# fumchin/bird-sound-event-detecion

Measured on AMD Instinct MI355X. Metric: 10 s clips/sec through mel+CRNN train step, higher is better.
Workload: dtype f32; 1 GPU; waveform->STFT/mel/dB->CRNN(7 conv/BN/GLU/pool + 2xBiGRU128)->Predictor->BCE strong+weak->backward->Adam; BASELINE configs[2] (main_baseline.py train step on SYN); mode=crnn, sr=22050, frames=865, out_frames=216, batch_per_gpu=256, global_batch=256, parallelism=dp1, hip_graph=False

## Files before the change

### bird-sound-event-detecion_amd/csrc/bsed_common.h

```cpp
#pragma once
#include <hip/hip_runtime.h>
#include <stdint.h>
#include <stdio.h>
#include <algorithm>
#include "../../include/bsed.h"

#define BSED_OK 0
#define BSED_ERR_ARG (-1)
#define BSED_ERR_HIP (-2)
#define BSED_ERR_STATE (-3)

void bsed_set_error(const char* fmt, ...);
const uint64_t* bsed_seed_add_ptr();
const int* bsed_step_add_ptr();
const float* bsed_lr_ptr();

#define BSED_CHECK_ARG(cond, ...)                 \
  do {                                            \
    if (!(cond)) {                                \
      bsed_set_error(__VA_ARGS__);                \
      return BSED_ERR_ARG;                        \
    }                                             \
  } while (0)

// ... 210 lines not shown
  return kernel >= 0 && kernel < 8 ? names[kernel] : nullptr;
}
static inline int bsed_glu_plan_for(const BsedGluDesc& d, int kernel, BsedGluPlan& p) {
  const char* who = bsed_glu_name(kernel);
  BSED_CHECK_ARG(who, "bsed_glu_plan: unknown kernel %d", kernel);
  const bool tiled = kernel >= BSED_GLU_BWD_FUSED, glu3 = kernel >= BSED_GLU_FWD3;
  const bool block0 = kernel == BSED_GLU_BLOCK0_FWD || kernel == BSED_GLU_BLOCK0_BWD;
  const int C = d.C;
  BSED_CHECK_ARG(d.NB > 0 && d.H > 0 && d.W > 0, "%s: bad shape", who);
  BSED_CHECK_ARG((d.ph == 1 || d.ph == 2) && (d.pw == 1 || d.pw == 2), "%s: pooling windows must be 1 or 2", who);
  BSED_CHECK_ARG(d.act_bf16 == 0 || (d.act_bf16 == 1 && (glu3 || block0)), "%s: no bf16 activations (act_bf16 = %d)",
                 who, d.act_bf16);
  if (!tiled) BSED_CHECK_ARG(C == 16, "%s: built for 16 channels (got %d)", who, C);
  else if (kernel == BSED_GLU_BWD3) BSED_CHECK_ARG(C == 32 || C == 64, "%s: built for C in {32,64} (got %d)", who, C);
  else if (kernel == BSED_GLU_BWD3N) BSED_CHECK_ARG(C == 128, "%s: built for C = 128 (got %d)", who, C);
  else BSED_CHECK_ARG(C == 32 || C == 64 || C == 128, "%s: built for C in {32,64,128} (got %d)", who, C);
  const long positions = (long)d.NB * d.H * d.W;
  p.dw_rows = 0; p.variant = 0; p.table_bytes = 0;
  if (!tiled) {
    BSED_CHECK_ARG(d.TH == 0 && d.TW == 0, "%s: a streaming kernel without a tile: TH = TW = 0 (got %dx%d)", who, d.TH,
                   d.TW);
    BSED_CHECK_ARG(d.W % d.pw == 0 && d.H >= d.ph, "%s: bad shape (W %% pw == 0, H >= ph)", who);
    BSED_CHECK_ARG(!block0 || positions < (1L << 31), "%s: too many positions", who);
    const long rows = (long)d.NB * (d.H / d.ph);
    long items = rows, g = std::min<long>(rows, 8192);
    if (kernel == BSED_GLU_16_BWD) {
      items = (long)d.NB * d.H * ((d.W + 63) / 64);
      g = std::min<long>(2048, (long)d.NB * d.H);
    } else if (kernel == BSED_GLU_BLOCK0_FWD) {
      items = rows * ((d.W + 127) / 128);
      g = std::min<long>(items, 8192);
    } else if (kernel == BSED_GLU_BLOCK0_BWD) {
      items = rows * ((d.W + 63) / 64);
      g = std::min<long>(8192, rows);
    }
    BSED_CHECK_ARG(items < (1L << 30), "%s: too many rows", who);
    p.G = (int)g; p.max_G = (int)items;
    if (kernel == BSED_GLU_16_BWD || kernel == BSED_GLU_BLOCK0_BWD) p.dw_rows = p.G;
    if (block0) p.variant = d.ph | (positions < (1L << 28) && !(d.act_bf16 && kernel == BSED_GLU_BLOCK0_FWD) ? 16 : 0);
    return BSED_OK;
  }
  BSED_CHECK_ARG(d.TH * d.TW == 128, "%s: TH*TW must be 128 (got %dx%d)", who, d.TH, d.TW);
  const int lgTW = ilog2_exact(d.TW);
  BSED_CHECK_ARG(lgTW >= 0, "%s: TW must be a power of two", who);
  BSED_CHECK_ARG(d.W % d.TW == 0, "%s: TW must divide W", who);
  const long ntiles = (long)d.NB * ceil_div(d.H, d.TH) * (d.W / d.TW);
  BSED_CHECK_ARG(ntiles < (1L << 31), "%s: too many tiles", who);
  BSED_CHECK_ARG(!glu3 || positions * C < (1L << 32),
                 "%s: activation tensor beyond the 32-bit element offsets of this kernel", who);
  int round = 0, slabs = 0;
  if (kernel == BSED_GLU_BWD_FUSED) {
    round = C == 128 ? 256 : (C == 64 ? 512 : 768);
    slabs = C == 128 ? 1 : (C == 64 ? 2 : 4);
    p.variant = C == 128 ? 8 : 4;
  } else if (kernel == BSED_GLU_FWD3) {
    round = C == 128 ? 512 : 1536;
  } else if (kernel == BSED_GLU_BWD3) {
    round = C == 32 ? 768 : 512;
    slabs = 4;
  } else {
    round = 256;
    p.table_bytes = (size_t)2 * 4 * 8 * 2 * 64 * 16;
  }
  p.max_G = (int)(kernel == BSED_GLU_BWD3N ? (ntiles + 1) / 2 : ntiles);
  p.G = std::min(p.max_G, round);
  p.dw_rows = p.G * slabs;
  if (kernel == BSED_GLU_FWD3 || kernel == BSED_GLU_BWD3) p.variant = lgTW == 4 ? 4 : -1;
  return BSED_OK;
}

static inline int bsed_glu_args(const BsedGluDesc* desc, int kernel, unsigned reads, BsedGluPlan& plan,
                                const uint64_t*& seed_add) {
  const char* who = bsed_glu_name(kernel);
  BSED_CHECK_ARG(desc, "%s: null descriptor", who);
  const BsedGluDesc& d = *desc;
  const int rc = bsed_glu_plan_for(d, kernel, plan);
  if (rc) return rc;
  static const char* const names[] = {"x", "y", "cw", "cb", "scale", "shift", "w", "wfwd", "bias", "dpool", "pooled", "g",
                                      "dlin", "part_dw", "part_db", "part_st", "part_gx", "frag_table"};
  const void* const ptrs[] = {d.x, d.y, d.cw, d.cb, d.scale, d.shift, d.w, d.wfwd, d.bias, d.dpool, d.pooled, d.g,
                              d.dlin, d.part_dw, d.part_db, d.part_st, d.part_gx, d.frag_table};
  for (int i = 0; i < 18; ++i) {
    const bool wants = (reads >> i) & 1;
    BSED_CHECK_ARG(wants == (ptrs[i] != nullptr), wants ? "%s: null tensor %s" : "%s: does not read %s: it must be null",
                   who, names[i]);
  }
  BSED_CHECK_ARG(d.G > 0 && d.G <= plan.max_G, "%s: G must be in 1..%d (got %d)", who, plan.max_G, d.G);
  seed_add = bsed_seed_add_ptr();
  return BSED_OK;
}
enum : unsigned {
  GLU_X = 1u << 0, GLU_Y = 1u << 1, GLU_CONV = 3u << 2 , GLU_BN = 3u << 4 , GLU_W = 1u << 6,
  GLU_WFWD = 1u << 7, GLU_BIAS = 1u << 8, GLU_DPOOL = 1u << 9, GLU_POOLED = 1u << 10, GLU_G = 1u << 11,
  GLU_DLIN = 1u << 12, GLU_PART_DW = 1u << 13, GLU_PART_B = 3u << 14 , GLU_PART_GX = 1u << 16,
  GLU_FRAG = 1u << 17,
  GLU_LIN = GLU_BN | GLU_W | GLU_BIAS
};

template <class Params>
static int bsed_glu_geometry(Params& P, const BsedGluDesc* desc, int kernel, unsigned reads, BsedGluPlan& plan) {
  const int rc = bsed_glu_args(desc, kernel, reads, plan, P.seed_add);
  if (rc) return rc;
  const BsedGluDesc& d = *desc;
  P.y = d.y; P.scale = d.scale; P.shift = d.shift; P.bias = d.bias; P.dpool = d.dpool;
  P.g = d.g; P.part_dw = d.part_dw; P.part_db = d.part_db; P.part_st = d.part_st;
  P.NB = d.NB; P.H = d.H; P.W = d.W; P.TH = d.TH; P.TW = d.TW;
  P.lgTW = ilog2_exact(d.TW);
  P.tilesH = ceil_div(d.H, d.TH); P.tilesW = d.W / d.TW;
  P.ntiles = d.NB * P.tilesH * P.tilesW;
  P.ph = d.ph; P.pw = d.pw; P.Hp = d.H / d.ph; P.Wp = d.W / d.pw;
  P.drop_p = d.drop_p; P.rng_stream = d.rng_stream; P.seed = d.seed;
  return BSED_OK;
}

#if defined(__HIPCC__)
__device__ __forceinline__ uint4 philox4x32(uint64_t counter, uint32_t stream, uint64_t seed) {
  uint32_t c0 = (uint32_t)counter, c1 = (uint32_t)(counter >> 32), c2 = stream, c3 = 0x5eed5eedu;
  uint32_t k0 = (uint32_t)seed, k1 = (uint32_t)(seed >> 32);
#pragma unroll
  for (int r = 0; r < 10; ++r) {
    const uint32_t M0 = 0xD2511F53u, M1 = 0xCD9E8D57u;
    uint32_t hi0 = __umulhi(M0, c0), lo0 = M0 * c0;
    uint32_t hi1 = __umulhi(M1, c2), lo1 = M1 * c2;
    uint32_t n0 = hi1 ^ c1 ^ k0, n1 = lo1, n2 = hi0 ^ c3 ^ k1, n3 = lo0;
    c0 = n0; c1 = n1; c2 = n2; c3 = n3;
    k0 += 0x9E3779B9u; k1 += 0xBB67AE85u;
  }
  return make_uint4(c0, c1, c2, c3);
}

__device__ __forceinline__ float dropout_scale(uint64_t e, uint32_t stream, uint64_t seed, float p) {
  if (p <= 0.f) return 1.f;
  uint4 r = philox4x32(e >> 2, stream, seed);
  uint32_t w = (e & 3) == 0 ? r.x : (e & 3) == 1 ? r.y : (e & 3) == 2 ? r.z : r.w;
  float u = (float)(w >> 8) * (1.0f / 16777216.0f);
  return u >= p ? 1.0f / (1.0f - p) : 0.f;
}

__device__ __forceinline__ float sigmoidf_(float x) { return 1.0f / (1.0f + expf(-x)); }
__device__ __forceinline__ float sigmoid_fast(float x) { return __builtin_amdgcn_rcpf(1.0f + __expf(-x)); }

__device__ __forceinline__ uint32_t mix32(uint32_t x) {
  x ^= x >> 16; x *= 0x7feb352dU; x ^= x >> 15; x *= 0x846ca68bU; x ^= x >> 16;
  return x;
}
__device__ __forceinline__ uint32_t drop_key(uint32_t stream, uint64_t seed) {
  return mix32((uint32_t)seed ^ (stream * 0x9E3779B9u)) + mix32((uint32_t)(seed >> 32) ^ 0x85ebca6bu);
}
__device__ __forceinline__ uint32_t drop_threshold(float p) { return (uint32_t)(p * 16777216.0f); }
__device__ __forceinline__ float drop_mul(uint64_t e, uint32_t key, uint32_t thr, float scale) {
  const uint32_t h = mix32((uint32_t)e * 0x9E3779B1u + key + (uint32_t)(e >> 32) * 0x85ebca6bu);
  return (h >> 8) >= thr ? scale : 0.f;
}

__device__ __forceinline__ uint32_t drop_threshold16(float p) { return (uint32_t)(p * 65536.0f); }
__device__ __forceinline__ void drop_mul2(uint64_t e_even, uint32_t key, uint32_t thr16, float scale, float& m0,
                                          float& m1) {
  const uint64_t e = e_even >> 1;
  const uint32_t h = mix32((uint32_t)e * 0x9E3779B1u + key + (uint32_t)(e >> 32) * 0x85ebca6bu);
  m0 = (h & 0xFFFFu) >= thr16 ? scale : 0.f;
  m1 = (h >> 16) >= thr16 ? scale : 0.f;
}

__device__ __forceinline__ void drop_mul2_32(uint32_t e_even, uint32_t key, uint32_t thr16, float scale, float& m0,
                                             float& m1) {
  const uint32_t h = mix32((e_even >> 1) * 0x9E3779B1u + key);
  m0 = (h & 0xFFFFu) >= thr16 ? scale : 0.f;
  m1 = (h >> 16) >= thr16 ? scale : 0.f;
}

__device__ __forceinline__ float wave_sum(float v) {
#pragma unroll
  for (int o = 32; o > 0; o >>= 1) v += __shfl_xor(v, o, 64);
  return v;
}
__device__ __forceinline__ float wave_max(float v) {
#pragma unroll
  for (int o = 32; o > 0; o >>= 1) v = fmaxf(v, __shfl_xor(v, o, 64));
  return v;
}
#endif
```

### bird-sound-event-detecion_amd/csrc/capi.hip

```cpp
#include "bsed_common.h"
#include "../../include/bsed.h"
#include <stdarg.h>

static thread_local char g_err[512] = "";

void bsed_set_error(const char* fmt, ...) {
  va_list ap;
  va_start(ap, fmt);
  vsnprintf(g_err, sizeof(g_err), fmt, ap);
  va_end(ap);
}

extern "C" const char* bsed_last_error(void) { return g_err; }
extern "C" const char* bsed_build_info(void) { return "libbsed gfx950: fp32 storage/accumulation, split-fp32 (bf16x3) contractions on v_mfma_f32_32x32x16_bf16 by default, "
         "exact-fp32 v_mfma_f32_32x32x2_f32 kernels selectable (hand-written HIP)"; }
extern "C" int bsed_abi_version(void) { return 15; }

extern "C" int bsed_glu_plan(const BsedGluDesc* desc, int kernel, BsedGluPlan* out) {
  BSED_CHECK_ARG(desc && out, "bsed_glu_plan: null argument");
  return bsed_glu_plan_for(*desc, kernel, *out);
}
extern "C" int bsed_igemm_plan(const BsedIgemmDesc* desc, int kernel, BsedContractPlan* out) {
  static int (*const run[])(const BsedIgemmDesc*, void*, BsedContractPlan*) = {bsed_run_igemm, bsed_run_igemm3,
                                                                                bsed_run_igemm3s, bsed_run_igemm3n};
  BSED_CHECK_ARG(desc && out && kernel >= BSED_CONTRACT_IGEMM && kernel <= BSED_CONTRACT_IGEMM3N,
                 "bsed_igemm_plan: null argument or unknown kernel %d", kernel);
  return run[kernel](desc, nullptr, out);
}
extern "C" int bsed_wgrad_plan(const BsedWgradDesc* desc, int kernel, BsedContractPlan* out) {
  BSED_CHECK_ARG(desc && out && (kernel == BSED_CONTRACT_WGRAD || kernel == BSED_CONTRACT_WGRAD3),
                 "bsed_wgrad_plan: null argument or unknown kernel %d", kernel);
  return bsed_run_wgrad(desc, kernel == BSED_CONTRACT_WGRAD3, nullptr, out);
}

static thread_local const uint64_t* g_seed_add = nullptr;
static thread_local const int* g_step_add = nullptr;
static thread_local const float* g_lr = nullptr;
const uint64_t* bsed_seed_add_ptr() { return g_seed_add; }
const int* bsed_step_add_ptr() { return g_step_add; }
const float* bsed_lr_ptr() { return g_lr; }
extern "C" int bsed_set_step_state(const void* seed_add_dev, const void* step_add_dev, const void* lr_dev) {
  BSED_CHECK_ARG((seed_add_dev != nullptr) == (step_add_dev != nullptr) && (seed_add_dev != nullptr) == (lr_dev != nullptr),
                 "bsed_set_step_state: the three pointers are set together or cleared together");
  g_seed_add = (const uint64_t*)seed_add_dev;
  g_step_add = (const int*)step_add_dev;
  g_lr = (const float*)lr_dev;
  return BSED_OK;
}
__global__ void step_state_advance_kernel(uint64_t* seed_add, int* step_add, uint64_t seed_inc, int step_inc) {
  if (threadIdx.x == 0 && blockIdx.x == 0) { *seed_add += seed_inc; *step_add += step_inc; }
}
extern "C" int bsed_step_state_advance(void* seed_add_dev, void* step_add_dev, uint64_t seed_inc, int step_inc, void* stream) {
  BSED_CHECK_ARG(seed_add_dev && step_add_dev, "bsed_step_state_advance: null state");
  hipLaunchKernelGGL(step_state_advance_kernel, dim3(1), dim3(64), 0, (hipStream_t)stream, (uint64_t*)seed_add_dev,
                     (int*)step_add_dev, seed_inc, step_inc);
  BSED_LAUNCH_CHECK();
  return BSED_OK;
}
```

### bird-sound-event-detecion_amd/csrc/glu3.hip

```cpp
#include "bsed_common.h"
#include "../../include/bsed.h"
#include <algorithm>
#include <stdlib.h>

typedef short bf16x8 __attribute__((ext_vector_type(8)));
typedef uint32_t u32x4 __attribute__((ext_vector_type(4)));

#define G3_THREADS 256
#define G3_M 128

struct Glu3Params {
  const float* y; const float* scale; const float* shift;
  const float* w;
  const float* bias; const float* dpool;
  float* g; float* part_dw; float* part_db; float* part_st;
  float* pooled;
  int NB, H, W, TH, TW, lgTW, tilesH, tilesW, ntiles;
  int ph, pw, Hp, Wp;
  float drop_p; uint32_t rng_stream; uint64_t seed;
  const uint64_t* seed_add;
};

__device__ __forceinline__ void wave_lds_fence() { asm volatile("s_waitcnt lgkmcnt(0)" ::: "memory"); }
template <int NT>
__device__ __forceinline__ void acc_handoff_fence(f32x16 (&acc)[NT]) {
  if constexpr (NT == 1) asm volatile("s_waitcnt lgkmcnt(0)\n\ts_nop 7" : "+v"(acc[0]) :: "memory");
  else if constexpr (NT == 2) asm volatile("s_waitcnt lgkmcnt(0)\n\ts_nop 7" : "+v"(acc[0]), "+v"(acc[1]) :: "memory");
  else asm volatile("s_waitcnt lgkmcnt(0)\n\ts_nop 7" : "+v"(acc[0]), "+v"(acc[1]), "+v"(acc[2]), "+v"(acc[3]) :: "memory");
}
template <int ABF>
__device__ __forceinline__ f32x16 mfma_sp(const bf16x8& a_hi, const bf16x8& a_lo, const bf16x8& b_hi, const bf16x8& b_lo,
                                          f32x16 acc) {
  if (!ABF) {
    acc = __builtin_amdgcn_mfma_f32_32x32x16_bf16(a_lo, b_hi, acc, 0, 0, 0);
    acc = __builtin_amdgcn_mfma_f32_32x32x16_bf16(a_hi, b_lo, acc, 0, 0, 0);
  }
  return __builtin_amdgcn_mfma_f32_32x32x16_bf16(a_hi, b_hi, acc, 0, 0, 0);
}
__device__ __forceinline__ int crow3g(int r, int lh) { return (r & 3) + 8 * (r >> 2) + 4 * lh; }
__device__ __forceinline__ uint32_t rne_bits(float x) {
  const uint32_t u = __float_as_uint(x);
  return u + 0x7FFFu + ((u >> 16) & 1u);
}
__device__ __forceinline__ void split_pack2(float a, float b, uint32_t& hi, uint32_t& lo) { bsed_split2(a, b, hi, lo); }
__device__ __forceinline__ void split_pack8(const float* v, bf16x8& hi, bf16x8& lo) {
  u32x4 h, l;
#pragma unroll
  for (int i = 0; i < 4; ++i) {
    uint32_t hh, ll;
    split_pack2(v[2 * i], v[2 * i + 1], hh, ll);
    h[i] = hh; l[i] = ll;
  }
  hi = __builtin_bit_cast(bf16x8, h);
  lo = __builtin_bit_cast(bf16x8, l);
}

template <int C>
__device__ __forceinline__ void build_weight_frags(const float* __restrict__ w, bf16x8* WF, bf16x8* WB, int tid) {
  constexpr int NT = C / 32, KS = C / 16;
  for (int f = tid; f < NT * KS * 64; f += G3_THREADS) {
    const int lane = f & 63, li = lane & 31, lh = lane >> 5;
    const int ks = (f >> 6) % KS, j = (f >> 6) / KS;
    float v[8];
    bf16x8 hi, lo;
#pragma unroll
    for (int q = 0; q < 8; ++q) v[q] = w[(size_t)(32 * j + li) * C + 16 * ks + 8 * lh + q];
    split_pack8(v, hi, lo);
    WF[((j * KS + ks) * 2 + 0) * 64 + lane] = hi;
    WF[((j * KS + ks) * 2 + 1) * 64 + lane] = lo;
    if (WB) {
#pragma unroll
      for (int q = 0; q < 8; ++q) v[q] = w[(size_t)(16 * ks + 8 * lh + q) * C + 32 * j + li];
      split_pack8(v, hi, lo);
      WB[((j * KS + ks) * 2 + 0) * 64 + lane] = hi;
      WB[((j * KS + ks) * 2 + 1) * 64 + lane] = lo;
    }
  }
}

template <int C, int ABF>
__device__ __forceinline__ float a_frags_issue(const Glu3Params& P, int lgTW, int nb, int th0, int tw0, int wave, int li, int lh,
                                               float (&raw)[C / 16][8]) {
  constexpr int KS = C / 16;
  const int mA = wave * 32 + li;
  const int gh = th0 + (mA >> lgTW), gw = tw0 + (mA & ((1 << lgTW) - 1));
  const bool ok = gh < P.H;
  const size_t rp = (((size_t)nb * P.H + (ok ? gh : 0)) * P.W + gw) * C + 8 * lh;
#pragma unroll
  for (int ks = 0; ks < KS; ++ks) act_ld8<ABF>(P.y, rp + 16 * ks, raw[ks]);
  return ok ? 1.0f : 0.0f;
}
template <int C>
__device__ __forceinline__ void a_frags_finish(const float (&raw)[C / 16][8], float okf, const float* s_sc, const float* s_sh,
                                               int lh, bf16x8* a_hi, bf16x8* a_lo) {
  constexpr int KS = C / 16;
#pragma unroll
  for (int ks = 0; ks < KS; ++ks) {
    const float4 s0 = *reinterpret_cast<const float4*>(s_sc + 16 * ks + 8 * lh);
    const float4 s1 = *reinterpret_cast<const float4*>(s_sc + 16 * ks + 8 * lh + 4);
    const float4 h0 = *reinterpret_cast<const float4*>(s_sh + 16 * ks + 8 * lh);
    const float4 h1 = *reinterpret_cast<const float4*>(s_sh + 16 * ks + 8 * lh + 4);
    float v[8];
    v[0] = fmaf(raw[ks][0], s0.x, h0.x) * okf; v[1] = fmaf(raw[ks][1], s0.y, h0.y) * okf;
    v[2] = fmaf(raw[ks][2], s0.z, h0.z) * okf; v[3] = fmaf(raw[ks][3], s0.w, h0.w) * okf;
    v[4] = fmaf(raw[ks][4], s1.x, h1.x) * okf; v[5] = fmaf(raw[ks][5], s1.y, h1.y) * okf;
    v[6] = fmaf(raw[ks][6], s1.z, h1.z) * okf; v[7] = fmaf(raw[ks][7], s1.w, h1.w) * okf;
    split_pack8(v, a_hi[ks], a_lo[ks]);
  }
}
template <int C, int ABF>
__device__ __forceinline__ void load_a_frags(const Glu3Params& P, int lgTW, const float* s_sc, const float* s_sh, int nb,
                                             int th0, int tw0, int wave, int li, int lh, bf16x8* a_hi, bf16x8* a_lo) {
  float raw[C / 16][8];
  const float okf = a_frags_issue<C, ABF>(P, lgTW, nb, th0, tw0, wave, li, lh, raw);
  a_frags_finish<C>(raw, okf, s_sc, s_sh, lh, a_hi, a_lo);
}

__device__ float g3_sink[G3_M];

__device__ __forceinline__ float drop_mul32(uint32_t e, uint32_t key, uint32_t thr, float scale) {
  const uint32_t h = mix32(e * 0x9E3779B1u + key);
  return (h >> 8) >= thr ? scale : 0.f;
}

#define G3_B32_WPE 3
template <int C, int LGTW, int ABF>
__global__ __launch_bounds__(G3_THREADS, C == 32 ? G3_B32_WPE : 2) void glu_bwd3_kernel(const Glu3Params P) {
  constexpr int NT = C / 32, KS = C / 16;
  const int lgTW = LGTW >= 0 ? LGTW : P.lgTW;
  const int TWc = 1 << lgTW, THc = G3_M >> lgTW;
  constexpr int DP = 2 * C + 8;
  extern __shared__ __align__(16) unsigned char smem_raw[];
  bf16x8* WF = reinterpret_cast<bf16x8*>(smem_raw);
  bf16x8* WB = WF + NT * KS * 2 * 64;
  float* s_sc = reinterpret_cast<float*>(WB + NT * KS * 2 * 64);
  float* s_sh = s_sc + C;
  unsigned short* Dall = reinterpret_cast<unsigned short*>(s_sh + C);
  const int tid = threadIdx.x, wave = __builtin_amdgcn_readfirstlane(tid >> 6), lane = tid & 63, li = lane & 31, lh = lane >> 5;
  unsigned short* D = Dall + wave * 32 * DP;

  build_weight_frags<C>(P.w, WF, WB, tid);
  for (int i = tid; i < C; i += G3_THREADS) { s_sc[i] = P.scale[i]; s_sh[i] = P.shift[i]; }
  __syncthreads();

  const int sph = P.ph >> 1, spw = P.pw >> 1;
  const float inv_pool = 1.0f / (float)(P.ph * P.pw);
  const uint32_t dkey = drop_key(P.rng_stream, P.seed + (P.seed_add ? *P.seed_add : 0)), dthr = drop_threshold(P.drop_p);
  const float dscale = P.drop_p > 0.f ? 1.0f / (1.0f - P.drop_p) : 1.0f;

  float bias[NT], csc[NT], csh[NT], sdb[NT], sgs[NT], sgy[NT];
  f32x16 acc3[NT][NT];
#pragma unroll
  for (int j = 0; j < NT; ++j) {
    bias[j] = P.bias[32 * j + li];
    csc[j] = s_sc[32 * j + li]; csh[j] = s_sh[32 * j + li];
    sdb[j] = 0.f; sgs[j] = 0.f; sgy[j] = 0.f;
#pragma unroll
    for (int jc = 0; jc < NT; ++jc)
#pragma unroll
      for (int r = 0; r < 16; ++r) acc3[j][jc][r] = 0.f;
  }

  constexpr bool PREF = C == 32 && LGTW >= 0;
  constexpr bool KEEPY = C == 32 && LGTW >= 0;
  constexpr bool G2 = C == 32 && LGTW >= 0;
  float nraw[KS][8];
  float nokf = 0.f;
  auto tile_origin = [&](int t, int& nb_, int& th0_, int& tw0_) {
    const int tw_i = t % P.tilesW; t /= P.tilesW;
    const int th_i = t % P.tilesH;
    nb_ = t / P.tilesH; th0_ = th_i * THc; tw0_ = tw_i * TWc;
  };
  if (PREF && (int)blockIdx.x < P.ntiles) {
    int nb_, th0_, tw0_;
    tile_origin(blockIdx.x, nb_, th0_, tw0_);
    nokf = a_frags_issue<C, ABF>(P, lgTW, nb_, th0_, tw0_, wave, li, lh, nraw);
  }
  for (int tile0 = blockIdx.x; tile0 < P.ntiles; tile0 += gridDim.x) {
    int nb, th0, tw0;
    tile_origin(tile0, nb, th0, tw0);
    int lhv = 4 * lh;
    if (LGTW < 0) asm volatile("" : "+v"(lhv));

    f32x16 acc[NT];
    {
      bf16x8 a_hi[KS], a_lo[KS];
      if (PREF) a_frags_finish<C>(nraw, nokf, s_sc, s_sh, lh, a_hi, a_lo);
      else load_a_frags<C, ABF>(P, lgTW, s_sc, s_sh, nb, th0, tw0, wave, li, lh, a_hi, a_lo);
#pragma unroll
      for (int j = 0; j < NT; ++j)
#pragma unroll
        for (int r = 0; r < 16; ++r) acc[j][r] = 0.f;
#pragma unroll
      for (int ks = 0; ks < KS; ++ks)
#pragma unroll
        for (int j = 0; j < NT; ++j) {
          const bf16x8 b_hi = WF[((j * KS + ks) * 2 + 0) * 64 + lane];
          const bf16x8 b_lo = WF[((j * KS + ks) * 2 + 1) * 64 + lane];
          acc[j] = mfma_sp<ABF>(a_hi[ks], a_lo[ks], b_hi, b_lo, acc[j]);
        }
    }
    if (PREF) {
      const int nt = tile0 + (int)gridDim.x < P.ntiles ? tile0 + (int)gridDim.x : tile0;
      int nb_, th0_, tw0_;
      tile_origin(nt, nb_, th0_, tw0_);
      nokf = a_frags_issue<C, ABF>(P, lgTW, nb_, th0_, tw0_, wave, li, lh, nraw);
    }

    bf16x8 da_hi[NT][2], da_lo[NT][2], xb_hi[NT][2], xb_lo[NT][2];
    uint32_t ykeep[KEEPY ? 16 : 1][NT];
#pragma unroll
    for (int f = 0; f < 2; ++f) {
      float dl8[NT][8], xn8[NT][8];
      uint32_t dvr[2][4][NT], yvr[2][4][NT];
      float mk[2][4];
      uint32_t posv[2][4];
      auto issue = [&](int h) {
        const int rg = 2 * f + h;
#pragma unroll
        for (int rr = 0; rr < 4; ++rr) {
          const int mm = wave * 32 + 8 * rg + lhv + rr;
          const int gh = th0 + (mm >> lgTW), gw = tw0 + (mm & (TWc - 1));
          const int gph = gh >> sph, gpw = gw >> spw;
          mk[h][rr] = (gh < P.H && gph < P.Hp && gpw < P.Wp) ? inv_pool : 0.f;
          posv[h][rr] = ((uint32_t)(nb * P.H + min(gh, P.H - 1)) * (uint32_t)P.W + gw) * C + li;
          const uint32_t dpo = ((uint32_t)(nb * P.Hp + min(gph, P.Hp - 1)) * (uint32_t)P.Wp + min(gpw, P.Wp - 1)) * C + li;
#pragma unroll
          for (int j = 0; j < NT; ++j) {
            dvr[h][rr][j] = act_ld_raw<ABF>(P.dpool, dpo + 32 * j);
            yvr[h][rr][j] = act_ld_raw<ABF>(P.y, posv[h][rr] + 32 * j);
          }
        }
      };
      if (G2) { issue(0); issue(1); __builtin_amdgcn_sched_barrier(0); }
#pragma unroll
      for (int h = 0; h < 2; ++h) {
        const int rg = 2 * f + h;
        if (!G2) { issue(h); __builtin_amdgcn_sched_barrier(0); }
#pragma unroll
        for (int rr = 0; rr < 4; ++rr) {
          const int r = 4 * rg + rr;
          const int row = 8 * rg + lhv + rr;
#pragma unroll
          for (int j = 0; j < NT; ++j) {
            const int n = 32 * j + li;
            if (KEEPY) ykeep[r][j] = yvr[h][rr][j];
            const float xn = fmaf(act_cvt<ABF>(yvr[h][rr][j]), csc[j], csh[j]);
            const float sg = sigmoid_fast(xn);
            const float lin = acc[j][r] + bias[j];
            const float dres = act_cvt<ABF>(dvr[h][rr][j]) * mk[h][rr] * drop_mul32(posv[h][rr] + 32 * j, dkey, dthr, dscale);
            const float dl = dres * sg;
            const float tt = dres * lin * sg * (1.0f - sg);
            sdb[j] += dl;
            dl8[j][4 * h + rr] = dl;
            xn8[j][4 * h + rr] = xn;
            acc[j][r] = tt;
            const uint32_t hb = rne_bits(dl) & 0xFFFF0000u;
            D[row * DP + n] = (unsigned short)(hb >> 16);
            D[row * DP + C + n] = (unsigned short)(rne_bits(dl - __uint_as_float(hb)) >> 16);
          }
        }
      }
#pragma unroll
      for (int j = 0; j < NT; ++j) {
        split_pack8(dl8[j], da_hi[j][f], da_lo[j][f]);
        split_pack8(xn8[j], xb_hi[j][f], xb_lo[j][f]);
      }
    }
    acc_handoff_fence<NT>(acc);

#pragma unroll
    for (int ks = 0; ks < KS; ++ks) {
      const bf16x8 d_hi = *reinterpret_cast<const bf16x8*>(D + li * DP + 16 * ks + 8 * lh);
      const bf16x8 d_lo = *reinterpret_cast<const bf16x8*>(D + li * DP + C + 16 * ks + 8 * lh);
#pragma unroll
      for (int j = 0; j < NT; ++j) {
        const bf16x8 b_hi = WB[((j * KS + ks) * 2 + 0) * 64 + lane];
        const bf16x8 b_lo = WB[((j * KS + ks) * 2 + 1) * 64 + lane];
        acc[j] = mfma_sp<ABF>(d_hi, d_lo, b_hi, b_lo, acc[j]);
      }
    }
    wave_lds_fence();

#pragma unroll
    for (int jc = 0; jc < NT; ++jc)
#pragma unroll
      for (int jn = 0; jn < NT; ++jn)
#pragma unroll
        for (int f = 0; f < 2; ++f) {
          acc3[jn][jc] = mfma_sp<ABF>(da_hi[jn][f], da_lo[jn][f], xb_hi[jc][f], xb_lo[jc][f], acc3[jn][jc]);
        }

#pragma unroll
    for (int rg = 0; rg < 4; ++rg) {
      uint32_t yvr[4][NT];
      float okf[4];
      uint32_t posv[4];
      float* gdst[4];
      uint32_t gidx[4];
#pragma unroll
      for (int rr = 0; rr < 4; ++rr) {
        const int mm = wave * 32 + 8 * rg + lhv + rr;
        const int gh = th0 + (mm >> lgTW), gw = tw0 + (mm & (TWc - 1));
        okf[rr] = gh < P.H ? 1.0f : 0.0f;
        posv[rr] = ((uint32_t)(nb * P.H + min(gh, P.H - 1)) * (uint32_t)P.W + gw) * C + li;
        gdst[rr] = gh < P.H ? P.g : g3_sink;
        gidx[rr] = gh < P.H ? posv[rr] : (uint32_t)li;
#pragma unroll
        for (int j = 0; j < NT; ++j) yvr[rr][j] = KEEPY ? ykeep[4 * rg + rr][j] : act_ld_raw<ABF>(P.y, posv[rr] + 32 * j);
      }
      if (!KEEPY) __builtin_amdgcn_sched_barrier(0);
#pragma unroll
      for (int rr = 0; rr < 4; ++rr) {
#pragma unroll
        for (int j = 0; j < NT; ++j) {
          const float gv = acc[j][4 * rg + rr] * okf[rr];
          act_st<ABF>(gdst[rr], gidx[rr] + 32 * j, gv);
          sgs[j] += gv;
          sgy[j] = fmaf(gv, act_cvt<ABF>(yvr[rr][j]), sgy[j]);
        }
      }
    }
  }

#pragma unroll
  for (int jn = 0; jn < NT; ++jn)
#pragma unroll
    for (int jc = 0; jc < NT; ++jc)
#pragma unroll
      for (int r = 0; r < 16; ++r) {
        const int n = 32 * jn + crow3g(r, lh);
        P.part_dw[(((size_t)blockIdx.x * 4 + wave) * C + n) * C + 32 * jc + li] = acc3[jn][jc][r];
      }
  __syncthreads();
  float* red = reinterpret_cast<float*>(Dall);
#pragma unroll
  for (int j = 0; j < NT; ++j) {
    const float a = sdb[j] + __shfl_xor(sdb[j], 32, 64);
    const float b = sgs[j] + __shfl_xor(sgs[j], 32, 64);
    const float c = sgy[j] + __shfl_xor(sgy[j], 32, 64);
    if (lh == 0) {
      red[(wave * 3 + 0) * C + 32 * j + li] = a;
      red[(wave * 3 + 1) * C + 32 * j + li] = b;
      red[(wave * 3 + 2) * C + 32 * j + li] = c;
    }
  }
  __syncthreads();
  for (int e = tid; e < 3 * C; e += G3_THREADS) {
    const int which = e / C, n = e % C;
    const float s = red[(0 * 3 + which) * C + n] + red[(1 * 3 + which) * C + n] + red[(2 * 3 + which) * C + n] +
                    red[(3 * 3 + which) * C + n];
    if (which == 0) {
      P.part_db[((size_t)blockIdx.x * 2 + 0) * C + n] = s;
      P.part_db[((size_t)blockIdx.x * 2 + 1) * C + n] = 0.f;
    } else {
      P.part_st[((size_t)blockIdx.x * 2 + (which - 1)) * C + n] = s;
    }
  }
}

__global__ void glu3_pack_frags_kernel(const float* __restrict__ w, bf16x8* __restrict__ table) {
  constexpr int C = 128, NT = 4, KS = 8;
  const int f = blockIdx.x * blockDim.x + threadIdx.x;
  if (f >= NT * KS * 64) return;
  const int lane = f & 63, li = lane & 31, lh = lane >> 5;
  const int ks = (f >> 6) % KS, j = (f >> 6) / KS;
  bf16x8* WF = table;
  bf16x8* WB = table + NT * KS * 2 * 64;
  float v[8];
  bf16x8 hi, lo;
#pragma unroll
  for (int q = 0; q < 8; ++q) v[q] = w[(size_t)(32 * j + li) * C + 16 * ks + 8 * lh + q];
  split_pack8(v, hi, lo);
  WF[((j * KS + ks) * 2 + 0) * 64 + lane] = hi;
  WF[((j * KS + ks) * 2 + 1) * 64 + lane] = lo;
#pragma unroll
  for (int q = 0; q < 8; ++q) v[q] = w[(size_t)(16 * ks + 8 * lh + q) * C + 32 * j + li];
  split_pack8(v, hi, lo);
  WB[((j * KS + ks) * 2 + 0) * 64 + lane] = hi;
  WB[((j * KS + ks) * 2 + 1) * 64 + lane] = lo;
}

#define G3N_THREADS 512
template <int ABF>
__global__ __launch_bounds__(G3N_THREADS) void glu_bwd3n_kernel(const Glu3Params P, const bf16x8* __restrict__ table,
                                                                float* __restrict__ dlin) {
  constexpr int C = 128, NT = 4, KS = 8;
#ifdef G3N_LGTW
  constexpr int g3n_lgTW = G3N_LGTW, g3n_TW = 1 << G3N_LGTW;
#else
  const int g3n_lgTW = P.lgTW, g3n_TW = P.TW;
#endif
  constexpr int DQ = 2 * 16 + 8;
  extern __shared__ __align__(16) unsigned char smem_raw[];
  bf16x8* WF = reinterpret_cast<bf16x8*>(smem_raw);
  bf16x8* WB = WF + NT * KS * 2 * 64;
  float* s_sc = reinterpret_cast<float*>(WB + NT * KS * 2 * 64);
  float* s_sh = s_sc + C;
  unsigned short* Dall = reinterpret_cast<unsigned short*>(s_sh + C);
  const int tid = threadIdx.x, wave8 = __builtin_amdgcn_readfirstlane(tid >> 6), lane = tid & 63, li = lane & 31, lh = lane >> 5;
  const int wave = wave8 & 3, half = wave8 >> 2;
  unsigned short* D = Dall + wave8 * 32 * DQ;

  for (int i = tid; i < 2 * NT * KS * 2 * 64; i += G3N_THREADS) WF[i] = table[i];
  for (int i = tid; i < C; i += G3N_THREADS) { s_sc[i] = P.scale[i]; s_sh[i] = P.shift[i]; }
  __syncthreads();

  const int sph = P.ph >> 1, spw = P.pw >> 1;
  const float inv_pool = 1.0f / (float)(P.ph * P.pw);
  const uint32_t dkey = drop_key(P.rng_stream, P.seed + (P.seed_add ? *P.seed_add : 0)), dthr = drop_threshold(P.drop_p);
  const float dscale = P.drop_p > 0.f ? 1.0f / (1.0f - P.drop_p) : 1.0f;

  float bias[NT], csc[NT], csh[NT], sdb[NT], sgs[NT], sgy[NT];
#pragma unroll
  for (int j = 0; j < NT; ++j) {
    bias[j] = P.bias[32 * j + li];
    csc[j] = s_sc[32 * j + li]; csh[j] = s_sh[32 * j + li];
    sdb[j] = 0.f; sgs[j] = 0.f; sgy[j] = 0.f;
  }

  for (int tile0 = 2 * blockIdx.x + half; tile0 < P.ntiles; tile0 += 2 * gridDim.x) {
    int tile = tile0;
    const int tw_i = tile % P.tilesW; tile /= P.tilesW;
    const int th_i = tile % P.tilesH;
    const int nb = tile / P.tilesH;
    const int th0 = th_i * P.TH, tw0 = tw_i * P.TW;
    int lhv = 4 * lh;
    asm volatile("" : "+v"(lhv));

    f32x16 acc[NT];
    {
      bf16x8 a_hi[KS], a_lo[KS];
      load_a_frags<C, ABF>(P, g3n_lgTW, s_sc, s_sh, nb, th0, tw0, wave, li, lh, a_hi, a_lo);
#pragma unroll
      for (int j = 0; j < NT; ++j)
#pragma unroll
        for (int r = 0; r < 16; ++r) acc[j][r] = 0.f;
#pragma unroll
      for (int ks = 0; ks < KS; ++ks)
#pragma unroll
        for (int j = 0; j < NT; ++j) {
          const bf16x8 b_hi = WF[((j * KS + ks) * 2 + 0) * 64 + lane];
          const bf16x8 b_lo = WF[((j * KS + ks) * 2 + 1) * 64 + lane];
          acc[j] = mfma_sp<ABF>(a_hi[ks], a_lo[ks], b_hi, b_lo, acc[j]);
        }
    }

    uint32_t dph[NT][8], dpl[NT][8];
#pragma unroll
    for (int rg = 0; rg < 4; ++rg) {
      uint32_t dvr[4][NT], yvr[4][NT];
      float mk[4];
      uint32_t posv[4];
      float* dlrow[4];
      uint32_t dlidx[4];
#pragma unroll
      for (int rr = 0; rr < 4; ++rr) {
        const int mm = wave * 32 + 8 * rg + lhv + rr;
        const int gh = th0 + (mm >> g3n_lgTW), gw = tw0 + (mm & (g3n_TW - 1));
        const int gph = gh >> sph, gpw = gw >> spw;
        mk[rr] = (gh < P.H && gph < P.Hp && gpw < P.Wp) ? inv_pool : 0.f;
        posv[rr] = ((uint32_t)(nb * P.H + min(gh, P.H - 1)) * (uint32_t)P.W + gw) * C + li;
        dlrow[rr] = gh < P.H ? dlin : g3_sink;
        dlidx[rr] = gh < P.H ? posv[rr] : (uint32_t)li;
        const uint32_t dpo = ((uint32_t)(nb * P.Hp + min(gph, P.Hp - 1)) * (uint32_t)P.Wp + min(gpw, P.Wp - 1)) * C + li;
#pragma unroll
        for (int j = 0; j < NT; ++j) {
          dvr[rr][j] = act_ld_raw<ABF>(P.dpool, dpo + 32 * j);
          yvr[rr][j] = act_ld_raw<ABF>(P.y, posv[rr] + 32 * j);
        }
      }
      __builtin_amdgcn_sched_barrier(0);
#pragma unroll
      for (int rp = 0; rp < 2; ++rp)
#pragma unroll
        for (int j = 0; j < NT; ++j) {
          float dl2[2];
#pragma unroll
          for (int e = 0; e < 2; ++e) {
            const int rr = 2 * rp + e, r = 4 * rg + rr;
            const float xn = fmaf(act_cvt<ABF>(yvr[rr][j]), csc[j], csh[j]);
            const float sg = sigmoid_fast(xn);
            const float lin = acc[j][r] + bias[j];
            const float dres = act_cvt<ABF>(dvr[rr][j]) * mk[rr] * drop_mul32(posv[rr] + 32 * j, dkey, dthr, dscale);
            const float dl = dres * sg;
            acc[j][r] = dres * lin * sg * (1.0f - sg);
            sdb[j] += dl;
            act_st<ABF>(dlrow[rr], dlidx[rr] + 32 * j, dl);
            dl2[e] = dl;
          }
          split_pack2(dl2[0], dl2[1], dph[j][2 * rg + rp], dpl[j][2 * rg + rp]);
        }
    }

    acc_handoff_fence<NT>(acc);
#pragma unroll
    for (int q = 0; q < 8; ++q) {
      if ((li >> 4) == (q & 1)) {
#pragma unroll
        for (int i = 0; i < 8; ++i) {
          const int r = 2 * i;
          const int row = 8 * (r >> 2) + lhv + (r & 3);
          D[row * DQ + (li & 15)] = (unsigned short)(dph[q >> 1][i] & 0xFFFFu);
          D[(row + 1) * DQ + (li & 15)] = (unsigned short)(dph[q >> 1][i] >> 16);
          D[row * DQ + 16 + (li & 15)] = (unsigned short)(dpl[q >> 1][i] & 0xFFFFu);
          D[(row + 1) * DQ + 16 + (li & 15)] = (unsigned short)(dpl[q >> 1][i] >> 16);
        }
      }
      wave_lds_fence();
      const bf16x8 d_hi = *reinterpret_cast<const bf16x8*>(D + li * DQ + 8 * lh);
      const bf16x8 d_lo = *reinterpret_cast<const bf16x8*>(D + li * DQ + 16 + 8 * lh);
#pragma unroll
      for (int j = 0; j < NT; ++j) {
        const bf16x8 b_hi = WB[((j * KS + q) * 2 + 0) * 64 + lane];
        const bf16x8 b_lo = WB[((j * KS + q) * 2 + 1) * 64 + lane];
        acc[j] = mfma_sp<ABF>(d_hi, d_lo, b_hi, b_lo, acc[j]);
      }
      wave_lds_fence();
    }

#pragma unroll
    for (int rg = 0; rg < 4; ++rg) {
      uint32_t yvr[4][NT];
      float okf[4];
      uint32_t posv[4];
      float* gdst[4];
      uint32_t gidx[4];
#pragma unroll
      for (int rr = 0; rr < 4; ++rr) {
        const int mm = wave * 32 + 8 * rg + lhv + rr;
        const int gh = th0 + (mm >> g3n_lgTW), gw = tw0 + (mm & (g3n_TW - 1));
        okf[rr] = gh < P.H ? 1.0f : 0.0f;
        posv[rr] = ((uint32_t)(nb * P.H + min(gh, P.H - 1)) * (uint32_t)P.W + gw) * C + li;
        gdst[rr] = gh < P.H ? P.g : g3_sink;
        gidx[rr] = gh < P.H ? posv[rr] : (uint32_t)li;
#pragma unroll
        for (int j = 0; j < NT; ++j) yvr[rr][j] = act_ld_raw<ABF>(P.y, posv[rr] + 32 * j);
      }
      __builtin_amdgcn_sched_barrier(0);
#pragma unroll
      for (int rr = 0; rr < 4; ++rr)
#pragma unroll
        for (int j = 0; j < NT; ++j) {
          const float gv = acc[j][4 * rg + rr] * okf[rr];
          act_st<ABF>(gdst[rr], gidx[rr] + 32 * j, gv);
          sgs[j] += gv;
          sgy[j] = fmaf(gv, act_cvt<ABF>(yvr[rr][j]), sgy[j]);
        }
    }
  }

  __syncthreads();
  float* red = reinterpret_cast<float*>(Dall);
#pragma unroll
  for (int j = 0; j < NT; ++j) {
    const float a = sdb[j] + __shfl_xor(sdb[j], 32, 64);
    const float b = sgs[j] + __shfl_xor(sgs[j], 32, 64);
    const float c = sgy[j] + __shfl_xor(sgy[j], 32, 64);
    if (lh == 0) {
      red[(wave8 * 3 + 0) * C + 32 * j + li] = a;
      red[(wave8 * 3 + 1) * C + 32 * j + li] = b;
      red[(wave8 * 3 + 2) * C + 32 * j + li] = c;
    }
  }
  __syncthreads();
  for (int e = tid; e < 3 * C; e += G3N_THREADS) {
    const int which = e / C, n = e % C;
    float s = 0.f;
#pragma unroll
    for (int wv = 0; wv < 8; ++wv) s += red[(wv * 3 + which) * C + n];
    if (which == 0) {
      P.part_db[((size_t)blockIdx.x * 2 + 0) * C + n] = s;
      P.part_db[((size_t)blockIdx.x * 2 + 1) * C + n] = 0.f;
    } else {
      P.part_st[((size_t)blockIdx.x * 2 + (which - 1)) * C + n] = s;
    }
  }
}

template <int C, int LGTW, int ABF>
__global__ __launch_bounds__(G3_THREADS, 2) void glu_fwd3_kernel(const Glu3Params P) {
  constexpr int NT = C / 32, KS = C / 16;
  const int lgTW = LGTW >= 0 ? LGTW : P.lgTW;
  const int TWc = 1 << lgTW, THc = G3_M >> lgTW;
  extern __shared__ __align__(16) unsigned char smem_raw[];
  bf16x8* WF = reinterpret_cast<bf16x8*>(smem_raw);
  float* s_sc = reinterpret_cast<float*>(WF + NT * KS * 2 * 64);
  float* s_sh = s_sc + C;
  const int tid = threadIdx.x, wave = __builtin_amdgcn_readfirstlane(tid >> 6), lane = tid & 63, li = lane & 31, lh = lane >> 5;
  constexpr bool STAGE = C <= 64;
  constexpr int YROW = C + 4;
  float* Ys = s_sh + C + wave * 32 * YROW;

  build_weight_frags<C>(P.w, WF, nullptr, tid);
  for (int i = tid; i < C; i += G3_THREADS) { s_sc[i] = P.scale[i]; s_sh[i] = P.shift[i]; }
  __syncthreads();

  const int sph = P.ph >> 1, spw = P.pw >> 1;
  const float inv_pool = 1.0f / (float)(P.ph * P.pw);
  const uint32_t dkey = drop_key(P.rng_stream, P.seed + (P.seed_add ? *P.seed_add : 0)), dthr = drop_threshold(P.drop_p);
  const float dscale = P.drop_p > 0.f ? 1.0f / (1.0f - P.drop_p) : 1.0f;
  const int TW = TWc;
  float bias[NT], csc[NT], csh[NT];
#pragma unroll
  for (int j = 0; j < NT; ++j) {
    bias[j] = P.bias[32 * j + li];
    csc[j] = s_sc[32 * j + li]; csh[j] = s_sh[32 * j + li];
  }

  for (int tile0 = blockIdx.x; tile0 < P.ntiles; tile0 += gridDim.x) {
    int tile = tile0;
    const int tw_i = tile % P.tilesW; tile /= P.tilesW;
    const int th_i = tile % P.tilesH;
    const int nb = tile / P.tilesH;
    const int th0 = th_i * THc, tw0 = tw_i * TWc;
    int lhv = 4 * lh;
    if (C > 64) asm volatile("" : "+v"(lhv));

    f32x16 acc[NT];
    {
      bf16x8 a_hi[KS], a_lo[KS];
      if constexpr (STAGE) {
        constexpr int EP = ABF ? 8 : 4, Q = C / EP, NL = 32 * Q / 64;
        f32x4 raw[NL][ABF ? 2 : 1];
#pragma unroll
        for (int k = 0; k < NL; ++k) {
          const int e = lane + 64 * k, pr = e / Q, q = e % Q;
          const int mm = wave * 32 + pr;
          const int gh = th0 + (mm >> lgTW), gw = tw0 + (mm & (TW - 1));
          const size_t o = (((size_t)nb * P.H + min(gh, P.H - 1)) * P.W + gw) * C + EP * q;
          const float okr = gh < P.H ? 1.0f : 0.0f;
          if (ABF) {
            float v8[8];
            act_ld8<ABF>(P.y, o, v8);
            raw[k][0] = f32x4{v8[0], v8[1], v8[2], v8[3]} * okr;
            raw[k][ABF ? 1 : 0] = f32x4{v8[4], v8[5], v8[6], v8[7]} * okr;
          } else {
            raw[k][0] = *reinterpret_cast<const f32x4*>(P.y + o) * okr;
          }
        }
        asm volatile("s_waitcnt lgkmcnt(0)" ::: "memory");
#pragma unroll
        for (int k = 0; k < NL; ++k) {
          const int e = lane + 64 * k;
          *reinterpret_cast<f32x4*>(Ys + (e / Q) * YROW + EP * (e % Q)) = raw[k][0];
          if (ABF) *reinterpret_cast<f32x4*>(Ys + (e / Q) * YROW + EP * (e % Q) + 4) = raw[k][ABF ? 1 : 0];
        }
        asm volatile("s_waitcnt lgkmcnt(0)" ::: "memory");
        const int mA = wave * 32 + li;
        const float okf = th0 + (mA >> lgTW) < P.H ? 1.0f : 0.0f;
#pragma unroll
        for (int ks = 0; ks < KS; ++ks) {
          const f32x4 r0 = *reinterpret_cast<const f32x4*>(Ys + li * YROW + 16 * ks + 8 * lh);
          const f32x4 r1 = *reinterpret_cast<const f32x4*>(Ys + li * YROW + 16 * ks + 8 * lh + 4);
          const float4 s0 = *reinterpret_cast<const float4*>(s_sc + 16 * ks + 8 * lh);
          const float4 s1 = *reinterpret_cast<const float4*>(s_sc + 16 * ks + 8 * lh + 4);
          const float4 h0 = *reinterpret_cast<const float4*>(s_sh + 16 * ks + 8 * lh);
          const float4 h1 = *reinterpret_cast<const float4*>(s_sh + 16 * ks + 8 * lh + 4);
          float v[8];
          v[0] = fmaf(r0[0], s0.x, h0.x) * okf; v[1] = fmaf(r0[1], s0.y, h0.y) * okf;
          v[2] = fmaf(r0[2], s0.z, h0.z) * okf; v[3] = fmaf(r0[3], s0.w, h0.w) * okf;
          v[4] = fmaf(r1[0], s1.x, h1.x) * okf; v[5] = fmaf(r1[1], s1.y, h1.y) * okf;
          v[6] = fmaf(r1[2], s1.z, h1.z) * okf; v[7] = fmaf(r1[3], s1.w, h1.w) * okf;
          split_pack8(v, a_hi[ks], a_lo[ks]);
        }
      } else {
        load_a_frags<C, ABF>(P, lgTW, s_sc, s_sh, nb, th0, tw0, wave, li, lh, a_hi, a_lo);
      }
#pragma unroll
      for (int j = 0; j < NT; ++j)
#pragma unroll
        for (int r = 0; r < 16; ++r) acc[j][r] = 0.f;
#pragma unroll
      for (int ks = 0; ks < KS; ++ks)
#pragma unroll
        for (int j = 0; j < NT; ++j) {
          const bf16x8 b_hi = WF[((j * KS + ks) * 2 + 0) * 64 + lane];
          const bf16x8 b_lo = WF[((j * KS + ks) * 2 + 1) * 64 + lane];
          acc[j] = mfma_sp<ABF>(a_hi[ks], a_lo[ks], b_hi, b_lo, acc[j]);
        }
    }

#pragma unroll
    for (int rg = 0; rg < 4; ++rg) {
      uint32_t yvr[4][NT];
      float mk[4];
      uint32_t posv[4];
#pragma unroll
      for (int rr = 0; rr < 4; ++rr) {
        const int mm = wave * 32 + 8 * rg + lhv + rr;
        const int gh = th0 + (mm >> lgTW), gw = tw0 + (mm & (TW - 1));
        mk[rr] = gh < P.H ? 1.0f : 0.0f;
        posv[rr] = ((uint32_t)(nb * P.H + min(gh, P.H - 1)) * (uint32_t)P.W + gw) * C + li;
#pragma unroll
        for (int j = 0; j < NT; ++j)
          yvr[rr][j] = STAGE ? __float_as_uint(Ys[(8 * rg + lhv + rr) * YROW + 32 * j + li]) : act_ld_raw<ABF>(P.y, posv[rr] + 32 * j);
      }
      if (!STAGE) __builtin_amdgcn_sched_barrier(0);
#pragma unroll
      for (int rr = 0; rr < 4; ++rr)
#pragma unroll
        for (int j = 0; j < NT; ++j) {
          const float xn = fmaf((STAGE ? __uint_as_float(yvr[rr][j]) : act_cvt<ABF>(yvr[rr][j])), csc[j], csh[j]);
          const float keep = mk[rr] * drop_mul32(posv[rr] + 32 * j, dkey, dthr, dscale);
          acc[j][4 * rg + rr] = (acc[j][4 * rg + rr] + bias[j]) * sigmoid_fast(xn) * keep;
        }
    }

    if (P.ph == 1) {
#pragma unroll
      for (int r = 0; r < 16; ++r) {
        if (P.pw == 2 && (r & 1)) continue;
        const int mm = wave * 32 + crow3g(r, 0) + lhv;
        const int gh = th0 + (mm >> lgTW), gw = tw0 + (mm & (TW - 1));
        const int gpw = gw >> spw;
        if (gh < P.H && gpw < P.Wp) {
          const size_t dst = (((size_t)nb * P.Hp + gh) * P.Wp + gpw) * C + li;
#pragma unroll
          for (int j = 0; j < NT; ++j) {
            const float v = P.pw == 2 ? acc[j][r] + acc[j][r | 1] : acc[j][r];
            act_st<ABF>(P.pooled, dst + 32 * j, v * inv_pool);
          }
        }
      }
    } else {
      const int dr = TW == 16 ? 8 : (TW == 8 ? 4 : (TW == 2 ? 2 : 1));
#pragma unroll
      for (int r = 0; r < 16; ++r) {
        const int mm = wave * 32 + crow3g(r, 0) + lhv;
        const int lr = mm >> lgTW;
        const int gh = th0 + lr, gw = tw0 + (mm & (TW - 1));
        const int gph = gh >> 1, gpw = gw >> spw;
        const bool top = (lr & 1) == 0 && (P.pw == 1 || (gw & 1) == 0);
        if (top && gph < P.Hp && gpw < P.Wp) {
          const size_t dst = (((size_t)nb * P.Hp + gph) * P.Wp + gpw) * C + li;
#pragma unroll
          for (int j = 0; j < NT; ++j) {
            float v;
            if (dr == 8) v = acc[j][r] + acc[j][(r + 8) & 15] + (P.pw == 2 ? acc[j][r | 1] + acc[j][((r + 8) & 15) | 1] : 0.f);
            else if (dr == 4) v = acc[j][r] + acc[j][(r + 4) & 15] + (P.pw == 2 ? acc[j][r | 1] + acc[j][((r + 4) & 15) | 1] : 0.f);
            else if (dr == 2) v = acc[j][r] + acc[j][(r + 2) & 15] + (P.pw == 2 ? acc[j][r | 1] + acc[j][((r + 2) & 15) | 1] : 0.f);
            else v = acc[j][r] + acc[j][(r + 1) & 15];
            act_st<ABF>(P.pooled, dst + 32 * j, v * inv_pool);
          }
        }
      }
    }
  }
}

template <int C, int ABF>
static int launch_glu_fwd3(const Glu3Params& P, int G, bool const_tw, hipStream_t s) {
  constexpr int NT = C / 32, KS = C / 16;
  const size_t smem = (size_t)NT * KS * 2 * 64 * 16 + 2 * C * sizeof(float) +
                      (C <= 64 ? (size_t)4 * 32 * (C + 4) * sizeof(float) : 0);
  static BsedLdsOnce once, once4;
  if (const_tw) {
    BSED_HIP(bsed_max_lds(once4, (const void*)glu_fwd3_kernel<C, 4, ABF>));
    hipLaunchKernelGGL((glu_fwd3_kernel<C, 4, ABF>), dim3(G), dim3(G3_THREADS), smem, s, P);
  } else {
    BSED_HIP(bsed_max_lds(once, (const void*)glu_fwd3_kernel<C, -1, ABF>));
    hipLaunchKernelGGL((glu_fwd3_kernel<C, -1, ABF>), dim3(G), dim3(G3_THREADS), smem, s, P);
  }
  BSED_LAUNCH_CHECK();
  return BSED_OK;
}

template <int C>
static size_t glu_bwd3_smem() {
  constexpr int NT = C / 32, KS = C / 16;
  return (size_t)2 * NT * KS * 2 * 64 * 16 + 2 * C * sizeof(float) + (size_t)4 * 32 * (2 * C + 8) * 2;
}

template <int C, int ABF>
static int launch_glu_bwd3(const Glu3Params& P, int G, bool const_tw, hipStream_t s) {
  const size_t smem = glu_bwd3_smem<C>();
  static BsedLdsOnce once, once4;
  if (const_tw) {
    BSED_HIP(bsed_max_lds(once4, (const void*)glu_bwd3_kernel<C, 4, ABF>));
    hipLaunchKernelGGL((glu_bwd3_kernel<C, 4, ABF>), dim3(G), dim3(G3_THREADS), smem, s, P);
  } else {
    BSED_HIP(bsed_max_lds(once, (const void*)glu_bwd3_kernel<C, -1, ABF>));
    hipLaunchKernelGGL((glu_bwd3_kernel<C, -1, ABF>), dim3(G), dim3(G3_THREADS), smem, s, P);
  }
  BSED_LAUNCH_CHECK();
  return BSED_OK;
}

extern "C" int bsed_glu_bwd3(const BsedGluDesc* desc, void* stream) {
  Glu3Params P;
  BsedGluPlan plan;
  const int rc = bsed_glu_geometry(P, desc, BSED_GLU_BWD3, GLU_Y | GLU_LIN | GLU_DPOOL | GLU_G | GLU_PART_DW | GLU_PART_B,
                                   plan);
  if (rc) return rc;
  P.w = desc->w; P.pooled = nullptr;
  const int C = desc->C, G = desc->G;
  const bool ctw = plan.variant == 4;
  hipStream_t s = (hipStream_t)stream;
  if (desc->act_bf16) return C == 64 ? launch_glu_bwd3<64, 1>(P, G, ctw, s) : launch_glu_bwd3<32, 1>(P, G, ctw, s);
  if (C == 64) return launch_glu_bwd3<64, 0>(P, G, ctw, s);
  return launch_glu_bwd3<32, 0>(P, G, ctw, s);
}

extern "C" int bsed_glu_fwd3(const BsedGluDesc* desc, void* stream) {
  Glu3Params P;
  BsedGluPlan plan;
  const int rc = bsed_glu_geometry(P, desc, BSED_GLU_FWD3, GLU_Y | GLU_LIN | GLU_POOLED, plan);
  if (rc) return rc;
  const int C = desc->C, G = desc->G, TH = P.TH, TW = P.TW, ph = P.ph, pw = P.pw;
  BSED_CHECK_ARG(pw == 1 || TW >= 2, "bsed_glu_fwd3: horizontal pooling needs TW >= 2");
  BSED_CHECK_ARG(ph == 1 || ((TW == 16 || TW == 8 || TW == 2 || (TW == 1 && pw == 1)) && TH % 2 == 0),
                 "bsed_glu_fwd3: vertical pooling is lane-local only for TW in {1,2,8,16} (got %d)", TW);
  P.w = desc->w; P.pooled = desc->pooled;
  const bool ctw = plan.variant == 4;
  hipStream_t s = (hipStream_t)stream;
  if (desc->act_bf16) return C == 128 ? launch_glu_fwd3<128, 1>(P, G, ctw, s) : (C == 64 ? launch_glu_fwd3<64, 1>(P, G, ctw, s) : launch_glu_fwd3<32, 1>(P, G, ctw, s));
  if (C == 128) return launch_glu_fwd3<128, 0>(P, G, ctw, s);
  if (C == 64) return launch_glu_fwd3<64, 0>(P, G, ctw, s);
  return launch_glu_fwd3<32, 0>(P, G, ctw, s);
}

extern "C" int bsed_glu_bwd3n(const BsedGluDesc* desc, void* stream) {
  Glu3Params P;
  BsedGluPlan plan;
  const int rc = bsed_glu_geometry(P, desc, BSED_GLU_BWD3N,
                                   GLU_Y | GLU_LIN | GLU_DPOOL | GLU_G | GLU_DLIN | GLU_PART_B | GLU_FRAG, plan);
  if (rc) return rc;
  P.w = desc->w; P.pooled = nullptr;
  void* frag_table = desc->frag_table;
  float* dlin = desc->dlin;
  const int G = desc->G;
  hipStream_t s = (hipStream_t)stream;
  hipLaunchKernelGGL(glu3_pack_frags_kernel, dim3(4 * 8 * 64 / 256), dim3(256), 0, s, P.w, (bf16x8*)frag_table);
  const size_t smem = plan.table_bytes + 2 * 128 * sizeof(float) + (size_t)8 * 32 * (2 * 16 + 8) * 2;
  static BsedLdsOnce once, onceb;
  if (desc->act_bf16) {
    BSED_HIP(bsed_max_lds(onceb, (const void*)glu_bwd3n_kernel<1>));
    hipLaunchKernelGGL(glu_bwd3n_kernel<1>, dim3(G), dim3(G3N_THREADS), smem, s, P, (const bf16x8*)frag_table, dlin);
  } else {
    BSED_HIP(bsed_max_lds(once, (const void*)glu_bwd3n_kernel<0>));
    hipLaunchKernelGGL(glu_bwd3n_kernel<0>, dim3(G), dim3(G3N_THREADS), smem, s, P, (const bf16x8*)frag_table, dlin);
  }
  BSED_LAUNCH_CHECK();
  return BSED_OK;
}
```

### bird-sound-event-detecion_amd/csrc/wgrad.hip

```cpp
#include "wgrad_tiles.h"
#include <algorithm>
#include <type_traits>

#define W3_DY_BYTES (2 * IG_TILE_M * 32 * 2)

struct WgradParams {
  BsedWgradDesc d;
  int PW, PH, PP, lgTW, dy_off, ntiles, nct, ntw;
  int CC, lgc4, pw_magic;
  int pack2;
};

template <int MAXS, int NW>
__global__ __launch_bounds__(NW * 64) void wgrad_kernel(const WgradParams P) {
  constexpr int NTHR = NW * 64;
  const BsedWgradDesc& p = P.d;
  extern __shared__ __align__(16) float smem[];
  const int XP = P.CC + 1;
  const int cz0 = blockIdx.z * P.CC;
  float* Xs = smem;
  float* DYs = smem + P.dy_off;
  const int tid = threadIdx.x, wave = tid >> 6, lane = tid & 63, li = lane & 31, lh = lane >> 5;
  const int DYW = 32 * P.ntw;
  const int n0 = blockIdx.y * DYW;
  const int PW = P.PW;
  const int ntap_items = P.pack2 ? (p.ntaps + 1) / 2 : p.ntaps;
  const int nitems = ntap_items * P.nct * P.ntw;

  int xoff[MAXS], boff[MAXS];
  bool valid[MAXS];
  f32x16 acc[MAXS];
#pragma unroll
  for (int s = 0; s < MAXS; ++s) {
    const int it = wave + NW * s;
    valid[s] = it < nitems;
    const int cit = valid[s] ? it % P.nct : 0, rr = valid[s] ? it / P.nct : 0;
    const int nt = rr % P.ntw, tap = rr / P.ntw;
    if (P.pack2) {
      const int ta = 2 * tap, tb = 2 * tap + 1;
      if (li < 16 || tb >= p.ntaps) xoff[s] = (p.dh[ta] * PW + p.dw[ta]) * XP + li;
      else xoff[s] = (p.dh[tb] * PW + p.dw[tb]) * XP + (li - 16);
    } else {
      xoff[s] = (p.dh[tap] * PW + p.dw[tap]) * XP + cit * 32 + li;
    }
    boff[s] = nt * 32 + li;
#pragma unroll
    for (int r = 0; r < 16; ++r) acc[s][r] = 0.f;
  }

  for (int tile0 = blockIdx.x; tile0 < P.ntiles; tile0 += gridDim.x) {
    int tile = tile0;
    const int tw_i = tile % p.tilesW; tile /= p.tilesW;
    const int th_i = tile % p.tilesH;
    const int nb = tile / p.tilesH;
    const int th0 = th_i * p.TH, tw0 = tw_i * p.TW;
    const float* inb = p.in + (size_t)nb * p.H * p.W * p.in_pitch;
    const float* dyb = p.dy + (size_t)nb * p.H * p.W * p.dy_pitch;
    __syncthreads();
    const int c4n = 1 << P.lgc4;
    const int x_total = P.PP * c4n;
    for (int e0 = tid; e0 < x_total; e0 += 4 * NTHR) {
      float4 v[4];
      bool okv[4];
#pragma unroll
      for (int u = 0; u < 4; ++u) {
        const int e = e0 + u * NTHR;
        const int c4 = e & (c4n - 1), pos = e >> P.lgc4;
        const int pr = (pos * P.pw_magic) >> 20, pc = pos - pr * PW;
        const int gh = th0 - p.hh + pr, gw = tw0 - p.hw + pc;
        const int cg = cz0 + 4 * c4;
        v[u] = make_float4(0.f, 0.f, 0.f, 0.f);
        okv[u] = e < x_total && gh >= 0 && gh < p.H && gw >= 0 && gw < p.W && cg < p.CIN;
        if (okv[u]) v[u] = *reinterpret_cast<const float4*>(inb + ((size_t)gh * p.W + gw) * p.in_pitch + cg);
      }
#pragma unroll
      for (int u = 0; u < 4; ++u) {
        const int e = e0 + u * NTHR;
        if (e < x_total) {
          const int c4 = e & (c4n - 1), pos = e >> P.lgc4;
          if (p.a_scale && okv[u]) {
            const int cg = cz0 + 4 * c4;
            const float4 sc = *reinterpret_cast<const float4*>(p.a_scale + cg);
            const float4 sh = *reinterpret_cast<const float4*>(p.a_shift + cg);
            v[u].x = fmaf(v[u].x, sc.x, sh.x); v[u].y = fmaf(v[u].y, sc.y, sh.y);
            v[u].z = fmaf(v[u].z, sc.z, sh.z); v[u].w = fmaf(v[u].w, sc.w, sh.w);
          }
          float* dst = Xs + pos * XP + 4 * c4;
          dst[0] = v[u].x; dst[1] = v[u].y; dst[2] = v[u].z; dst[3] = v[u].w;
        }
      }
    }
    const int n4n = 8 * P.ntw;
    const int lgn4 = P.ntw == 4 ? 5 : (P.ntw == 2 ? 4 : 3);
    for (int e0 = tid; e0 < IG_TILE_M * n4n; e0 += 4 * NTHR) {
      float4 v[4];
#pragma unroll
      for (int u = 0; u < 4; ++u) {
        const int e = e0 + u * NTHR;
        const int n4 = e & (n4n - 1), mm = e >> lgn4;
        const int gh = th0 + (mm >> P.lgTW), gw = tw0 + (mm & (p.TW - 1));
        v[u] = make_float4(0.f, 0.f, 0.f, 0.f);
        if (e < IG_TILE_M * n4n && gh < p.H && gw < p.W && n0 + 4 * n4 < p.N)
          v[u] = *reinterpret_cast<const float4*>(dyb + ((size_t)gh * p.W + gw) * p.dy_pitch + n0 + 4 * n4);
      }
#pragma unroll
      for (int u = 0; u < 4; ++u) {
        const int e = e0 + u * NTHR;
        const int n4 = e & (n4n - 1), mm = e >> lgn4;
        if (e < IG_TILE_M * n4n) *reinterpret_cast<float4*>(DYs + mm * DYW + 4 * n4) = v[u];
      }
    }
    __syncthreads();
#pragma unroll 2
    for (int kp = 0; kp < IG_TILE_M; kp += 2) {
      const int mk = kp + lh;
      const float* dyrow = DYs + mk * DYW;
      const float* xrow = Xs + (((mk >> P.lgTW) + p.hh) * PW + (mk & (p.TW - 1)) + p.hw) * XP;
      float av[MAXS], bv[MAXS];
#pragma unroll
      for (int s = 0; s < MAXS; ++s) {
        av[s] = xrow[xoff[s]];
        bv[s] = dyrow[boff[s]];
      }
#pragma unroll
      for (int s = 0; s < MAXS; ++s) acc[s] = __builtin_amdgcn_mfma_f32_32x32x2f32(av[s], bv[s], acc[s], 0, 0, 0);
    }
  }
  const int NPo = gridDim.y * DYW;
#pragma unroll
  for (int s = 0; s < MAXS; ++s) {
    if (valid[s]) {
      const int it = wave + NW * s;
      const int cit = it % P.nct, rr = it / P.nct;
      const int nt = rr % P.ntw, tap = rr / P.ntw;
#pragma unroll
      for (int r = 0; r < 16; ++r) {
        int ci = cz0 + cit * 32 + crow(r, lh), tp = tap;
        if (P.pack2) {
          const int row = crow(r, lh);
          tp = 2 * tap + (row >> 4);
          ci = row & 15;
          if (tp >= p.ntaps) continue;
        }
        p.part[(((size_t)blockIdx.x * p.ntaps + tp) * p.CINP + ci) * NPo + n0 + nt * 32 + li] = acc[s][r];
      }
    }
  }
}


#define W3_WPE(MAXS, NW) ((MAXS) <= 2 && (NW) == 4 ? 4 : 2)
template <int MAXS, int NW, bool BS, int ABF>
__global__ __launch_bounds__(NW * 64) __attribute__((amdgpu_waves_per_eu(W3_WPE(MAXS, NW)))) void wgrad3_kernel(const WgradParams P) {
  constexpr int NTHR = NW * 64;
  const BsedWgradDesc& p = P.d;
  extern __shared__ __align__(16) uint32_t smw[];
  const int CC = P.CC;
  const int cz0 = blockIdx.z * CC;
  const int DYW = 32 * P.ntw;
  w3_lds_u16* Xh = (w3_lds_u16*)smw;
  w3_lds_u16* Xl = Xh + P.PP * CC;
  w3_lds_u16* DYh = Xh + 2 * P.dy_off;
  w3_lds_u16* DYl = DYh + IG_TILE_M * DYW;
  const int tid = threadIdx.x, wave = tid >> 6, lane = tid & 63, li = lane & 31, lh = lane >> 5;
// ... 26 lines not shown
      const int mk = 8 * lh + 4 * rd + gq;
      const int pr = (mk >> P.lgTW) + p.hh + p.dh[tp], pc = (mk & (p.TW - 1)) + p.hw + p.dw[tp];
      xa[s][rd] = xh0 + 2 * ((pr * PW + pc) * CC + (w3_chunk(cit, pc, P.nct) << 5) + col);
      if (!BS || s == 0) xb[BS ? 0 : s][rd] = dh0 + 2 * (mk * DYW + (w3_chunk(nt, mk, P.ntw) << 5) + 16 * gh + gc);
    }
#pragma unroll
    for (int r = 0; r < 16; ++r) acc[s][r] = 0.f;
  }
  const uint32_t kstep = 2 * (16 >> P.lgTW) * PW * CC;
  const uint32_t bstep = 2 * 16 * DYW;
  float4 sc = make_float4(1.f, 1.f, 1.f, 1.f), sh = make_float4(0.f, 0.f, 0.f, 0.f);
  if (p.a_scale && cz0 + 4 * (tid & ((1 << P.lgc4) - 1)) < p.CIN) {
    sc = *reinterpret_cast<const float4*>(p.a_scale + cz0 + 4 * (tid & ((1 << P.lgc4) - 1)));
    sh = *reinterpret_cast<const float4*>(p.a_shift + cz0 + 4 * (tid & ((1 << P.lgc4) - 1)));
  }
  float4 cA = make_float4(1.f, 1.f, 1.f, 1.f), cB = make_float4(0.f, 0.f, 0.f, 0.f), cC = cB;
  if (p.bn_y && n0 + 4 * (tid & (8 * P.ntw - 1)) < p.N) {
    const int cn = n0 + 4 * (tid & (8 * P.ntw - 1));
    cA = *reinterpret_cast<const float4*>(p.bn_coef + cn);
    cB = *reinterpret_cast<const float4*>(p.bn_coef + p.N + cn);
    const float4 c2 = *reinterpret_cast<const float4*>(p.bn_coef + 2 * p.N + cn);
    const float4 mu = *reinterpret_cast<const float4*>(p.bn_mean + cn);
    cC = make_float4(fmaf(-cB.x, mu.x, c2.x), fmaf(-cB.y, mu.y, c2.y), fmaf(-cB.z, mu.z, c2.z), fmaf(-cB.w, mu.w, c2.w));
  }

  for (int tile0 = blockIdx.x; tile0 < P.ntiles; tile0 += gridDim.x) {
    int tile = tile0;
    const int tw_i = tile % p.tilesW; tile /= p.tilesW;
    const int th_i = tile % p.tilesH;
    const int nb = tile / p.tilesH;
    const int th0 = th_i * p.TH, tw0 = tw_i * p.TW;
    const float* inb = p.in + (size_t)nb * p.H * p.W * p.in_pitch;
    const float* dyb = p.dy + (size_t)nb * p.H * p.W * p.dy_pitch;
    __syncthreads();
    constexpr int UX = 6, UD = 8;
    const int c4n = 1 << P.lgc4;
    const int x_total = P.PP * c4n;
    for (int e0 = tid; e0 < x_total; e0 += UX * NTHR) {
      float4 v[UX];
      bool okv[UX];
      int ov[UX];
#pragma unroll
      for (int u = 0; u < UX; ++u) {
        const int e = e0 + u * NTHR;
        const int c4 = e & (c4n - 1), pos = e >> P.lgc4;
        const int pr = (pos * P.pw_magic) >> 20, pc = pos - pr * PW;
        const int gh_ = th0 - p.hh + pr, gw = tw0 - p.hw + pc;
        const int cg = cz0 + 4 * c4;
        ov[u] = pos * CC + (w3_chunk(c4 >> 3, pc, P.nct) << 5) + 4 * (c4 & 7);
        v[u] = make_float4(0.f, 0.f, 0.f, 0.f);
        okv[u] = e < x_total && gh_ >= 0 && gh_ < p.H && gw >= 0 && gw < p.W && cg < p.CIN;
        if (okv[u]) v[u] = w3_ld4<ABF>(p.in, inb + ((size_t)gh_ * p.W + gw) * p.in_pitch + cg);
      }
#pragma unroll
      for (int u = 0; u < UX; ++u) {
        const int e = e0 + u * NTHR;
        if (e < x_total) {
          if (p.a_scale && okv[u]) {
            v[u].x = fmaf(v[u].x, sc.x, sh.x); v[u].y = fmaf(v[u].y, sc.y, sh.y);
            v[u].z = fmaf(v[u].z, sc.z, sh.z); v[u].w = fmaf(v[u].w, sc.w, sh.w);
          }
          w3_store4<ABF>(Xh, Xl, ov[u], v[u]);
        }
      }
    }
    const int n4n = 8 * P.ntw, lgn4 = P.ntw == 4 ? 5 : (P.ntw == 2 ? 4 : 3);
    const int d_total = IG_TILE_M * n4n;
    for (int e0 = tid; e0 < d_total; e0 += UD * NTHR) {
      float4 v[UD];
#pragma unroll
      for (int u = 0; u < UD; ++u) {
        const int e = e0 + u * NTHR;
        const int n4 = e & (n4n - 1), mm = e >> lgn4;
        const int gh_ = th0 + (mm >> P.lgTW), gw = tw0 + (mm & (p.TW - 1));
        v[u] = make_float4(0.f, 0.f, 0.f, 0.f);
        if (e < d_total && gh_ < p.H && gw < p.W && n0 + 4 * n4 < p.N) {
          const size_t o = ((size_t)nb * p.H * p.W + (size_t)gh_ * p.W + gw) * p.dy_pitch + n0 + 4 * n4;
          v[u] = w3_ld4<ABF>(p.dy, p.dy + o);
          if (p.bn_y) {
            const float4 yv = w3_ld4<ABF>(p.bn_y, p.bn_y + o);
            v[u].x = fmaf(cA.x, v[u].x, fmaf(cB.x, yv.x, cC.x)); v[u].y = fmaf(cA.y, v[u].y, fmaf(cB.y, yv.y, cC.y));
            v[u].z = fmaf(cA.z, v[u].z, fmaf(cB.z, yv.z, cC.z)); v[u].w = fmaf(cA.w, v[u].w, fmaf(cB.w, yv.w, cC.w));
            if (p.dy_out && blockIdx.z == 0) w3_st4<ABF>(p.dy_out, p.dy_out + o, v[u]);
          }
        }
      }
#pragma unroll
      for (int u = 0; u < UD; ++u) {
        const int e = e0 + u * NTHR;
        const int n4 = e & (n4n - 1), mm = e >> lgn4;
        if (e < d_total) w3_store4<ABF>(DYh, DYl, mm * DYW + (w3_chunk(n4 >> 3, mm, P.ntw) << 5) + 4 * (n4 & 7), v[u]);
      }
    }
    __syncthreads();
    constexpr int SG = MAXS > 5 ? 2 : 3, NG = (MAXS + SG - 1) / SG;
    constexpr int SB = BS ? 1 : SG;
    uint32_t ko = 0, kb = 0;
#pragma unroll 1
    for (int kp = 0; kp < IG_TILE_M; kp += 16, ko += kstep, kb += bstep) {
      w3_bf16x8 ah[2][SG], al[2][SG], bh[2][SB], bl[2][SB];
#pragma unroll
      for (int g = 0; g <= NG; ++g) {
        if (g < NG) {
#pragma unroll
          for (int j = 0; j < SG; ++j) {
            const int sl = g * SG + j;
            if (sl < MAXS) {
              ah[g & 1][j] = w3_frag(xa[sl][0] + ko, xa[sl][1] + ko);
              al[g & 1][j] = w3_frag(xa[sl][0] + ko + xlo, xa[sl][1] + ko + xlo);
              if (!BS || sl == 0) {
                bh[g & 1][BS ? 0 : j] = w3_frag(xb[BS ? 0 : sl][0] + kb, xb[BS ? 0 : sl][1] + kb);
                bl[g & 1][BS ? 0 : j] = w3_frag(xb[BS ? 0 : sl][0] + kb + dlo, xb[BS ? 0 : sl][1] + kb + dlo);
              }
            }
          }
        }
        __builtin_amdgcn_sched_barrier(0);
        if (g > 0) {
#pragma unroll
          for (int j = 0; j < SG; ++j) {
            const int sl = (g - 1) * SG + j;
            if (sl < MAXS) {
              const w3_bf16x8 b_hi = BS ? bh[0][0] : bh[(g - 1) & 1][BS ? 0 : j];
              const w3_bf16x8 b_lo = BS ? bl[0][0] : bl[(g - 1) & 1][BS ? 0 : j];
              acc[sl] = w3_mfma<ABF>(ah[(g - 1) & 1][j], al[(g - 1) & 1][j], b_hi, b_lo, acc[sl]);
            }
          }
          __builtin_amdgcn_sched_barrier(0);
        }
      }
    }
  }
  const int NPo = gridDim.y * DYW;
#pragma unroll
  for (int s = 0; s < MAXS; ++s) {
    if (valid[s]) {
      const int it = wave + NW * s;
      const int cit = it % P.nct, rr = it / P.nct;
      const int nt = rr % P.ntw, tap = rr / P.ntw;
#pragma unroll
      for (int r = 0; r < 16; ++r) {
        int ci = cz0 + cit * 32 + crow(r, lh), tp = tap;
        if (P.pack2) {
          const int row = crow(r, lh);
          tp = 2 * tap + (row >> 4);
          ci = row & 15;
          if (tp >= p.ntaps) continue;
        }
        p.part[(((size_t)blockIdx.x * p.ntaps + tp) * p.CINP + ci) * NPo + n0 + nt * 32 + li] = acc[s][r];
      }
    }
  }
}

#define W1_TP 64
#define W1_THREADS 512
#define W1_PLANE (W1_TP * 128 * 2)
#define W1_STAGE (4 * W1_PLANE)

struct W1Set { float4 x[4], d[4]; };

template <bool SHIFT, int ABF>
__global__ __launch_bounds__(W1_THREADS) __attribute__((amdgpu_waves_per_eu(2, 2))) void wgrad1_kernel(const WgradParams P) {
  const BsedWgradDesc& p = P.d;
  extern __shared__ __align__(16) uint32_t smw[];
  const int tid = threadIdx.x, wave = tid >> 6, lane = tid & 63, li = lane & 31, lh = lane >> 5;
  const int cz0 = blockIdx.z * 128, n0 = blockIdx.y * 128;
  const long M = (long)p.NB * p.H * p.W;
  const int ntile = (int)((M + W1_TP - 1) / W1_TP);
  const int cit = wave & 3, nt0 = wave >> 2;
  const int gq = (lane >> 2) & 3, gc = 4 * (lane & 3), gh = (lane >> 4) & 1;
  const uint32_t base = (uint32_t)(uintptr_t)smw;
  uint32_t xa[2], xb[2][2];
#pragma unroll
  for (int rd = 0; rd < 2; ++rd) {
    const int mk = 8 * lh + 4 * rd + gq;
    xa[rd] = base + 2 * (mk * 128 + (w3_chunk(cit, mk, 4) << 5) + 16 * gh + gc);
#pragma unroll
    for (int s = 0; s < 2; ++s)
      xb[s][rd] = base + 2 * W1_PLANE + 2 * (mk * 128 + (w3_chunk(nt0 + 2 * s, mk, 4) << 5) + 16 * gh + gc);
  }
  f32x16 acc[2];
#pragma unroll
  for (int s = 0; s < 2; ++s)
#pragma unroll
    for (int r = 0; r < 16; ++r) acc[s][r] = 0.f;

  const int c4 = tid & 31, p0 = tid >> 5;
  const bool xok = cz0 + 4 * c4 < p.CIN, dok = n0 + 4 * c4 < p.N;
  const float* xsrc = p.in + cz0 + 4 * (xok ? c4 : 0);
  const float* dsrc = p.dy + n0 + 4 * (dok ? c4 : 0);
  float4 sc = make_float4(1.f, 1.f, 1.f, 1.f), sh = make_float4(0.f, 0.f, 0.f, 0.f);
  if (p.a_scale && xok) {
    sc = *reinterpret_cast<const float4*>(p.a_scale + cz0 + 4 * c4);
    sh = *reinterpret_cast<const float4*>(p.a_shift + cz0 + 4 * c4);
  }
  const int shift = SHIFT ? p.dh[0] * p.W + p.dw[0] : 0;
  const int so = p0 * 128 + (w3_chunk(c4 >> 3, p0, 4) << 5) + 4 * (c4 & 7);
  w3_lds_u16* lds = (w3_lds_u16*)smw;

  uint32_t xmask = 0, dmask = 0;
  auto issue = [&](int tile, W1Set& S) {
#pragma unroll
    for (int u = 0; u < 4; ++u) {
      const long m = (long)tile * W1_TP + p0 + 16 * u;
      const long mc = m < M ? m : M - 1;
      long ms = mc;
      if (SHIFT) {
        ms = mc + shift;
        ms = ms < 0 ? 0 : (ms >= M ? M - 1 : ms);
      }
      S.x[u] = w3_ld4<ABF>(p.in, xsrc + (size_t)ms * p.in_pitch);
      S.d[u] = w3_ld4<ABF>(p.dy, dsrc + (size_t)mc * p.dy_pitch);
    }
  };
  auto convert = [&](int tile, const W1Set& S, int stage) {
    w3_lds_u16* xh = lds + stage * (W1_STAGE / 2);
    w3_lds_u16* xl = xh + W1_PLANE / 2;
    w3_lds_u16* dh_ = xh + W1_PLANE;
    w3_lds_u16* dl = dh_ + W1_PLANE / 2;
#pragma unroll
    for (int u = 0; u < 4; ++u) {
      const long m = (long)tile * W1_TP + p0 + 16 * u;
      bool okx = m < M && xok;
      if (SHIFT) {
        const int rem = (int)(m % ((long)p.H * p.W));
        const int h = rem / p.W + p.dh[0], w = rem % p.W + p.dw[0];
        okx = okx && h >= 0 && h < p.H && w >= 0 && w < p.W;
      }
      const bool okd = m < M && dok;
      float4 v = S.x[u];
      v.x = okx ? fmaf(v.x, sc.x, sh.x) : 0.f; v.y = okx ? fmaf(v.y, sc.y, sh.y) : 0.f;
      v.z = okx ? fmaf(v.z, sc.z, sh.z) : 0.f; v.w = okx ? fmaf(v.w, sc.w, sh.w) : 0.f;
      w3_store4<ABF>(xh, xl, so + 16 * u * 128, v);
      float4 g = S.d[u];
      g.x = okd ? g.x : 0.f; g.y = okd ? g.y : 0.f; g.z = okd ? g.z : 0.f; g.w = okd ? g.w : 0.f;
      w3_store4<ABF>(dh_, dl, so + 16 * u * 128, g);
    }
  };
  auto mma = [&](int stage) {
    const uint32_t so_ = stage * W1_STAGE;
#pragma unroll
    for (int k = 0; k < W1_TP / 16; ++k) {
      const uint32_t ko = so_ + k * 16 * 128 * 2;
      const w3_bf16x8 ah = w3_frag(xa[0] + ko, xa[1] + ko);
      const w3_bf16x8 al = w3_frag(xa[0] + ko + W1_PLANE, xa[1] + ko + W1_PLANE);
      w3_bf16x8 bh[2], bl[2];
#pragma unroll
      for (int s = 0; s < 2; ++s) {
        bh[s] = w3_frag(xb[s][0] + ko, xb[s][1] + ko);
        bl[s] = w3_frag(xb[s][0] + ko + W1_PLANE, xb[s][1] + ko + W1_PLANE);
      }
#pragma unroll
      for (int s = 0; s < 2; ++s) {
        acc[s] = w3_mfma<ABF>(ah, al, bh[s], bl[s], acc[s]);
      }
    }
  };
  (void)xmask; (void)dmask;

  const int t0 = blockIdx.x, G = gridDim.x;
  const int n = t0 < ntile ? (ntile - t0 + G - 1) / G : 0;
  W1Set A, B;
  if (n > 0) {
    issue(t0, A);
    issue(t0 + G, B);
    convert(t0, A, 0);
    __syncthreads();
    for (int i = 0; i < n; i += 2) {
      issue(t0 + (i + 2) * G, A);
      mma(0);
      convert(t0 + (i + 1) * G, B, 1);
      __syncthreads();
      if (i + 1 >= n) break;
      issue(t0 + (i + 3) * G, B);
      mma(1);
      convert(t0 + (i + 2) * G, A, 0);
      __syncthreads();
    }
  }
  const int NPo = gridDim.y * 128;
#pragma unroll
  for (int s = 0; s < 2; ++s)
#pragma unroll
    for (int r = 0; r < 16; ++r) {
      const int ci = cz0 + cit * 32 + crow(r, lh);
      p.part[((size_t)blockIdx.x * p.CINP + ci) * NPo + n0 + (nt0 + 2 * s) * 32 + li] = acc[s][r];
    }
}

#define W3P_UX 13
#define W3P_UD 8

struct W3Geo { int CC, lgTW, PW, PP, ntw; };
__host__ __device__ constexpr W3Geo w3_geo(int g) {
  return g == 1 ? W3Geo{64, 4, 18, 180, 2}
       : g == 2 ? W3Geo{64, 3, 10, 180, 2}
       : g == 3 ? W3Geo{32, 4, 18, 180, 2}
       : g == 4 ? W3Geo{64, 2, 6, 204, 1}
       : g == 5 ? W3Geo{32, 1, 4, 264, 2}
       : g == 6 ? W3Geo{32, 4, 18, 180, 1}
                : W3Geo{0, 0, 0, 0, 0};
}
#define W3_NGEO 6

template <int MAXS, int GEO, int ABF>
__global__ __launch_bounds__(512) __attribute__((amdgpu_waves_per_eu(2, 2))) void wgrad3p_kernel(const WgradParams P) {
  constexpr int NTHR = 256, NW = 4, UX = W3P_UX, UD = W3P_UD;
  const BsedWgradDesc& p = P.d;
  extern __shared__ __align__(16) uint32_t smw[];
  const int CC = P.CC;
  const int cz0 = blockIdx.z * CC;
  const int DYW = 32 * P.ntw;
// ... 213 lines not shown
      for (int u = 0; u < UD; ++u) {
        if (GEO && u * NTHR >= d_tot) continue;
        bool ok;
        const uint32_t o = d_at(u, gc, ok);
        vd[u] = ld16(p.dy, gc.dy_img, o);
        if (BNB) vy[u] = ld16(p.bn_y, gc.dy_img, o);
      }
#pragma unroll
      for (int u = 0; u < UX; ++u) {
        if (GEO && u * NTHR >= x_tot) continue;
        bool ok;
        vx[u] = ld16(p.in, gc.in_img, x_at(u, gc, ok));
      }
      for (; tile < P.ntiles; buf ^= 1) {
        const int nxt = tile + gridDim.x;
        const W3Tile gn = w3_tile(p, nxt < P.ntiles ? nxt : tile);
        const int bo = buf * buf_u16;
#pragma unroll
        for (int u = 0; u < UD; ++u) {
          if (GEO && u * NTHR >= d_tot) continue;
          bool ok, okn;
          const uint32_t o = d_at(u, gc, ok);
          w3_f32x4 v = vd[u];
          if (BNB) {
            v[0] = fmaf(cA.x, v[0], fmaf(cB.x, vy[u][0], cC.x));
            v[1] = fmaf(cA.y, v[1], fmaf(cB.y, vy[u][1], cC.y));
            v[2] = fmaf(cA.z, v[2], fmaf(cB.z, vy[u][2], cC.z));
            v[3] = fmaf(cA.w, v[3], fmaf(cB.w, vy[u][3], cC.w));
            if (STORE) *reinterpret_cast<w3_f32x4*>(reinterpret_cast<char*>(p.dy_out + gc.dy_img) + o) = v;
          }
          const float4 w = make_float4(ok ? v[0] : 0.f, ok ? v[1] : 0.f, ok ? v[2] : 0.f, ok ? v[3] : 0.f);
          if (tid + u * NTHR < d_tot) w3_store4<ABF>(DYh, DYl, bo + dyo[u], w);
          const uint32_t on = d_at(u, gn, okn);
          vd[u] = ld16(p.dy, gn.dy_img, on);
          if (BNB) vy[u] = ld16(p.bn_y, gn.dy_img, on);
        }
#pragma unroll
        for (int u = 0; u < UX; ++u) {
          if (GEO && u * NTHR >= x_tot) continue;
          bool ok, okn;
          (void)x_at(u, gc, ok);
          const w3_f32x4 v = vx[u];
          const float4 w = make_float4(ok ? fmaf(v[0], sc.x, sh.x) : 0.f, ok ? fmaf(v[1], sc.y, sh.y) : 0.f,
                                       ok ? fmaf(v[2], sc.z, sh.z) : 0.f, ok ? fmaf(v[3], sc.w, sh.w) : 0.f);
          if (tid + u * NTHR < x_tot) w3_store4<ABF>(Xh, Xl, bo + xo[u], w);
          vx[u] = ld16(p.in, gn.in_img, x_at(u, gn, okn));
        }
        gc = gn; tile = nxt;
        __syncthreads();
      }
    };
    if (!bnb) produce(std::false_type{}, std::false_type{});
    else if (!dy_store) produce(std::true_type{}, std::false_type{});
    else produce(std::true_type{}, std::true_type{});
    __syncthreads();
    return;
  }

  const int tid = threadIdx.x, wave = tid >> 6, lane = tid & 63, li = lane & 31, lh = lane >> 5;
  const int ntap_items = P.pack2 ? (p.ntaps + 1) / 2 : p.ntaps;
  const int nitems = ntap_items * P.nct * P.ntw;
  const int gq = (lane >> 2) & 3, gc = 4 * (lane & 3), gh = (lane >> 4) & 1;
  const uint32_t xh0 = (uint32_t)(uintptr_t)Xh, dh0 = (uint32_t)(uintptr_t)DYh;
  const uint32_t xlo = 2 * P.PP * CC, dlo = 2 * IG_TILE_M * DYW;
  uint32_t xa[MAXS][2], xb[1][2];
  bool valid[MAXS];
  f32x16 acc[MAXS];
#pragma unroll
  for (int s = 0; s < MAXS; ++s) {
    const int it = wave + NW * s;
    valid[s] = it < nitems;
    const int cit = valid[s] ? it % P.nct : 0, rr = valid[s] ? it / P.nct : 0;
    const int nt = rr % P.ntw, tap = rr / P.ntw;
    int tp = tap, col = 16 * gh + gc;
    if (P.pack2) {
      const int tb = 2 * tap + 1;
      tp = 2 * tap;
      if (gh && tb < p.ntaps) { tp = tb; col = gc; }
    }
#pragma unroll
    for (int rd = 0; rd < 2; ++rd) {
      const int mk = 8 * lh + 4 * rd + gq;
      const int pr = (mk >> P.lgTW) + p.hh + p.dh[tp], pc = (mk & (p.TW - 1)) + p.hw + p.dw[tp];
      xa[s][rd] = xh0 + 2 * ((pr * PW + pc) * CC + (w3_chunk(cit, pc, P.nct) << 5) + col);
      if (s == 0) xb[0][rd] = dh0 + 2 * (mk * DYW + (w3_chunk(nt, mk, P.ntw) << 5) + 16 * gh + gc);
    }
#pragma unroll
    for (int r = 0; r < 16; ++r) acc[s][r] = 0.f;
  }
  __syncthreads();
  int buf = 0;
  constexpr int SG = 2;
  for (int tile = blockIdx.x; tile < P.ntiles; tile += gridDim.x, buf ^= 1) {
    if constexpr (GEO > 0) {
      constexpr W3Geo Gm = w3_geo(GEO);
      constexpr uint32_t kstep = 2 * (16 >> Gm.lgTW) * Gm.PW * Gm.CC, bstep = 2 * 16 * 32 * Gm.ntw;
      constexpr uint32_t xloc = 2 * Gm.PP * Gm.CC, dloc = 2 * IG_TILE_M * 32 * Gm.ntw;
      const uint32_t bo = 2 * buf * buf_u16;
      uint32_t xab[MAXS][2], xbb[1][2];
#pragma unroll
      for (int s = 0; s < MAXS; ++s) { xab[s][0] = xa[s][0] + bo; xab[s][1] = xa[s][1] + bo; }
      xbb[0][0] = xb[0][0] + bo; xbb[0][1] = xb[0][1] + bo;
#pragma unroll
      for (int kpi = 0; kpi < IG_TILE_M / 16; ++kpi) w3_kstep<MAXS, SG, true, ABF>(xab, xbb, kpi * kstep, kpi * bstep, xloc, dloc, acc);
    } else {
      const uint32_t kstep = 2 * (16 >> P.lgTW) * PW * CC;
      const uint32_t bstep = 2 * 16 * DYW;
      uint32_t ko = 2 * buf * buf_u16, kb = ko;
#pragma unroll 1
      for (int kp = 0; kp < IG_TILE_M; kp += 16, ko += kstep, kb += bstep) w3_kstep<MAXS, SG, true, ABF>(xa, xb, ko, kb, xlo, dlo, acc);
    }
    __syncthreads();
  }
  const int NPo = gridDim.y * DYW;
#pragma unroll
  for (int s = 0; s < MAXS; ++s) {
    if (valid[s]) {
      const int it = wave + NW * s;
      const int cit = it % P.nct, rr = it / P.nct;
      const int nt = rr % P.ntw, tap = rr / P.ntw;
#pragma unroll
      for (int r = 0; r < 16; ++r) {
        int ci = cz0 + cit * 32 + crow(r, lh), tp = tap;
        if (P.pack2) {
          const int row = crow(r, lh);
          tp = 2 * tap + (row >> 4);
          ci = row & 15;
          if (tp >= p.ntaps) continue;
        }
        p.part[(((size_t)blockIdx.x * p.ntaps + tp) * p.CINP + ci) * NPo + n0 + nt * 32 + li] = acc[s][r];
      }
    }
  }
}

template <int MAXS, int NW>
static int launch_wgrad(const WgradParams& P, const BsedLaunch& L) {
  BSED_LABEL_ONLY(L, "wgrad_kernel<%d, %d>", MAXS, NW);
  static BsedLdsOnce once;
  BSED_HIP(bsed_max_lds(once, (const void*)wgrad_kernel<MAXS, NW>));
  hipLaunchKernelGGL((wgrad_kernel<MAXS, NW>), L.grid, dim3(NW * 64), L.smem, L.s, P);
  BSED_LAUNCH_CHECK();
  return BSED_OK;
}

static int wgrad_prepare(const BsedWgradDesc* desc, WgradParams& P, size_t& smem, dim3& grid_yz, int mode3 = 0) {
  BSED_CHECK_ARG(desc, "bsed_wgrad: null descriptor");
  P.d = *desc;
  BsedWgradDesc& d = P.d;
  P.ntiles = bsed_tile_geometry(P, "bsed_wgrad", 4, 4);
  if (P.ntiles < 0) return P.ntiles;
  BSED_CHECK_ARG(d.N % 4 == 0, "bsed_wgrad: N must be a multiple of 4");
  BSED_CHECK_ARG(d.CINP % 32 == 0 && d.CINP >= d.CIN, "bsed_wgrad: bad padding");
  BSED_CHECK_ARG(d.dy_pitch >= d.N && d.dy_pitch % 4 == 0, "bsed_wgrad: bad pitch");
  BSED_CHECK_ARG((d.bn_y == nullptr) == (d.bn_coef == nullptr) && (d.bn_y == nullptr) == (d.bn_mean == nullptr),
                 "bsed_wgrad: bn_y, bn_coef and bn_mean come together (BatchNorm backward applied on load) or not at all");
  BSED_CHECK_ARG(d.bn_y || !d.dy_out, "bsed_wgrad: dy_out only goes with bn_y");
  BSED_CHECK_ARG(!d.bn_y || mode3, "bsed_wgrad: BatchNorm backward on load is built into the split-fp32 kernels (bsed_wgrad3) only");
  BSED_CHECK_ARG(!d.dy_out || (d.dy_out != d.dy && d.dy_out != d.bn_y), "bsed_wgrad: dy_out must not alias dy or bn_y "
                 "(other workgroups still read them)");
  const bool wide1 = d.ntaps == 1;
  P.CC = 32;
  for (int cand = (wide1 ? 128 : 64); cand >= 32; cand >>= 1)
    if (d.CINP % cand == 0) { P.CC = cand; break; }
  if (mode3 && d.ntaps > 1 && P.CC > 32 && (size_t)P.PP * P.CC * 4 + (size_t)W3_DY_BYTES > 80 * 1024) P.CC = 32;
  BSED_CHECK_ARG(d.CINP % P.CC == 0 && d.CINP / P.CC <= 65535, "bsed_wgrad: CINP must be a multiple of 32");
  P.lgc4 = ilog2_exact(P.CC / 4);
  P.nct = P.CC / 32;
  P.pack2 = (d.CIN <= 16 && d.CINP == 32 && d.ntaps > 1) ? 1 : 0;
  P.dy_off = mode3 ? P.PP * P.CC : ((P.PP * (P.CC + 1) + 3) & ~3);
  P.ntw = 1;
  const int tap_items = P.pack2 ? (d.ntaps + 1) / 2 : d.ntaps;
  for (int cand = 4; cand >= 2; cand >>= 1) {
    const size_t need = mode3 ? (size_t)P.dy_off * 4 + (size_t)W3_DY_BYTES * cand
                              : ((size_t)P.dy_off + IG_TILE_M * 32 * cand) * sizeof(float);
    const size_t budget = wide1 ? 160 * 1024 : 80 * 1024;
    if (d.NP % (32 * cand) == 0 && tap_items * P.nct * cand <= 36 && need <= budget) { P.ntw = cand; break; }
  }
  smem = mode3 ? (size_t)P.dy_off * 4 + (size_t)W3_DY_BYTES * P.ntw
               : ((size_t)P.dy_off + IG_TILE_M * 32 * P.ntw) * sizeof(float);
  BSED_CHECK_ARG(tap_items * P.nct * P.ntw <= 36, "bsed_wgrad: %d work items per workgroup exceed the 36 supported",
                 tap_items * P.nct * P.ntw);
  BSED_CHECK_ARG(smem <= 160 * 1024, "bsed_wgrad: tile needs %zu B of LDS", smem);
  grid_yz = dim3(1, d.NP / (32 * P.ntw), d.CINP / P.CC);
  return BSED_OK;
}

static int wgrad_auto_g(const WgradParams& P, size_t smem, dim3 gyz) {
  const long slots = smem <= 80 * 1024 ? 512 : 256;
  const long want = std::max<long>(1, slots / ((long)gyz.y * gyz.z));
  return (int)std::max<long>(1, std::min<long>(want, P.ntiles));
}

static int wgrad_variant(const WgradParams& P) {
  const BsedWgradDesc& d = P.d;
  const int nitems = (P.pack2 ? (d.ntaps + 1) / 2 : d.ntaps) * P.nct * P.ntw;
  if (nitems >= 16 && d.ntaps == 1) {
    const int slots8 = ceil_div(nitems, 8);
    if (slots8 <= 2) return 2 * 16 + 8;
    if (slots8 <= 3) return 3 * 16 + 8;
    if (slots8 <= 5) return 5 * 16 + 8;
  }
  const int slots = ceil_div(nitems, 4);
  const int m = slots <= 1 ? 1 : slots <= 2 ? 2 : slots <= 3 ? 3 : slots <= 5 ? 5 : 9;
  return m * 16 + 4;
}

static int wgrad_dispatch(const WgradParams& P, const BsedLaunch& L) {
  switch (wgrad_variant(P)) {
#define CASE(MAXS, NW) \
  case MAXS * 16 + NW: return launch_wgrad<MAXS, NW>(P, L);
    CASE(2, 8) CASE(3, 8) CASE(5, 8)
    CASE(1, 4) CASE(2, 4) CASE(3, 4) CASE(5, 4) CASE(9, 4)
#undef CASE
  }
  bsed_set_error("bsed_wgrad: no kernel instance for variant %d", wgrad_variant(P));
  return BSED_ERR_ARG;
}

template <int MAXS, int NW, bool BS>
static int launch_wgrad3(const WgradParams& P, const BsedLaunch& L) {
  BSED_LABEL_ONLY(L, "wgrad3_kernel<%d, %d, %s, %d>", MAXS, NW, BS ? "true" : "false", P.d.act_bf16 ? 1 : 0);
  static BsedLdsOnce once, onceb;
  if (P.d.act_bf16) {
    BSED_HIP(bsed_max_lds(onceb, (const void*)wgrad3_kernel<MAXS, NW, BS, 1>));
    hipLaunchKernelGGL((wgrad3_kernel<MAXS, NW, BS, 1>), L.grid, dim3(NW * 64), L.smem, L.s, P);
  } else {
    BSED_HIP(bsed_max_lds(once, (const void*)wgrad3_kernel<MAXS, NW, BS, 0>));
    hipLaunchKernelGGL((wgrad3_kernel<MAXS, NW, BS, 0>), L.grid, dim3(NW * 64), L.smem, L.s, P);
  }
  BSED_LAUNCH_CHECK();
  return BSED_OK;
}

template <int MAXS, int GEO>
static int launch_wgrad3p_geo(const WgradParams& P, const BsedLaunch& L) {
  BSED_LABEL_ONLY(L, "wgrad3p_kernel<%d, %d, %d>", MAXS, GEO, P.d.act_bf16 ? 1 : 0);
  static BsedLdsOnce once, onceb;
  if (P.d.act_bf16) {
    BSED_HIP(bsed_max_lds(onceb, (const void*)wgrad3p_kernel<MAXS, GEO, 1>));
    hipLaunchKernelGGL((wgrad3p_kernel<MAXS, GEO, 1>), L.grid, dim3(512), 2 * L.smem, L.s, P);
  } else {
    BSED_HIP(bsed_max_lds(once, (const void*)wgrad3p_kernel<MAXS, GEO, 0>));
    hipLaunchKernelGGL((wgrad3p_kernel<MAXS, GEO, 0>), L.grid, dim3(512), 2 * L.smem, L.s, P);
  }
  BSED_LAUNCH_CHECK();
  return BSED_OK;
}

static int wgrad3p_geo(const WgradParams& P) {
  for (int g = 1; g <= W3_NGEO; ++g) {
    const W3Geo G = w3_geo(g);
    if (P.CC == G.CC && P.lgTW == G.lgTW && P.PW == G.PW && P.PP == G.PP && P.ntw == G.ntw) return g;
  }
  return 0;
}

static constexpr int w3p_geo_maxs(int g) { return g <= 2 ? 9 : (g <= 5 ? 5 : 3); }

static bool wgrad3_pipelined(const WgradParams& P, size_t smem) {
  const int nitems = (P.pack2 ? (P.d.ntaps + 1) / 2 : P.d.ntaps) * P.nct * P.ntw;
  return P.d.ntaps > 1 && nitems > 4 &&
         P.d.H < 16384 && P.d.W < 16384 && 2 * smem <= 160 * 1024 && 4 % (P.nct * P.ntw) == 0 && nitems <= 36 &&
         P.PP * (P.CC / 4) <= W3P_UX * 256 && IG_TILE_M * 8 * P.ntw <= W3P_UD * 256 && !getenv("BSED_WGRAD3_NOPIPE");
}

static bool wgrad1_streaming(const WgradParams& P) {
  const BsedWgradDesc& d = P.d;
  return d.ntaps == 1 && P.CC == 128 && P.ntw == 4 && d.CINP % 128 == 0 && d.NP % 128 == 0 && !d.bn_y &&
         (long)d.NB * d.H * d.W < (1L << 31) - 4 * 65536;
}

enum W3Kind { W3_TILE, W3_PIPE, W3_STREAM1 };
struct W3Plan {
  W3Kind kind;
  int maxs, nw, geo;
  bool bs, shifted;
};
static W3Plan wgrad3_plan(const WgradParams& P, size_t smem) {
  if (wgrad1_streaming(P)) return {W3_STREAM1, 0, 0, 0, false, P.d.dh[0] != 0 || P.d.dw[0] != 0};
  const int v = wgrad_variant(P), maxs = v / 16, nw = v % 16;
  if (wgrad3_pipelined(P, smem)) {
    const int m = maxs <= 3 ? 3 : (maxs <= 5 ? 5 : 9), g = wgrad3p_geo(P);
    return {W3_PIPE, m, 1, g && w3p_geo_maxs(g) == m ? g : 0, false, false};
  }
  return {W3_TILE, maxs, nw, 0, nw % (P.nct * P.ntw) == 0, false};
}

template <int GEO = W3_NGEO>
static int launch_wgrad3p(const W3Plan& pl, const WgradParams& P, const BsedLaunch& L) {
  if constexpr (GEO > 0) {
    if (pl.geo == GEO) return launch_wgrad3p_geo<w3p_geo_maxs(GEO), GEO>(P, L);
    return launch_wgrad3p<GEO - 1>(pl, P, L);
  } else {
    if (pl.maxs == 3) return launch_wgrad3p_geo<3, 0>(P, L);
    if (pl.maxs == 5) return launch_wgrad3p_geo<5, 0>(P, L);
    return launch_wgrad3p_geo<9, 0>(P, L);
  }
}

template <bool SHIFT>
static int launch_wgrad1(const WgradParams& P, const BsedLaunch& L) {
  BSED_LABEL_ONLY(L, "wgrad1_kernel<%s, %d>", SHIFT ? "true" : "false", P.d.act_bf16 ? 1 : 0);
  static BsedLdsOnce once, onceb;
  if (P.d.act_bf16) {
    BSED_HIP(bsed_max_lds(onceb, (const void*)wgrad1_kernel<SHIFT, 1>));
    hipLaunchKernelGGL((wgrad1_kernel<SHIFT, 1>), L.grid, dim3(W1_THREADS), 2 * W1_STAGE, L.s, P);
  } else {
    BSED_HIP(bsed_max_lds(once, (const void*)wgrad1_kernel<SHIFT, 0>));
    hipLaunchKernelGGL((wgrad1_kernel<SHIFT, 0>), L.grid, dim3(W1_THREADS), 2 * W1_STAGE, L.s, P);
  }
  BSED_LAUNCH_CHECK();
  return BSED_OK;
}

template <int MAXS, int NW>
static int launch_wgrad3_tile(const W3Plan& pl, const WgradParams& P, const BsedLaunch& L) {
  return pl.bs ? launch_wgrad3<MAXS, NW, true>(P, L) : launch_wgrad3<MAXS, NW, false>(P, L);
}

static int wgrad3_auto_g(const WgradParams& P, const W3Plan& pl, size_t smem, dim3 gyz) {
  long slots = pl.kind == W3_PIPE ? 256 : smem <= 80 * 1024 ? 512 : 256;
  if (pl.kind != W3_PIPE && smem <= 52 * 1024 && wgrad_variant(P) / 16 <= 2) slots = 1024;
  long want = std::max<long>(1, slots / ((long)gyz.y * gyz.z));
  if (gyz.y * gyz.z > 1 && (want % 8) * 16 <= want) want -= want % 8;
  return (int)std::max<long>(1, std::min<long>(want, P.ntiles));
}

static int wgrad3_dispatch(const WgradParams& P, const W3Plan& pl, const BsedLaunch& L) {
  if (pl.kind == W3_STREAM1) return pl.shifted ? launch_wgrad1<true>(P, L) : launch_wgrad1<false>(P, L);
  if (pl.kind == W3_PIPE) return launch_wgrad3p(pl, P, L);
  if (pl.nw == 8) {
    if (pl.maxs == 2) return launch_wgrad3_tile<2, 8>(pl, P, L);
    if (pl.maxs == 3) return launch_wgrad3_tile<3, 8>(pl, P, L);
    return launch_wgrad3_tile<5, 8>(pl, P, L);
  }
  if (pl.maxs == 1) return launch_wgrad3_tile<1, 4>(pl, P, L);
  if (pl.maxs == 2) return launch_wgrad3_tile<2, 4>(pl, P, L);
  if (pl.maxs == 3) return launch_wgrad3_tile<3, 4>(pl, P, L);
  if (pl.maxs == 5) return launch_wgrad3_tile<5, 4>(pl, P, L);
  return launch_wgrad3_tile<9, 4>(pl, P, L);
}

int bsed_run_wgrad(const BsedWgradDesc* desc, int mode3, void* stream, BsedContractPlan* plan) {
  WgradParams P;
  size_t smem;
  dim3 gyz;
  const int rc = wgrad_prepare(desc, P, smem, gyz, mode3);
  if (rc != BSED_OK) return rc;
  const BsedWgradDesc& d = P.d;
  const W3Plan pl = mode3 ? wgrad3_plan(P, smem) : W3Plan{};
  BsedLaunch L;
  if (plan) L = bsed_plan_begin(plan, mode3 ? wgrad3_auto_g(P, pl, smem, gyz) : wgrad_auto_g(P, smem, gyz), P.ntiles, 0);
  else {
    const char* who = mode3 ? "bsed_wgrad3" : "bsed_wgrad";
    BSED_CHECK_ARG(d.in && d.dy && d.part, "%s: null tensor", who);
    BSED_CHECK_ARG(d.G > 0 && d.G <= P.ntiles, "%s: G (%d) must be in 1..%d tiles", who, d.G, P.ntiles);
    L = BsedLaunch{dim3((unsigned)d.G, gyz.y, gyz.z), smem, (hipStream_t)stream, nullptr};
  }
  return mode3 ? wgrad3_dispatch(P, pl, L) : wgrad_dispatch(P, L);
}
extern "C" int bsed_wgrad(const BsedWgradDesc* desc, void* stream) { return bsed_run_wgrad(desc, 0, stream, nullptr); }
extern "C" int bsed_wgrad3(const BsedWgradDesc* desc, void* stream) { return bsed_run_wgrad(desc, 1, stream, nullptr); }
```

### bird-sound-event-detecion_amd/csrc/wgrad_tiles.h

```cpp
#pragma once
#include "bsed_common.h"
#include "../../include/bsed.h"

struct W3Tile { int nb, th0, tw0; size_t in_img, dy_img; };
__device__ __forceinline__ W3Tile w3_tile(const BsedWgradDesc& p, int tile) {
  int t = tile;
  const int tw_i = t % p.tilesW; t /= p.tilesW;
  const int th_i = t % p.tilesH;
  W3Tile g;
  g.nb = t / p.tilesH;
  g.th0 = th_i * p.TH; g.tw0 = tw_i * p.TW;
  g.in_img = (size_t)g.nb * p.H * p.W * p.in_pitch;
  g.dy_img = (size_t)g.nb * p.H * p.W * p.dy_pitch;
  return g;
}

struct W3Bn { float4 A, B, C; };
__device__ __forceinline__ W3Bn w3_bn_identity() {
  const float4 z = make_float4(0.f, 0.f, 0.f, 0.f);
  return W3Bn{make_float4(1.f, 1.f, 1.f, 1.f), z, z};
}
__device__ __forceinline__ W3Bn w3_bn_coef(const BsedWgradDesc& p, int cn) {
  W3Bn c;
  c.A = *reinterpret_cast<const float4*>(p.bn_coef + cn);
  c.B = *reinterpret_cast<const float4*>(p.bn_coef + p.N + cn);
  const float4 c2 = *reinterpret_cast<const float4*>(p.bn_coef + 2 * p.N + cn);
  const float4 mu = *reinterpret_cast<const float4*>(p.bn_mean + cn);
  c.C = make_float4(fmaf(-c.B.x, mu.x, c2.x), fmaf(-c.B.y, mu.y, c2.y), fmaf(-c.B.z, mu.z, c2.z), fmaf(-c.B.w, mu.w, c2.w));
  return c;
}

template <int MAXS, int SG, bool BS, int ABF>
__device__ __forceinline__ void w3_kstep(const uint32_t (&xa)[MAXS][2], const uint32_t (&xb)[BS ? 1 : MAXS][2], uint32_t ko, uint32_t kb,
                                         uint32_t xlo, uint32_t dlo, f32x16 (&acc)[MAXS]) {
  constexpr int NG = (MAXS + SG - 1) / SG, SB = BS ? 1 : SG;
  w3_bf16x8 ah[2][SG], al[2][SG], bh[2][SB], bl[2][SB];
#pragma unroll
  for (int g = 0; g <= NG; ++g) {
    if (g < NG) {
#pragma unroll
      for (int j = 0; j < SG; ++j) {
        const int sl = g * SG + j;
        if (sl < MAXS) {
          ah[g & 1][j] = w3_frag(xa[sl][0] + ko, xa[sl][1] + ko);
          al[g & 1][j] = w3_frag(xa[sl][0] + ko + xlo, xa[sl][1] + ko + xlo);
          if (!BS || sl == 0) {
            bh[g & 1][BS ? 0 : j] = w3_frag(xb[BS ? 0 : sl][0] + kb, xb[BS ? 0 : sl][1] + kb);
            bl[g & 1][BS ? 0 : j] = w3_frag(xb[BS ? 0 : sl][0] + kb + dlo, xb[BS ? 0 : sl][1] + kb + dlo);
          }
        }
      }
    }
    __builtin_amdgcn_sched_barrier(0);
    if (g > 0) {
#pragma unroll
      for (int j = 0; j < SG; ++j) {
        const int sl = (g - 1) * SG + j;
        if (sl < MAXS) {
          const w3_bf16x8 b_hi = BS ? bh[0][0] : bh[(g - 1) & 1][BS ? 0 : j];
          const w3_bf16x8 b_lo = BS ? bl[0][0] : bl[(g - 1) & 1][BS ? 0 : j];
          acc[sl] = w3_mfma<ABF>(ah[(g - 1) & 1][j], al[(g - 1) & 1][j], b_hi, b_lo, acc[sl]);
        }
      }
      __builtin_amdgcn_sched_barrier(0);
    }
  }
}
```

### bird-sound-event-detecion_amd/ops.py

```python
import ctypes
import functools
import os
from typing import NamedTuple

import torch

from . import _lib as L

EPI_PLAIN, EPI_STATS, EPI_GLU_POOL, EPI_GLU_BWD, EPI_ADD_STATS2 = (
    L.CONSTANTS["BSED_EPI_" + n] for n in ("PLAIN", "STATS", "GLU_POOL", "GLU_BWD", "ADD_STATS2"))
PACK_MAX_JOBS = L.CONSTANTS["BSED_PACK_MAX_JOBS"]
REDUCE_MAX_JOBS = L.CONSTANTS["BSED_REDUCE_MAX_JOBS"]
BN_EVAL_MAX_JOBS = L.CONSTANTS["BSED_BN_EVAL_MAX_JOBS"]
IgemmDesc, WgradDesc, HeadBwdDesc, PackJob, ReduceJob, BnEvalJob, GluDesc, GluPlan, ContractPlan = (
    L.STRUCTS["Bsed" + n] for n in ("IgemmDesc", "WgradDesc", "HeadBwdDesc", "PackJob", "ReduceJob", "BnEvalJob", "GluDesc",
                                    "GluPlan", "ContractPlan"))

TAPS3x3 = [(kh - 1, kw - 1) for kh in range(3) for kw in range(3)]
TAP1 = ((0, 0),)


class WeightView(NamedTuple):
    tensor: torch.Tensor
    offset: int
# ... 574 lines not shown

_GLU_KERNELS = {
    "bsed_glu16_fwd": (L.CONSTANTS["BSED_GLU_16_FWD"], False, "glu16_fwd_kernel"),
    "bsed_glu16_bwd": (L.CONSTANTS["BSED_GLU_16_BWD"], False, "glu16_bwd_kernel"),
    "bsed_block0_fwd": (L.CONSTANTS["BSED_GLU_BLOCK0_FWD"], False, "b0_fwd_kernel<{ph}, {small}, {ab}>"),
    "bsed_block0_bwd": (L.CONSTANTS["BSED_GLU_BLOCK0_BWD"], False, "b0_bwd_kernel<{ph}, {small}, {ab}>"),
    "bsed_glu_bwd_fused": (L.CONSTANTS["BSED_GLU_BWD_FUSED"], True, "glu_bwd_fused_kernel<{C}, {v}>"),
    "bsed_glu_fwd3": (L.CONSTANTS["BSED_GLU_FWD3"], True, "glu_fwd3_kernel<{C}, {v}, {ab}>"),
    "bsed_glu_bwd3": (L.CONSTANTS["BSED_GLU_BWD3"], True, "glu_bwd3_kernel<{C}, {v}, {ab}>"),
    "bsed_glu_bwd3n": (L.CONSTANTS["BSED_GLU_BWD3N"], True, "glu_bwd3n_kernel<{ab}>"),
}
_GLU_ACTIVATIONS = ("y", "dpool", "pooled", "g", "dlin")
_GLU_PARAMETERS = ("cw", "cb", "w", "bias")


def _glu_plan(entry, d):
    plan = GluPlan()
    L.check(L.lib().bsed_glu_plan(ctypes.byref(d), _GLU_KERNELS[entry][0], ctypes.byref(plan)), entry)
    d.G = plan.G
    return plan


def _glu_label(entry, d, plan):
    v = plan.variant
    return _GLU_KERNELS[entry][2].format(C=d.C, v=v, ph=v & 15, small="true" if v >> 4 else "false", ab=d.act_bf16)


def _glu_desc(entry, NB, H, W, C, pool, drop_p, rng_stream, seed, **tensors):
    d = GluDesc(NB=NB, H=H, W=W, C=C, ph=pool[0], pw=pool[1], drop_p=drop_p, rng_stream=rng_stream, seed=seed,
                act_bf16=_abf(*(tensors.get(n) for n in _GLU_ACTIVATIONS)))
    if _GLU_KERNELS[entry][1]:
        d.TH, d.TW = tile_for(W)
    for name, t in tensors.items():
        setattr(d, name, _pa(t) if name in _GLU_ACTIVATIONS else _dp(t) if name in _GLU_PARAMETERS else L.ptr(t))
    return d, _glu_plan(entry, d)


def _glu_launch(entry, d, plan, flops, nbytes):
    if L.timer is not None:
        label = _glu_label(entry, d, plan)
        if _GLU_KERNELS[entry][1]:
            return _launch((label, 1, d.C, d.C, d.H, d.W), flops, lambda: L.call(entry, ctypes.byref(d), L.stream()), nbytes)
        _note(label, f"{d.H}x{d.W}", flops, nbytes)
    L.call(entry, ctypes.byref(d), L.stream())


def _glu_partials(plan, C, dev):
    return (torch.empty((plan.dw_rows, C, C), device=dev, dtype=torch.float32),
            torch.empty((plan.G, 2, C), device=dev, dtype=torch.float32),
            torch.empty((plan.G, 2, C), device=dev, dtype=torch.float32))


def glu16_fwd(y, scale, shift, wg, bg, B, H, W, pool, drop_p, rng_stream, seed):
    ph, pw = pool
    out = torch.empty((B, H // ph, W // pw, 16), device=y.device, dtype=torch.float32)
    d, plan = _glu_desc("bsed_glu16_fwd", B, H, W, 16, pool, drop_p, rng_stream, seed, y=y, scale=scale,
                        shift=shift, w=wg, bias=bg, pooled=out)
    _glu_launch("bsed_glu16_fwd", d, plan, 2.0 * B * H * W * 256, 4.0 * B * H * W * 16 * (1.0 + 1.0 / (ph * pw)))
    return out


def glu16_bwd(y, scale, shift, wg, bg, dpool, B, H, W, pool, drop_p, rng_stream, seed):
    ph, pw = pool
    g = torch.empty_like(y)
    d, plan = _glu_desc("bsed_glu16_bwd", B, H, W, 16, pool, drop_p, rng_stream, seed, y=y, scale=scale,
                        shift=shift, w=wg, bias=bg, dpool=dpool, g=g)
    part_dw, part_db, part_st = _glu_partials(plan, 16, y.device)
    d.part_dw, d.part_db, d.part_st = L.ptr(part_dw), L.ptr(part_db), L.ptr(part_st)
    _glu_launch("bsed_glu16_bwd", d, plan, 3 * 2.0 * B * H * W * 256,
                4.0 * B * H * W * 16 * (2.0 + 1.0 / (ph * pw)))
    return g, part_dw, part_db, part_st, plan.G


def block0_stats(x, cw, cb, NB, H, W):
    G = int(min(2048, max(1, (NB * H * W) // 256)))
    dev = x.device
    stats = torch.empty((G, 2, 16), device=dev, dtype=torch.float32)
    xr_part = torch.empty((G, 54), device=dev, dtype=torch.float32)
    xr64 = torch.empty(54, device=dev, dtype=torch.float64)
    _note("b0_stats_kernel", f"{H}x{W}", 2.0 * NB * H * W * (9 * 16 + 16 + 54), 4.0 * NB * H * W)
    cwt = cw.detach().reshape(16, 9).t().contiguous()
    L.call("bsed_block0_stats", L.ptr(x), L.ptr(cwt), _dp(cb), L.ptr(stats), L.ptr(xr_part),
           L.ptr(xr64, torch.float64), G, NB, H, W, 16, L.stream())
    return stats, xr64


def block0_fwd(x, cw, cb, scale, shift, wg, bg, B, H, W, pool, drop_p, rng_stream, seed, out_dtype=torch.float32):
    ph, pw = pool
    out = torch.empty((B, H // ph, W // pw, 16), device=x.device, dtype=out_dtype)
    d, plan = _glu_desc("bsed_block0_fwd", B, H, W, 16, pool, drop_p, rng_stream, seed, x=x, cw=cw, cb=cb,
                        scale=scale, shift=shift, w=wg, bias=bg, pooled=out)
    _glu_launch("bsed_block0_fwd", d, plan, 2.0 * B * H * W * (9 * 16 + 256),
                B * H * W * (4.0 + _esz(out) * 16.0 / (ph * pw)))
    return out


def block0_bwd(x, cw, cb, scale, shift, wg, bg, dpool, B, H, W, pool, drop_p, rng_stream, seed):
    ph, pw = pool
    d, plan = _glu_desc("bsed_block0_bwd", B, H, W, 16, pool, drop_p, rng_stream, seed, x=x, cw=cw, cb=cb,
                        scale=scale, shift=shift, w=wg, bias=bg, dpool=dpool)
    part_dw, part_db, part_st = _glu_partials(plan, 16, x.device)
    part_gx = torch.empty((plan.G, 9, 16), device=x.device, dtype=torch.float32)
    d.part_dw, d.part_db, d.part_st, d.part_gx = L.ptr(part_dw), L.ptr(part_db), L.ptr(part_st), L.ptr(part_gx)
    _glu_launch("bsed_block0_bwd", d, plan, 2.0 * B * H * W * (2 * 9 * 16 + 3 * 256),
                B * H * W * (4.0 + _esz(dpool) * 16.0 / (ph * pw)))
    return part_dw, part_db, part_st, part_gx, plan.G


def block0_wgrad_finish(part_gx, G, xr64, coef, mean, cw, cb, dst, accumulate=True):
    _note("b0_wgrad_finish_kernel", f"G{G}", float(part_gx.numel()), 4.0 * part_gx.numel())
    L.call("bsed_block0_wgrad_finish", L.ptr(part_gx), G, L.ptr(xr64, torch.float64), L.ptr(coef), L.ptr(mean),
           _dp(cw), _dp(cb), _dp(dst), 1 if accumulate else 0, 16, L.stream())


def _glu_bwd_tiled(entry, esz, y, dpool, B, H, W, C, pool, drop_p, rng_stream, seed, **weights):
    g = torch.empty_like(y)
    d, plan = _glu_desc(entry, B, H, W, C, pool, drop_p, rng_stream, seed, y=y, dpool=dpool, g=g, **weights)
    part_dw, part_db, part_st = _glu_partials(plan, C, y.device)
    d.part_dw, d.part_db, d.part_st = L.ptr(part_dw), L.ptr(part_db), L.ptr(part_st)
    _glu_launch(entry, d, plan, 3 * 2.0 * B * H * W * C * C,
                esz * B * H * W * C * (2.0 + 1.0 / (pool[0] * pool[1])))
    return g, part_dw, part_db, part_st, plan.G, plan.dw_rows // plan.G


def glu_bwd_fused(y, scale, shift, wfwd, w, bias, dpool, B, H, W, C, pool, drop_p, rng_stream, seed):
    return _glu_bwd_tiled("bsed_glu_bwd_fused", 4.0, y, dpool, B, H, W, C, pool, drop_p, rng_stream, seed,
                          scale=scale, shift=shift, wfwd=wfwd, w=w, bias=bias)


def glu_fwd3_supported(W, C, pool):
    TH, TW = tile_for(W)
    return (C in (32, 64, 128) and (pool[1] == 1 or TW >= 2) and
            (pool[0] == 1 or ((TW in (2, 8, 16) or (TW == 1 and pool[1] == 1)) and TH % 2 == 0)))


def glu_fwd3(y, scale, shift, w, bias, B, H, W, C, pool, drop_p, rng_stream, seed):
    ph, pw = pool
    out = torch.empty((B, H // ph, W // pw, C), device=y.device, dtype=y.dtype)
    d, plan = _glu_desc("bsed_glu_fwd3", B, H, W, C, pool, drop_p, rng_stream, seed, y=y, scale=scale, shift=shift,
                        w=w, bias=bias, pooled=out)
    _glu_launch("bsed_glu_fwd3", d, plan, 2.0 * B * H * W * C * C,
                _esz(y) * B * H * W * C * (1.0 + 1.0 / (ph * pw)))
    return out


def glu_bwd3(y, scale, shift, w, bias, dpool, B, H, W, C, pool, drop_p, rng_stream, seed):
    return _glu_bwd_tiled("bsed_glu_bwd3", _esz(y), y, dpool, B, H, W, C, pool, drop_p, rng_stream, seed,
                          scale=scale, shift=shift, w=w, bias=bias)


_frag_tables = {}


def glu_bwd3n(y, scale, shift, w, bias, dpool, B, H, W, C, pool, drop_p, rng_stream, seed):
    dev = y.device
    g = torch.empty_like(y)
    dlin = torch.empty_like(y)
    d, plan = _glu_desc("bsed_glu_bwd3n", B, H, W, C, pool, drop_p, rng_stream, seed, y=y, scale=scale,
                        shift=shift, w=w, bias=bias, dpool=dpool, g=g, dlin=dlin)
    tb = _frag_tables.get(str(dev))
    if tb is None:
        tb = _frag_tables[str(dev)] = torch.empty(plan.table_bytes, device=dev, dtype=torch.uint8)
    part_db = torch.empty((plan.G, 2, C), device=dev, dtype=torch.float32)
    part_st = torch.empty((plan.G, 2, C), device=dev, dtype=torch.float32)
    d.part_db, d.part_st, d.frag_table = L.ptr(part_db), L.ptr(part_st), tb.data_ptr()
    _glu_launch("bsed_glu_bwd3n", d, plan, 2 * 2.0 * B * H * W * C * C,
                _esz(y) * B * H * W * C * (3.0 + 1.0 / (pool[0] * pool[1])))
    return g, dlin, part_db, part_st, plan.G


def glu_route(direction, C, W, pool, mode, fused=True):
    if mode not in ("fp32", "bf16x3", "bf16"):
        raise L.BsedError(f"glu_route: unknown mode {mode!r}")
    if direction not in ("forward", "backward"):
        raise L.BsedError(f"glu_route: unknown direction {direction!r}")
    if C == 16:
        return "glu16"
    if direction == "forward":
        if mode != "fp32" and glu_fwd3_supported(W, C, pool):
            return "glu3"
        return "igemm"
    if C in (32, 64) and fused and mode != "fp32":
        return "glu3"
    if C == 128 and fused and mode != "fp32":
        return "glu3n"
    if C in (32, 64, 128) and fused:
        return "fused_fp32"
    return "unfused"


def glu_forward(y, scale, shift, w, bias, B, H, W, C, pool, drop_p, rng_stream, seed, *, mode):
    route = glu_route("forward", C, W, pool, mode)
    if route == "glu16":
        return glu16_fwd(y, scale, shift, w, bias, B, H, W, pool, drop_p, rng_stream, seed)
    if route == "glu3":
        return glu_fwd3(y, scale, shift, w, bias, B, H, W, C, pool, drop_p, rng_stream, seed)
    wg = pack_weight(w, 1, C, C, 0, 1, C)
    return igemm(y, wg, C, B, H, W, C, bias=bias, epilogue=EPI_GLU_POOL, a_scale=scale, a_shift=shift, e_src=y,
                 e_scale=scale, e_shift=shift, pool=pool, drop_p=drop_p, rng_stream=rng_stream, seed=seed)[0]


def glu_backward(y, scale, shift, w, bias, dpool, B, H, W, C, pool, drop_p, rng_stream, seed, *, mode, fused, dw, db):
    route = glu_route("backward", C, W, pool, mode, fused)
    dpool = dpool.contiguous()
    tail = (pool, drop_p, rng_stream, seed)
    if route in ("glu3n", "unfused"):
        if route == "glu3n":
            g, dlin, pdb, st2, _ = glu_bwd3n(y, scale, shift, w, bias, dpool, B, H, W, C, *tail)
        else:
            tt = torch.empty_like(y)
            dlin, pdb = igemm(y, pack_weight(w, 1, C, C, 0, 1, C), C, B, H, W, C, bias=bias, epilogue=EPI_GLU_BWD,
                              a_scale=scale, a_shift=shift, e_src=y, e_scale=scale, e_shift=shift, e_dpool=dpool,
                              out2=tt, pool=pool, drop_p=drop_p, rng_stream=rng_stream, seed=seed)
        stats_to_grad(pdb, C, 0, db)
        weight_grad(y, dlin, linear_weight(dw), B, H, W, a_scale=scale, a_shift=shift, mode=mode)
        if route == "unfused":
            g, st2 = igemm(dlin, pack_weight(w, 1, C, C, 0, C, 1), C, B, H, W, C, epilogue=EPI_ADD_STATS2, out=tt,
                           out2=tt, e_src=y)
        return g, st2
    if route == "glu16":
        g, pdw, pdb, st2, G = glu16_bwd(y, scale, shift, w, bias, dpool, B, H, W, *tail)
        slabs = 1
    elif route == "glu3":
        g, pdw, pdb, st2, G, slabs = glu_bwd3(y, scale, shift, w, bias, dpool, B, H, W, C, *tail)
    else:
        wfwd = pack_weight(w, 1, C, C, 0, 1, C)
        g, pdw, pdb, st2, G, slabs = glu_bwd_fused(y, scale, shift, wfwd, w, bias, dpool, B, H, W, C, *tail)
    reduce_partials(pdw, G * slabs, 1, C, C, C, C, dw, 0, C, 1)
    stats_to_grad(pdb, C, 0, db)
    return g, st2


def bn_finalize(stats, C, count, eps, momentum, gamma, beta, rmean, rvar, nbt):
    dev = stats.device
    mean, invstd, scale, shift = (torch.empty(C, device=dev, dtype=torch.float32) for _ in range(4))
    _note("stats_chunk_kernel+stats_finish_kernel", f"C{C}", 0.0, 4.0 * stats.numel())
    L.call("bsed_bn_finalize", L.ptr(stats), stats.shape[0], C, count, eps, momentum, _dp(gamma), _dp(beta), _dp(rmean),
           _dp(rvar), _dp(nbt), L.ptr(mean), L.ptr(invstd), L.ptr(scale),
           L.ptr(shift), L.ptr(stats_scratch(C, dev), torch.float64), L.stream())
    return mean, invstd, scale, shift


def bn_eval(C, eps, gamma, beta, rmean, rvar):
    dev = gamma.device
    scale, shift = (torch.empty(C, device=dev, dtype=torch.float32) for _ in range(2))
    L.call("bsed_bn_eval", C, eps, _dp(gamma), _dp(beta), _dp(rmean), _dp(rvar), L.ptr(scale), L.ptr(shift),
           L.stream())
    return scale, shift


def bn_eval_batch(layers, eps):
    dev = layers[0][1].device
    out = torch.empty(2 * sum(l[0] for l in layers), device=dev, dtype=torch.float32)
    arr = (BnEvalJob * len(layers))()
    res, off = [], 0
    for a, (C, gamma, beta, rmean, rvar) in zip(arr, layers):
        scale, shift = out[off:off + C], out[off + C:off + 2 * C]
        off += 2 * C
        a.gamma, a.beta, a.running_mean, a.running_var = _dp(gamma), _dp(beta), _dp(rmean), _dp(rvar)
        a.scale, a.shift, a.C = scale.data_ptr(), shift.data_ptr(), C
        res.append((scale, shift))
    _note("bn_eval_batch_kernel", "", 0.0, 4.0 * 3 * out.numel())
    L.call("bsed_bn_eval_batch", arr, len(layers), eps, L.stream())
    return res


def bn_bwd(stats, C, count, gamma, mean, invstd, dgamma, dbeta, g_inout, y, apply=True):
    dev = stats.device
    coef = torch.empty((3, C), device=dev, dtype=torch.float32)
    _note("bn_bwd_apply_kernel" if apply else "stats_chunk_kernel+stats_finish_kernel", f"C{C}", 3.0 * y.numel() if apply else 0.0,
          12.0 * y.numel() if apply else 4.0 * stats.numel())
    L.call("bsed_bn_bwd", L.ptr(stats), stats.shape[0], C, count, _dp(gamma), L.ptr(mean), L.ptr(invstd), _dp(dgamma),
           _dp(dbeta), 1,
           L.ptr(g_inout) if apply else None, L.ptr(y) if apply else None,
           y.numel() if apply else C, L.ptr(coef), L.ptr(stats_scratch(C, dev), torch.float64),
           L.stream())
    return coef


def stats_to_grad(stats, C, which, dst):
    if _rq is not None and _rq["stream"] == L.stream().value and which == 0 and stats.dim() == 3 and stats.shape[1] == 2:
        _rq["jobs"].append((stats, _dp(dst), stats.shape[0], 1, 2, C, 1, C, 0, 0, 1, 1))
        return
    _note("stats_chunk_kernel+stats_finish_kernel", f"C{C}", 0.0, 4.0 * stats.numel())
    L.call("bsed_stats_to_grad", L.ptr(stats), stats.shape[0], C, which, _dp(dst), 1,
           L.ptr(stats_scratch(C, stats.device), torch.float64), L.stream())


def colsum(inp, M, C, pitch, dst, accumulate=True, in_offset=0):
    G = int(min(512, M))
    part = torch.empty((G, 2, C), device=inp.device, dtype=torch.float32)
    _note("colsum_kernel", f"C{C}", float(M) * C, 4.0 * M * C)
    if _rq is not None and _rq["stream"] == L.stream().value:
        L.call("bsed_colsum_part", _dp(inp, in_offset), M, C, pitch, L.ptr(part), G,
               L.stream())
        _rq["jobs"].append((part, _dp(dst), G, 1, 2, C, 1, C, 0, 0, 1, 1 if accumulate else 0))
        return
    L.call("bsed_colsum", _dp(inp, in_offset), M, C, pitch, L.ptr(part), G,
           _dp(dst), 1 if accumulate else 0, L.ptr(stats_scratch(C, inp.device), torch.float64), L.stream())


def dropout(x, p, rng_stream, seed):
    out = torch.empty_like(x)
    _note("dropout_kernel", "", float(x.numel()), 8.0 * x.numel())
    L.call("bsed_dropout", L.ptr(x), L.ptr(out), x.numel(), p, rng_stream, seed, L.stream())
    return out


def gru_rows(B):
    return 1 if B * 2 <= 256 else 2


def gru_fwd(xp, w_hh, b_hh, B, T, save_gates, mode="fp32"):
    out = torch.empty((B, T, 256), device=xp.device, dtype=torch.float32)
    gates = torch.empty((B, T, 2, 4, 128), device=xp.device, dtype=torch.float32) if save_gates else None
    _note("gru_fwd_mfma_kernel<true>" if mode == "bf16x3" else "gru_fwd_kernel", f"T{T}", 2.0 * B * T * 2 * 128 * 384,
          4.0 * B * T * (768 + 256 + (1024 if save_gates else 0)))
    if mode == "bf16x3":
        L.call("bsed_gru_fwd3", L.ptr(xp), _dp(w_hh), _dp(b_hh), L.ptr(out), _p(gates), B, T,
               L.stream())
    else:
        L.call("bsed_gru_fwd", L.ptr(xp), _dp(w_hh), _dp(b_hh), L.ptr(out), _p(gates), B, T, gru_rows(B),
               L.stream())
    return out, gates


def gru_bwd(dout, out, gates, w_hh, B, T, mode="fp32"):
    dxp = torch.empty((B, T, 768), device=dout.device, dtype=torch.float32)
    dgh = torch.empty((B, T, 768), device=dout.device, dtype=torch.float32)
    _note("gru_bwd_mfma_kernel" if mode == "bf16x3" else "gru_bwd_kernel", f"T{T}", 2.0 * B * T * 2 * 128 * 384,
          4.0 * B * T * (256 + 256 + 1024 + 768 + 768))
    if mode == "bf16x3":
        rows = L.lib().bsed_gru_bwd3_rows(B)
        pih = torch.empty((rows, 768), device=dout.device, dtype=torch.float32)
        phh = torch.empty((rows, 768), device=dout.device, dtype=torch.float32)
        L.call("bsed_gru_bwd3", L.ptr(dout), L.ptr(out), L.ptr(gates), _dp(w_hh), L.ptr(dxp), L.ptr(dgh),
               L.ptr(pih), L.ptr(phh), B, T, L.stream())
        return dxp, dgh, pih, phh
    else:
        L.call("bsed_gru_bwd", L.ptr(dout), L.ptr(out), L.ptr(gates), _dp(w_hh), L.ptr(dxp), L.ptr(dgh), B, T,
               gru_rows(B), L.stream())
    return dxp, dgh, None, None


def max_over_time(y):
    y = y.contiguous().float()
    B, T, C = y.shape
    out = torch.empty((B, C), device=y.device, dtype=torch.float32)
    _note("max_over_time_kernel", f"T{T}", 0.0, 4.0 * (y.numel() + out.numel()))
    L.call("bsed_max_over_time", L.ptr(y), L.ptr(out), B, T, C, L.stream())
    return out


def _head_kernel(direction, C):
    if C == 20:
        return f"head_{direction}_kernel<20>"
    return f"head_{direction}_n_kernel<{(2 * C + 31) // 32},{'lds' if C <= 32 else 'l2'}>"


def head_fwd(x, w, b, B, T, K, C, attention):
    dev = x.device
    strong = torch.empty((B, T, C), device=dev, dtype=torch.float32)
    sof = torch.empty((B, T, C), device=dev, dtype=torch.float32)
    weak = torch.empty((B, C), device=dev, dtype=torch.float32)
    den = torch.empty((B, C), device=dev, dtype=torch.float32)
    S = L.lib().bsed_head_splits(B, T)
    part = torch.empty((B, S, 2, C), device=dev, dtype=torch.float32) if S > 1 else None
# ... 130 lines not shown
```

### include/bsed.h

```cpp
#ifndef BSED_H
#define BSED_H
#include <stddef.h>
#include <stdint.h>

#ifdef __cplusplus
extern "C" {
#endif

const char* bsed_last_error(void);
const char* bsed_build_info(void);
int bsed_abi_version(void);

typedef struct BsedMelCfg {
  int sr;
  int n_fft;
  int hop;
  int n_mels;
  float fmin;
  float fmax;
} BsedMelCfg;

int bsed_mel_plan_create(const BsedMelCfg* cfg , void** plan );
int bsed_mel_plan_destroy(void* plan);
int bsed_mel_plan_nnz(const void* plan);
int bsed_mel_plan_frames_per_wave(const void* plan);
int bsed_mel_num_frames(const void* plan, int n_samples);
long bsed_mel_scratch_floats(const void* plan, int B, int n_samples);
int bsed_mel_linear(const void* plan, const float* wav, int B, int n_samples, float* mel_lin,
                    float* clip_max, float* bin_sumsq, float* scratch, void* stream);
int bsed_mel_stats(const float* mel_lin, int B, int T, int n_mels, float* clip_max, float* bin_sumsq, void* stream);
int bsed_mel_noise(const float* mel_lin, const float* bin_sumsq, const float* unit_noise, int B, int T,
                   int n_mels, float snr_db, uint64_t seed, float* noisy, float* clip_max_noisy,
                   void* stream);
int bsed_mel_db(const float* mel_lin, const float* clip_max, int B, int T, int T_out, int n_mels,
                float top_db, float* out_db, void* stream);
int bsed_mel_db_views(const float* mel_lin, const float* clip_max, int B, int T, int T_out, int n_mels,
                      float top_db, const int* shift_frames, const int* shift_bins, float* out_db,
                      float* out_db_tshift, float* out_db_fshift, void* stream);

long bsed_scaler_scratch_doubles(int B, int T, int T_out, int n_mels);
int bsed_scaler_accum(const float* mel_lin, const float* clip_max, int B, int T, int T_out, int n_mels,
                      float top_db, double* acc, double* scratch, void* stream);
int bsed_scaler_accum_db(const float* x_db, int B, int T_out, int n_mels, double* acc, double* scratch,
                         void* stream);
int bsed_scaler_normalize(const float* x_db, long long n_rows, int n_mels, const double* mean, const double* stdev,
                          float* out, void* stream);
int bsed_mel_db_norm(const float* mel_lin, const float* clip_max, int B, int T, int T_out, int n_mels,
                     float top_db, const double* mean, const double* stdev, float* out_db, void* stream);
int bsed_mel_db_views_norm(const float* mel_lin, const float* clip_max, int B, int T, int T_out, int n_mels,
                           float top_db, const int* shift_frames, const int* shift_bins, const double* mean,
                           const double* stdev, float* out_db, float* out_db_tshift, float* out_db_fshift,
                           void* stream);

enum {
  BSED_EPI_PLAIN = 0,
  BSED_EPI_STATS = 1,
  BSED_EPI_GLU_POOL = 2,
  BSED_EPI_GLU_BWD = 3,
  BSED_EPI_ADD_STATS2 = 4
};

typedef struct BsedIgemmDesc {
  const float* in;
  const float* w;
  const float* bias;
  float* out;
  float* out2;
  float* stats;
  const float* a_scale;
  const float* a_shift;
  const float* e_src;
  const float* e_scale;
  const float* e_shift;
  const float* e_dpool;
  int in_pitch, out_pitch, e_pitch;
  int NB, H, W, CIN, N, NP;
  int TH, TW;
  int tilesH, tilesW;
  int hh, hw;
  int ntaps, dh[9], dw[9];
  int ph, pw, Hp, Wp;
  int epilogue;
  float drop_p;
  uint32_t rng_stream;
  uint64_t seed;
  int valid_h, valid_w;
  int act_bf16;
  int G;
} BsedIgemmDesc;

enum { BSED_CONTRACT_IGEMM = 0, BSED_CONTRACT_IGEMM3 = 1, BSED_CONTRACT_IGEMM3S = 2, BSED_CONTRACT_IGEMM3N = 3,
       BSED_CONTRACT_WGRAD = 4, BSED_CONTRACT_WGRAD3 = 5 };
typedef struct BsedContractPlan {
  int G;
  int max_G;
  int stats_rows;
  char label[96];
} BsedContractPlan;
int bsed_igemm_plan(const BsedIgemmDesc* desc , int kernel , BsedContractPlan* out );

int bsed_igemm(const BsedIgemmDesc* desc , void* stream);

int bsed_igemm3(const BsedIgemmDesc* desc , void* stream);
int bsed_pack_weight3(const float* src, void* dst, int ntaps, int K, int N, int NP, long s_tap, long s_k, long s_n,
                      void* stream);
int bsed_pack_weight3s(const float* src, void* dst, int ntaps, int K, int N, int NP, long s_tap, long s_k, long s_n,
                       void* stream);
#define BSED_PACK_MAX_JOBS 32
typedef struct BsedPackJob {
  const float* src; void* dst;
  int kind, ntaps, K, N, NP;
  long s_tap, s_k, s_n;
} BsedPackJob;
int bsed_pack_weights_batch(const BsedPackJob* jobs , int njobs, void* stream);
int bsed_igemm3s(const BsedIgemmDesc* desc , void* stream);
int bsed_igemm3n(const BsedIgemmDesc* desc , void* stream);
void bsed_igemm3n_set_wpe(int knob);
void bsed_igemm3n_set_shape(int shape);

typedef struct BsedWgradDesc {
  const float* in;
  const float* dy;
  float* part;
  const float* a_scale;
  const float* a_shift;
  int in_pitch, dy_pitch;
  int NB, H, W, CIN, CINP, N, NP, G;
  int TH, TW, tilesH, tilesW, hh, hw;
  int ntaps, dh[9], dw[9];
  const float* bn_y;
  const float* bn_coef;
  const float* bn_mean;
  float* dy_out;
  int act_bf16;
  const void* w3s;
  float* d_in;
  int din_pitch;
} BsedWgradDesc;

int bsed_wgrad_plan(const BsedWgradDesc* desc , int kernel , BsedContractPlan* out );
int bsed_wgrad(const BsedWgradDesc* desc , void* stream);
int bsed_wgrad3(const BsedWgradDesc* desc , void* stream);
int bsed_conv_bwd_plan(const BsedWgradDesc* desc , BsedContractPlan* out );
int bsed_conv_bwd3(const BsedWgradDesc* desc , void* stream);
int bsed_reduce_partials(const float* part, int G, int ntaps, int KP, int NP, int K, int N, float* dst,
                         long s_tap, long s_k, long s_n, int accumulate, void* stream);
#define BSED_REDUCE_MAX_JOBS 40
typedef struct BsedReduceJob {
  const float* part; float* dst;
  int G, ntaps, KP, NP, K, N, accumulate;
  long s_tap, s_k, s_n;
} BsedReduceJob;
int bsed_reduce_partials_batch(const BsedReduceJob* jobs , int njobs, void* stream);
int bsed_pack_weight(const float* src, float* dst, int ntaps, int K, int N, int NP, long s_tap, long s_k,
                     long s_n, void* stream);

int bsed_conv0_fwd(const float* x, const float* w, const float* bias, float* y, float* stats, int NB, int H,
                   int W, int CO, void* stream);
int bsed_conv0_num_tiles(int NB, int H, int W);
int bsed_conv0_wgrad(const float* x, const float* dy, const float* y, const float* coef, const float* mean,
                     float* part, int G, int NB, int H, int W, int CO, void* stream);
size_t bsed_stats_scratch_bytes(int C);
int bsed_bn_finalize(const float* partial, long ntiles, int C, double count, float eps, float momentum,
                     const float* gamma, const float* beta, float* running_mean, float* running_var,
                     long long* num_batches_tracked, float* mean, float* invstd, float* scale, float* shift,
                     void* scratch, void* stream);
int bsed_bn_eval(int C, float eps, const float* gamma, const float* beta, const float* running_mean,
                 const float* running_var, float* scale, float* shift, void* stream);
#define BSED_BN_EVAL_MAX_JOBS 16
typedef struct BsedBnEvalJob {
  const float *gamma, *beta, *running_mean, *running_var;
  float *scale, *shift;
  int C;
} BsedBnEvalJob;
int bsed_bn_eval_batch(const BsedBnEvalJob* jobs , int njobs, float eps, void* stream);
int bsed_bn_bwd(const float* partial, long ntiles, int C, double count, const float* gamma, const float* mean,
                const float* invstd, float* dgamma, float* dbeta, int accumulate, float* g_inout, const float* y,
                long n_elems, float* coef, void* scratch, void* stream);
int bsed_stats_to_grad(const float* partial, long ntiles, int C, int which, float* dst, int accumulate,
                       void* scratch, void* stream);
int bsed_colsum(const float* in, long M, int C, int pitch, float* part, int G, float* dst, int accumulate,
                void* scratch, void* stream);
int bsed_colsum_part(const float* in, long M, int C, int pitch, float* part, int G, void* stream);
int bsed_dropout(const float* in, float* out, long n, float p, uint32_t rng_stream, uint64_t seed, void* stream);

typedef struct BsedGluDesc {
  const float* x;
  const float* y;
  const float *cw, *cb;
  const float *scale, *shift;
  const float* w;
  const float* wfwd;
  const float* bias;
  const float* dpool;
  float* pooled;
  float* g;
  float* dlin;
  float* part_dw;
  float *part_db, *part_st;
  float* part_gx;
  void* frag_table;
  int NB, H, W, C;
  int TH, TW;
  int ph, pw;
  float drop_p;
  uint32_t rng_stream;
  uint64_t seed;
  int act_bf16;
  int G;
} BsedGluDesc;

enum {
  BSED_GLU_16_FWD = 0, BSED_GLU_16_BWD = 1, BSED_GLU_BLOCK0_FWD = 2, BSED_GLU_BLOCK0_BWD = 3,
  BSED_GLU_BWD_FUSED = 4, BSED_GLU_FWD3 = 5, BSED_GLU_BWD3 = 6, BSED_GLU_BWD3N = 7
};
typedef struct BsedGluPlan {
  int G;
  int max_G;
  int dw_rows;
  int variant;
  size_t table_bytes;
} BsedGluPlan;
int bsed_glu_plan(const BsedGluDesc* desc , int kernel, BsedGluPlan* out);

int bsed_glu16_fwd(const BsedGluDesc* desc , void* stream);
int bsed_glu16_bwd(const BsedGluDesc* desc , void* stream);

int bsed_block0_stats(const float* x, const float* cw_t ,
                      const float* cb, float* stats, float* xr_part, double* xr64,
                      int G, int NB, int H, int W, int CO, void* stream);
int bsed_block0_fwd(const BsedGluDesc* desc , void* stream);
int bsed_block0_bwd(const BsedGluDesc* desc , void* stream);
int bsed_block0_wgrad_finish(const float* part_gx, int G, const double* xr64, const float* coef, const float* mean,
                             const float* cw, const float* cb, float* dst, int accumulate, int CO, void* stream);

int bsed_glu_bwd_fused(const BsedGluDesc* desc , void* stream);
int bsed_glu_bwd3(const BsedGluDesc* desc , void* stream);
int bsed_glu_bwd3n(const BsedGluDesc* desc , void* stream);
int bsed_glu_fwd3(const BsedGluDesc* desc , void* stream);

int bsed_leaky_dropout_fwd(const float* a, float* out, long n, float slope, float drop_p, uint32_t rng_stream,
                           uint64_t seed, void* stream);
int bsed_leaky_dropout_bwd(const float* d_out, const float* a, float* d_a, long n, float slope, float drop_p,
                           uint32_t rng_stream, uint64_t seed, void* stream);
int bsed_frame_head_fwd(const float* x, const float* w, const float* b, float* d, long M, int K, void* stream);
int bsed_frame_head_bwd(const float* x, const float* w, const float* d, const float* d_out, float* dx, float* part, int G,
                        long M, int K, void* stream);

int bsed_s2d_fwd(const float* y, const float* scale, const float* shift, float* xp, int N, int Ha, int Wa, int Hi, int Wi,
                 int C, void* stream);
int bsed_s2d_num_blocks(int N, int Ha, int Wa, int C);
int bsed_s2d_bwd(const float* dxp, const float* y, const float* scale, const float* shift, float* g, float* stats, int N,
                 int Ha, int Wa, int Hi, int Wi, int C, void* stream);

int bsed_im2col_s2(const float* act, const float* scale, const float* shift, float* col, int N, int Hi, int Wi,
                   int C, int CP, void* stream);
int bsed_col2im_s2(const float* dcol, const float* y, const float* scale, const float* shift, float* out,
                   float* stats, int N, int Hi, int Wi, int C, int CP, float out_scale, void* stream);
int bsed_col2im_s2_num_blocks(int N, int Hi, int Wi, int C);
int bsed_disc_head(const float* y5, const float* scale, const float* shift, const float* wl, const float* bl, int N,
                   int Ns, int H5, int W5, int C5, int train, float* d_out, float* g5, float* stats, float* dwl_part,
                   float* dbl_part, float* loss_part, void* stream);

int bsed_upsample_time_fwd(const float* in, float* out, int B, int T_in, int T_out, int C, int in_pitch, int out_pitch,
                           void* stream);
int bsed_upsample_time_bwd(const float* dout, float* din, int B, int T_in, int T_out, int C, int dout_pitch,
                           int din_pitch, void* stream);

int bsed_gru_fwd(const float* xp, const float* w_hh, const float* b_hh, float* out, float* gates, int B, int T,
                 int rows_per_wg, void* stream);
int bsed_gru_bwd(const float* dout, const float* out, const float* gates, const float* w_hh, float* dxp,
                 float* dgh, int B, int T, int rows_per_wg, void* stream);
int bsed_gru_fwd3(const float* xp, const float* w_hh, const float* b_hh, float* out, float* gates, int B, int T,
                  void* stream);
int bsed_gru_bwd3(const float* dout, const float* out, const float* gates, const float* w_hh, float* dxp,
                  float* dgh, float* part_bih, float* part_bhh, int B, int T, void* stream);
int bsed_gru_bwd3_rows(int B);

int bsed_max_over_time(const float* y, float* out, int B, int T, int C, void* stream);
int bsed_head_splits(int B, int T);
#define BSED_HEAD_MAX_CLASSES 64
int bsed_head_lds_bytes(int C, int backward);
int bsed_head_fwd(const float* x, const float* w, const float* b, float* strong, float* sof_raw, float* weak,
                  float* den, float* part, int B, int T, int K, int C, int attention, void* stream);

int bsed_tag_splits(int B, int T);
int bsed_tag_head_fwd(const float* x, const float* logits, float* strong, float* weak, float* part, int B, int T, int C,
// ... 103 lines not shown
```

Baseline: 21820 clips/s.

## Recompute GLU d_lin inside the 1x1 weight-gradient kernel instead of storing it

Adds a GLU-aware wgrad path (wgrad1g) that forms d_lin on load from y, dpool, BN scale/shift and the dropout hash, so the GLU backward kernel can skip writing the d_lin tensor. It also adds a glu_bwd3k variant compiled without the d_lin store. The aim is to remove one full activation-sized write plus the matching read of d_lin. In exchange the wgrad kernel redoes the sigmoid and dropout arithmetic and gains new constraints (C=128, 1x1 tap only).

```diff
diff --git a/bird-sound-event-detecion_amd/csrc/bsed_common.h b/bird-sound-event-detecion_amd/csrc/bsed_common.h
--- a/bird-sound-event-detecion_amd/csrc/bsed_common.h
+++ b/bird-sound-event-detecion_amd/csrc/bsed_common.h
@@ -386,6 +386,10 @@
   const uint32_t h = mix32((uint32_t)e * 0x9E3779B1u + key + (uint32_t)(e >> 32) * 0x85ebca6bu);
   return (h >> 8) >= thr ? scale : 0.f;
 }
+__device__ __forceinline__ float drop_mul32(uint32_t e, uint32_t key, uint32_t thr, float scale) {
+  const uint32_t h = mix32(e * 0x9E3779B1u + key);
+  return (h >> 8) >= thr ? scale : 0.f;
+}
 
 __device__ __forceinline__ uint32_t drop_threshold16(float p) { return (uint32_t)(p * 65536.0f); }
 __device__ __forceinline__ void drop_mul2(uint64_t e_even, uint32_t key, uint32_t thr16, float scale, float& m0,
diff --git a/bird-sound-event-detecion_amd/csrc/capi.hip b/bird-sound-event-detecion_amd/csrc/capi.hip
--- a/bird-sound-event-detecion_amd/csrc/capi.hip
+++ b/bird-sound-event-detecion_amd/csrc/capi.hip
@@ -14,7 +14,7 @@
 extern "C" const char* bsed_last_error(void) { return g_err; }
 extern "C" const char* bsed_build_info(void) { return "libbsed gfx950: fp32 storage/accumulation, split-fp32 (bf16x3) contractions on v_mfma_f32_32x32x16_bf16 by default, "
          "exact-fp32 v_mfma_f32_32x32x2_f32 kernels selectable (hand-written HIP)"; }
-extern "C" int bsed_abi_version(void) { return 15; }
+extern "C" int bsed_abi_version(void) { return 16; }
 
 extern "C" int bsed_glu_plan(const BsedGluDesc* desc, int kernel, BsedGluPlan* out) {
   BSED_CHECK_ARG(desc && out, "bsed_glu_plan: null argument");
diff --git a/bird-sound-event-detecion_amd/csrc/glu3.hip b/bird-sound-event-detecion_amd/csrc/glu3.hip
--- a/bird-sound-event-detecion_amd/csrc/glu3.hip
+++ b/bird-sound-event-detecion_amd/csrc/glu3.hip
@@ -117,11 +117,6 @@
 }
 
 __device__ float g3_sink[G3_M];
-
-__device__ __forceinline__ float drop_mul32(uint32_t e, uint32_t key, uint32_t thr, float scale) {
-  const uint32_t h = mix32(e * 0x9E3779B1u + key);
-  return (h >> 8) >= thr ? scale : 0.f;
-}
 
 #define G3_B32_WPE 3
 template <int C, int LGTW, int ABF>
@@ -382,201 +377,16 @@
 }
 
 #define G3N_THREADS 512
-template <int ABF>
-__global__ __launch_bounds__(G3N_THREADS) void glu_bwd3n_kernel(const Glu3Params P, const bf16x8* __restrict__ table,
-                                                                float* __restrict__ dlin) {
-  constexpr int C = 128, NT = 4, KS = 8;
-#ifdef G3N_LGTW
-  constexpr int g3n_lgTW = G3N_LGTW, g3n_TW = 1 << G3N_LGTW;
-#else
-  const int g3n_lgTW = P.lgTW, g3n_TW = P.TW;
-#endif
-  constexpr int DQ = 2 * 16 + 8;
-  extern __shared__ __align__(16) unsigned char smem_raw[];
-  bf16x8* WF = reinterpret_cast<bf16x8*>(smem_raw);
-  bf16x8* WB = WF + NT * KS * 2 * 64;
-  float* s_sc = reinterpret_cast<float*>(WB + NT * KS * 2 * 64);
-  float* s_sh = s_sc + C;
-  unsigned short* Dall = reinterpret_cast<unsigned short*>(s_sh + C);
-  const int tid = threadIdx.x, wave8 = __builtin_amdgcn_readfirstlane(tid >> 6), lane = tid & 63, li = lane & 31, lh = lane >> 5;
-  const int wave = wave8 & 3, half = wave8 >> 2;
-  unsigned short* D = Dall + wave8 * 32 * DQ;
-
-  for (int i = tid; i < 2 * NT * KS * 2 * 64; i += G3N_THREADS) WF[i] = table[i];
-  for (int i = tid; i < C; i += G3N_THREADS) { s_sc[i] = P.scale[i]; s_sh[i] = P.shift[i]; }
-  __syncthreads();
-
-  const int sph = P.ph >> 1, spw = P.pw >> 1;
-  const float inv_pool = 1.0f / (float)(P.ph * P.pw);
-  const uint32_t dkey = drop_key(P.rng_stream, P.seed + (P.seed_add ? *P.seed_add : 0)), dthr = drop_threshold(P.drop_p);
-  const float dscale = P.drop_p > 0.f ? 1.0f / (1.0f - P.drop_p) : 1.0f;
-
-  float bias[NT], csc[NT], csh[NT], sdb[NT], sgs[NT], sgy[NT];
-#pragma unroll
-  for (int j = 0; j < NT; ++j) {
-    bias[j] = P.bias[32 * j + li];
-    csc[j] = s_sc[32 * j + li]; csh[j] = s_sh[32 * j + li];
-    sdb[j] = 0.f; sgs[j] = 0.f; sgy[j] = 0.f;
-  }
-
-  for (int tile0 = 2 * blockIdx.x + half; tile0 < P.ntiles; tile0 += 2 * gridDim.x) {
-    int tile = tile0;
-    const int tw_i = tile % P.tilesW; tile /= P.tilesW;
-    const int th_i = tile % P.tilesH;
-    const int nb = tile / P.tilesH;
-    const int th0 = th_i * P.TH, tw0 = tw_i * P.TW;
-    int lhv = 4 * lh;
-    asm volatile("" : "+v"(lhv));
-
-    f32x16 acc[NT];
-    {
-      bf16x8 a_hi[KS], a_lo[KS];
-      load_a_frags<C, ABF>(P, g3n_lgTW, s_sc, s_sh, nb, th0, tw0, wave, li, lh, a_hi, a_lo);
-#pragma unroll
-      for (int j = 0; j < NT; ++j)
-#pragma unroll
-        for (int r = 0; r < 16; ++r) acc[j][r] = 0.f;
-#pragma unroll
-      for (int ks = 0; ks < KS; ++ks)
-#pragma unroll
-        for (int j = 0; j < NT; ++j) {
-          const bf16x8 b_hi = WF[((j * KS + ks) * 2 + 0) * 64 + lane];
-          const bf16x8 b_lo = WF[((j * KS + ks) * 2 + 1) * 64 + lane];
-          acc[j] = mfma_sp<ABF>(a_hi[ks], a_lo[ks], b_hi, b_lo, acc[j]);
-        }
-    }
-
-    uint32_t dph[NT][8], dpl[NT][8];
-#pragma unroll
-    for (int rg = 0; rg < 4; ++rg) {
-      uint32_t dvr[4][NT], yvr[4][NT];
-      float mk[4];
-      uint32_t posv[4];
-      float* dlrow[4];
-      uint32_t dlidx[4];
-#pragma unroll
-      for (int rr = 0; rr < 4; ++rr) {
-        const int mm = wave * 32 + 8 * rg + lhv + rr;
-        const int gh = th0 + (mm >> g3n_lgTW), gw = tw0 + (mm & (g3n_TW - 1));
-        const int gph = gh >> sph, gpw = gw >> spw;
-        mk[rr] = (gh < P.H && gph < P.Hp && gpw < P.Wp) ? inv_pool : 0.f;
-        posv[rr] = ((uint32_t)(nb * P.H + min(gh, P.H - 1)) * (uint32_t)P.W + gw) * C + li;
-        dlrow[rr] = gh < P.H ? dlin : g3_sink;
-        dlidx[rr] = gh < P.H ? posv[rr] : (uint32_t)li;
-        const uint32_t dpo = ((uint32_t)(nb * P.Hp + min(gph, P.Hp - 1)) * (uint32_t)P.Wp + min(gpw, P.Wp - 1)) * C + li;
-#pragma unroll
-        for (int j = 0; j < NT; ++j) {
-          dvr[rr][j] = act_ld_raw<ABF>(P.dpool, dpo + 32 * j);
-          yvr[rr][j] = act_ld_raw<ABF>(P.y, posv[rr] + 32 * j);
-        }
-      }
-      __builtin_amdgcn_sched_barrier(0);
-#pragma unroll
-      for (int rp = 0; rp < 2; ++rp)
-#pragma unroll
-        for (int j = 0; j < NT; ++j) {
-          float dl2[2];
-#pragma unroll
-          for (int e = 0; e < 2; ++e) {
-            const int rr = 2 * rp + e, r = 4 * rg + rr;
-            const float xn = fmaf(act_cvt<ABF>(yvr[rr][j]), csc[j], csh[j]);
-            const float sg = sigmoid_fast(xn);
-            const float lin = acc[j][r] + bias[j];
-            const float dres = act_cvt<ABF>(dvr[rr][j]) * mk[rr] * drop_mul32(posv[rr] + 32 * j, dkey, dthr, dscale);
-            const float dl = dres * sg;
-            acc[j][r] = dres * lin * sg * (1.0f - sg);
-            sdb[j] += dl;
-            act_st<ABF>(dlrow[rr], dlidx[rr] + 32 * j, dl);
-            dl2[e] = dl;
-          }
-          split_pack2(dl2[0], dl2[1], dph[j][2 * rg + rp], dpl[j][2 * rg + rp]);
-        }
-    }
-
-    acc_handoff_fence<NT>(acc);
-#pragma unroll
-    for (int q = 0; q < 8; ++q) {
-      if ((li >> 4) == (q & 1)) {
-#pragma unroll
-        for (int i = 0; i < 8; ++i) {
-          const int r = 2 * i;
-          const int row = 8 * (r >> 2) + lhv + (r & 3);
-          D[row * DQ + (li & 15)] = (unsigned short)(dph[q >> 1][i] & 0xFFFFu);
-          D[(row + 1) * DQ + (li & 15)] = (unsigned short)(dph[q >> 1][i] >> 16);
-          D[row * DQ + 16 + (li & 15)] = (unsigned short)(dpl[q >> 1][i] & 0xFFFFu);
-          D[(row + 1) * DQ + 16 + (li & 15)] = (unsigned short)(dpl[q >> 1][i] >> 16);
-        }
-      }
-      wave_lds_fence();
-      const bf16x8 d_hi = *reinterpret_cast<const bf16x8*>(D + li * DQ + 8 * lh);
-      const bf16x8 d_lo = *reinterpret_cast<const bf16x8*>(D + li * DQ + 16 + 8 * lh);
-#pragma unroll
-      for (int j = 0; j < NT; ++j) {
-        const bf16x8 b_hi = WB[((j * KS + q) * 2 + 0) * 64 + lane];
-        const bf16x8 b_lo = WB[((j * KS + q) * 2 + 1) * 64 + lane];
-        acc[j] = mfma_sp<ABF>(d_hi, d_lo, b_hi, b_lo, acc[j]);
-      }
-      wave_lds_fence();
-    }
-
-#pragma unroll
-    for (int rg = 0; rg < 4; ++rg) {
-      uint32_t yvr[4][NT];
-      float okf[4];
-      uint32_t posv[4];
-      float* gdst[4];
-      uint32_t gidx[4];
-#pragma unroll
-      for (int rr = 0; rr < 4; ++rr) {
-        const int mm = wave * 32 + 8 * rg + lhv + rr;
-        const int gh = th0 + (mm >> g3n_lgTW), gw = tw0 + (mm & (g3n_TW - 1));
-        okf[rr] = gh < P.H ? 1.0f : 0.0f;
-        posv[rr] = ((uint32_t)(nb * P.H + min(gh, P.H - 1)) * (uint32_t)P.W + gw) * C + li;
-        gdst[rr] = gh < P.H ? P.g : g3_sink;
-        gidx[rr] = gh < P.H ? posv[rr] : (uint32_t)li;
-#pragma unroll
-        for (int j = 0; j < NT; ++j) yvr[rr][j] = act_ld_raw<ABF>(P.y, posv[rr] + 32 * j);
-      }
-      __builtin_amdgcn_sched_barrier(0);
-#pragma unroll
-      for (int rr = 0; rr < 4; ++rr)
-#pragma unroll
-        for (int j = 0; j < NT; ++j) {
-          const float gv = acc[j][4 * rg + rr] * okf[rr];
-          act_st<ABF>(gdst[rr], gidx[rr] + 32 * j, gv);
-          sgs[j] += gv;
-          sgy[j] = fmaf(gv, act_cvt<ABF>(yvr[rr][j]), sgy[j]);
-        }
-    }
-  }
-
-  __syncthreads();
-  float* red = reinterpret_cast<float*>(Dall);
-#pragma unroll
-  for (int j = 0; j < NT; ++j) {
-    const float a = sdb[j] + __shfl_xor(sdb[j], 32, 64);
-    const float b = sgs[j] + __shfl_xor(sgs[j], 32, 64);
-    const float c = sgy[j] + __shfl_xor(sgy[j], 32, 64);
-    if (lh == 0) {
-      red[(wave8 * 3 + 0) * C + 32 * j + li] = a;
-      red[(wave8 * 3 + 1) * C + 32 * j + li] = b;
-      red[(wave8 * 3 + 2) * C + 32 * j + li] = c;
-    }
-  }
-  __syncthreads();
-  for (int e = tid; e < 3 * C; e += G3N_THREADS) {
-    const int which = e / C, n = e % C;
-    float s = 0.f;
-#pragma unroll
-    for (int wv = 0; wv < 8; ++wv) s += red[(wv * 3 + which) * C + n];
-    if (which == 0) {
-      P.part_db[((size_t)blockIdx.x * 2 + 0) * C + n] = s;
-      P.part_db[((size_t)blockIdx.x * 2 + 1) * C + n] = 0.f;
-    } else {
-      P.part_st[((size_t)blockIdx.x * 2 + (which - 1)) * C + n] = s;
-    }
-  }
-}
+#define G3N_KERNEL glu_bwd3n_kernel
+#define G3N_DLIN 1
+#include "glu3n_body.h"
+#undef G3N_KERNEL
+#undef G3N_DLIN
+#define G3N_KERNEL glu_bwd3k_kernel
+#define G3N_DLIN 0
+#include "glu3n_body.h"
+#undef G3N_KERNEL
+#undef G3N_DLIN
 
 template <int C, int LGTW, int ABF>
 __global__ __launch_bounds__(G3_THREADS, 2) void glu_fwd3_kernel(const Glu3Params P) {
@@ -820,11 +630,24 @@
   return launch_glu_fwd3<32, 0>(P, G, ctw, s);
 }
 
+template <int ABF>
+static int launch_glu_bwd3n(const Glu3Params& P, const void* frag_table, float* dlin, int G, size_t smem, hipStream_t s) {
+  static BsedLdsOnce once, oncek;
+  if (dlin) {
+    BSED_HIP(bsed_max_lds(once, (const void*)glu_bwd3n_kernel<ABF>));
+    hipLaunchKernelGGL(glu_bwd3n_kernel<ABF>, dim3(G), dim3(G3N_THREADS), smem, s, P, (const bf16x8*)frag_table, dlin);
+  } else {
+    BSED_HIP(bsed_max_lds(oncek, (const void*)glu_bwd3k_kernel<ABF>));
+    hipLaunchKernelGGL(glu_bwd3k_kernel<ABF>, dim3(G), dim3(G3N_THREADS), smem, s, P, (const bf16x8*)frag_table, dlin);
+  }
+  BSED_LAUNCH_CHECK();
+  return BSED_OK;
+}
 extern "C" int bsed_glu_bwd3n(const BsedGluDesc* desc, void* stream) {
   Glu3Params P;
   BsedGluPlan plan;
-  const int rc = bsed_glu_geometry(P, desc, BSED_GLU_BWD3N,
-                                   GLU_Y | GLU_LIN | GLU_DPOOL | GLU_G | GLU_DLIN | GLU_PART_B | GLU_FRAG, plan);
+  const int rc = bsed_glu_geometry(P, desc, BSED_GLU_BWD3N, GLU_Y | GLU_LIN | GLU_DPOOL | GLU_G | GLU_PART_B | GLU_FRAG |
+                                   (desc && desc->dlin ? GLU_DLIN : 0), plan);
   if (rc) return rc;
   P.w = desc->w; P.pooled = nullptr;
   void* frag_table = desc->frag_table;
@@ -833,14 +656,6 @@
   hipStream_t s = (hipStream_t)stream;
   hipLaunchKernelGGL(glu3_pack_frags_kernel, dim3(4 * 8 * 64 / 256), dim3(256), 0, s, P.w, (bf16x8*)frag_table);
   const size_t smem = plan.table_bytes + 2 * 128 * sizeof(float) + (size_t)8 * 32 * (2 * 16 + 8) * 2;
-  static BsedLdsOnce once, onceb;
-  if (desc->act_bf16) {
-    BSED_HIP(bsed_max_lds(onceb, (const void*)glu_bwd3n_kernel<1>));
-    hipLaunchKernelGGL(glu_bwd3n_kernel<1>, dim3(G), dim3(G3N_THREADS), smem, s, P, (const bf16x8*)frag_table, dlin);
-  } else {
-    BSED_HIP(bsed_max_lds(once, (const void*)glu_bwd3n_kernel<0>));
-    hipLaunchKernelGGL(glu_bwd3n_kernel<0>, dim3(G), dim3(G3N_THREADS), smem, s, P, (const bf16x8*)frag_table, dlin);
-  }
-  BSED_LAUNCH_CHECK();
-  return BSED_OK;
-}
+  return desc->act_bf16 ? launch_glu_bwd3n<1>(P, frag_table, dlin, G, smem, s)
+                        : launch_glu_bwd3n<0>(P, frag_table, dlin, G, smem, s);
+}
diff --git a/bird-sound-event-detecion_amd/csrc/glu3n_body.h b/bird-sound-event-detecion_amd/csrc/glu3n_body.h
--- /dev/null
+++ b/bird-sound-event-detecion_amd/csrc/glu3n_body.h
@@ -0,0 +1,203 @@
+template <int ABF>
+__global__ __launch_bounds__(G3N_THREADS) void G3N_KERNEL(const Glu3Params P, const bf16x8* __restrict__ table,
+                                                          float* __restrict__ dlin) {
+  constexpr int C = 128, NT = 4, KS = 8;
+#ifdef G3N_LGTW
+  constexpr int g3n_lgTW = G3N_LGTW, g3n_TW = 1 << G3N_LGTW;
+#else
+  const int g3n_lgTW = P.lgTW, g3n_TW = P.TW;
+#endif
+  constexpr int DQ = 2 * 16 + 8;
+  extern __shared__ __align__(16) unsigned char smem_raw[];
+  bf16x8* WF = reinterpret_cast<bf16x8*>(smem_raw);
+  bf16x8* WB = WF + NT * KS * 2 * 64;
+  float* s_sc = reinterpret_cast<float*>(WB + NT * KS * 2 * 64);
+  float* s_sh = s_sc + C;
+  unsigned short* Dall = reinterpret_cast<unsigned short*>(s_sh + C);
+  const int tid = threadIdx.x, wave8 = __builtin_amdgcn_readfirstlane(tid >> 6), lane = tid & 63, li = lane & 31, lh = lane >> 5;
+  const int wave = wave8 & 3, half = wave8 >> 2;
+  unsigned short* D = Dall + wave8 * 32 * DQ;
+
+  for (int i = tid; i < 2 * NT * KS * 2 * 64; i += G3N_THREADS) WF[i] = table[i];
+  for (int i = tid; i < C; i += G3N_THREADS) { s_sc[i] = P.scale[i]; s_sh[i] = P.shift[i]; }
+  __syncthreads();
+
+  const int sph = P.ph >> 1, spw = P.pw >> 1;
+  const float inv_pool = 1.0f / (float)(P.ph * P.pw);
+  const uint32_t dkey = drop_key(P.rng_stream, P.seed + (P.seed_add ? *P.seed_add : 0)), dthr = drop_threshold(P.drop_p);
+  const float dscale = P.drop_p > 0.f ? 1.0f / (1.0f - P.drop_p) : 1.0f;
+
+  float bias[NT], csc[NT], csh[NT], sdb[NT], sgs[NT], sgy[NT];
+#pragma unroll
+  for (int j = 0; j < NT; ++j) {
+    bias[j] = P.bias[32 * j + li];
+    csc[j] = s_sc[32 * j + li]; csh[j] = s_sh[32 * j + li];
+    sdb[j] = 0.f; sgs[j] = 0.f; sgy[j] = 0.f;
+  }
+
+  for (int tile0 = 2 * blockIdx.x + half; tile0 < P.ntiles; tile0 += 2 * gridDim.x) {
+    int tile = tile0;
+    const int tw_i = tile % P.tilesW; tile /= P.tilesW;
+    const int th_i = tile % P.tilesH;
+    const int nb = tile / P.tilesH;
+    const int th0 = th_i * P.TH, tw0 = tw_i * P.TW;
+    int lhv = 4 * lh;
+    asm volatile("" : "+v"(lhv));
+
+    f32x16 acc[NT];
+    {
+      bf16x8 a_hi[KS], a_lo[KS];
+      load_a_frags<C, ABF>(P, g3n_lgTW, s_sc, s_sh, nb, th0, tw0, wave, li, lh, a_hi, a_lo);
+#pragma unroll
+      for (int j = 0; j < NT; ++j)
+#pragma unroll
+        for (int r = 0; r < 16; ++r) acc[j][r] = 0.f;
+#pragma unroll
+      for (int ks = 0; ks < KS; ++ks)
+#pragma unroll
+        for (int j = 0; j < NT; ++j) {
+          const bf16x8 b_hi = WF[((j * KS + ks) * 2 + 0) * 64 + lane];
+          const bf16x8 b_lo = WF[((j * KS + ks) * 2 + 1) * 64 + lane];
+          acc[j] = mfma_sp<ABF>(a_hi[ks], a_lo[ks], b_hi, b_lo, acc[j]);
+        }
+    }
+
+    uint32_t dph[NT][8], dpl[NT][8];
+#pragma unroll
+    for (int rg = 0; rg < 4; ++rg) {
+      uint32_t dvr[4][NT], yvr[4][NT];
+      float mk[4];
+      uint32_t posv[4];
+#if G3N_DLIN
+      float* dlrow[4];
+      uint32_t dlidx[4];
+#endif
+#pragma unroll
+      for (int rr = 0; rr < 4; ++rr) {
+        const int mm = wave * 32 + 8 * rg + lhv + rr;
+        const int gh = th0 + (mm >> g3n_lgTW), gw = tw0 + (mm & (g3n_TW - 1));
+        const int gph = gh >> sph, gpw = gw >> spw;
+        mk[rr] = (gh < P.H && gph < P.Hp && gpw < P.Wp) ? inv_pool : 0.f;
+        posv[rr] = ((uint32_t)(nb * P.H + min(gh, P.H - 1)) * (uint32_t)P.W + gw) * C + li;
+#if G3N_DLIN
+        dlrow[rr] = gh < P.H ? dlin : g3_sink;
+        dlidx[rr] = gh < P.H ? posv[rr] : (uint32_t)li;
+#endif
+        const uint32_t dpo = ((uint32_t)(nb * P.Hp + min(gph, P.Hp - 1)) * (uint32_t)P.Wp + min(gpw, P.Wp - 1)) * C + li;
+#pragma unroll
+        for (int j = 0; j < NT; ++j) {
+          dvr[rr][j] = act_ld_raw<ABF>(P.dpool, dpo + 32 * j);
+          yvr[rr][j] = act_ld_raw<ABF>(P.y, posv[rr] + 32 * j);
+        }
+      }
+      __builtin_amdgcn_sched_barrier(0);
+#pragma unroll
+      for (int rp = 0; rp < 2; ++rp)
+#pragma unroll
+        for (int j = 0; j < NT; ++j) {
+          float dl2[2];
+#pragma unroll
+          for (int e = 0; e < 2; ++e) {
+            const int rr = 2 * rp + e, r = 4 * rg + rr;
+            const float xn = fmaf(act_cvt<ABF>(yvr[rr][j]), csc[j], csh[j]);
+            const float sg = sigmoid_fast(xn);
+            const float lin = acc[j][r] + bias[j];
+            const float dres = act_cvt<ABF>(dvr[rr][j]) * mk[rr] * drop_mul32(posv[rr] + 32 * j, dkey, dthr, dscale);
+            const float dl = dres * sg;
+            acc[j][r] = dres * lin * sg * (1.0f - sg);
+            sdb[j] += dl;
+#if G3N_DLIN
+            act_st<ABF>(dlrow[rr], dlidx[rr] + 32 * j, dl);
+#else
+            asm volatile("" :: "v"(dl));
+#endif
+            dl2[e] = dl;
+          }
+          split_pack2(dl2[0], dl2[1], dph[j][2 * rg + rp], dpl[j][2 * rg + rp]);
+        }
+    }
+
+    acc_handoff_fence<NT>(acc);
+#pragma unroll
+    for (int q = 0; q < 8; ++q) {
+      if ((li >> 4) == (q & 1)) {
+#pragma unroll
+        for (int i = 0; i < 8; ++i) {
+          const int r = 2 * i;
+          const int row = 8 * (r >> 2) + lhv + (r & 3);
+          D[row * DQ + (li & 15)] = (unsigned short)(dph[q >> 1][i] & 0xFFFFu);
+          D[(row + 1) * DQ + (li & 15)] = (unsigned short)(dph[q >> 1][i] >> 16);
+          D[row * DQ + 16 + (li & 15)] = (unsigned short)(dpl[q >> 1][i] & 0xFFFFu);
+          D[(row + 1) * DQ + 16 + (li & 15)] = (unsigned short)(dpl[q >> 1][i] >> 16);
+        }
+      }
+      wave_lds_fence();
+      const bf16x8 d_hi = *reinterpret_cast<const bf16x8*>(D + li * DQ + 8 * lh);
+      const bf16x8 d_lo = *reinterpret_cast<const bf16x8*>(D + li * DQ + 16 + 8 * lh);
+#pragma unroll
+      for (int j = 0; j < NT; ++j) {
+        const bf16x8 b_hi = WB[((j * KS + q) * 2 + 0) * 64 + lane];
+        const bf16x8 b_lo = WB[((j * KS + q) * 2 + 1) * 64 + lane];
+        acc[j] = mfma_sp<ABF>(d_hi, d_lo, b_hi, b_lo, acc[j]);
+      }
+      wave_lds_fence();
+    }
+
+#pragma unroll
+    for (int rg = 0; rg < 4; ++rg) {
+      uint32_t yvr[4][NT];
+      float okf[4];
+      uint32_t posv[4];
+      float* gdst[4];
+      uint32_t gidx[4];
+#pragma unroll
+      for (int rr = 0; rr < 4; ++rr) {
+        const int mm = wave * 32 + 8 * rg + lhv + rr;
+        const int gh = th0 + (mm >> g3n_lgTW), gw = tw0 + (mm & (g3n_TW - 1));
+        okf[rr] = gh < P.H ? 1.0f : 0.0f;
+        posv[rr] = ((uint32_t)(nb * P.H + min(gh, P.H - 1)) * (uint32_t)P.W + gw) * C + li;
+        gdst[rr] = gh < P.H ? P.g : g3_sink;
+        gidx[rr] = gh < P.H ? posv[rr] : (uint32_t)li;
+#pragma unroll
+        for (int j = 0; j < NT; ++j) yvr[rr][j] = act_ld_raw<ABF>(P.y, posv[rr] + 32 * j);
+      }
+      __builtin_amdgcn_sched_barrier(0);
+#pragma unroll
+      for (int rr = 0; rr < 4; ++rr)
+#pragma unroll
+        for (int j = 0; j < NT; ++j) {
+          const float gv = acc[j][4 * rg + rr] * okf[rr];
+          act_st<ABF>(gdst[rr], gidx[rr] + 32 * j, gv);
+          sgs[j] += gv;
+          sgy[j] = fmaf(gv, act_cvt<ABF>(yvr[rr][j]), sgy[j]);
+        }
+    }
+  }
+
+  __syncthreads();
+  float* red = reinterpret_cast<float*>(Dall);
+#pragma unroll
+  for (int j = 0; j < NT; ++j) {
+    const float a = sdb[j] + __shfl_xor(sdb[j], 32, 64);
+    const float b = sgs[j] + __shfl_xor(sgs[j], 32, 64);
+    const float c = sgy[j] + __shfl_xor(sgy[j], 32, 64);
+    if (lh == 0) {
+      red[(wave8 * 3 + 0) * C + 32 * j + li] = a;
+      red[(wave8 * 3 + 1) * C + 32 * j + li] = b;
+      red[(wave8 * 3 + 2) * C + 32 * j + li] = c;
+    }
+  }
+  __syncthreads();
+  for (int e = tid; e < 3 * C; e += G3N_THREADS) {
+    const int which = e / C, n = e % C;
+    float s = 0.f;
+#pragma unroll
+    for (int wv = 0; wv < 8; ++wv) s += red[(wv * 3 + which) * C + n];
+    if (which == 0) {
+      P.part_db[((size_t)blockIdx.x * 2 + 0) * C + n] = s;
+      P.part_db[((size_t)blockIdx.x * 2 + 1) * C + n] = 0.f;
+    } else {
+      P.part_st[((size_t)blockIdx.x * 2 + (which - 1)) * C + n] = s;
+    }
+  }
+}
diff --git a/bird-sound-event-detecion_amd/csrc/wgrad.hip b/bird-sound-event-detecion_amd/csrc/wgrad.hip
--- a/bird-sound-event-detecion_amd/csrc/wgrad.hip
+++ b/bird-sound-event-detecion_amd/csrc/wgrad.hip
@@ -4,12 +4,6 @@
 
 #define W3_DY_BYTES (2 * IG_TILE_M * 32 * 2)
 
-struct WgradParams {
-  BsedWgradDesc d;
-  int PW, PH, PP, lgTW, dy_off, ntiles, nct, ntw;
-  int CC, lgc4, pw_magic;
-  int pack2;
-};
 
 template <int MAXS, int NW>
 __global__ __launch_bounds__(NW * 64) void wgrad_kernel(const WgradParams P) {
@@ -342,13 +336,6 @@
     }
   }
 }
-
-#define W1_TP 64
-#define W1_THREADS 512
-#define W1_PLANE (W1_TP * 128 * 2)
-#define W1_STAGE (4 * W1_PLANE)
-
-struct W1Set { float4 x[4], d[4]; };
 
 template <bool SHIFT, int ABF>
 __global__ __launch_bounds__(W1_THREADS) __attribute__((amdgpu_waves_per_eu(2, 2))) void wgrad1_kernel(const WgradParams P) {
@@ -868,7 +855,7 @@
   if (P.ntiles < 0) return P.ntiles;
   BSED_CHECK_ARG(d.N % 4 == 0, "bsed_wgrad: N must be a multiple of 4");
   BSED_CHECK_ARG(d.CINP % 32 == 0 && d.CINP >= d.CIN, "bsed_wgrad: bad padding");
-  BSED_CHECK_ARG(d.dy_pitch >= d.N && d.dy_pitch % 4 == 0, "bsed_wgrad: bad pitch");
+  BSED_CHECK_ARG(d.glu || (d.dy_pitch >= d.N && d.dy_pitch % 4 == 0), "bsed_wgrad: bad pitch");
   BSED_CHECK_ARG((d.bn_y == nullptr) == (d.bn_coef == nullptr) && (d.bn_y == nullptr) == (d.bn_mean == nullptr),
                  "bsed_wgrad: bn_y, bn_coef and bn_mean come together (BatchNorm backward applied on load) or not at all");
   BSED_CHECK_ARG(d.bn_y || !d.dy_out, "bsed_wgrad: dy_out only goes with bn_y");
@@ -987,13 +974,14 @@
          (long)d.NB * d.H * d.W < (1L << 31) - 4 * 65536;
 }
 
-enum W3Kind { W3_TILE, W3_PIPE, W3_STREAM1 };
+enum W3Kind { W3_TILE, W3_PIPE, W3_STREAM1, W3_STREAM1G };
 struct W3Plan {
   W3Kind kind;
   int maxs, nw, geo;
   bool bs, shifted;
 };
 static W3Plan wgrad3_plan(const WgradParams& P, size_t smem) {
+  if (wgrad1_streaming(P) && P.d.glu && bsed_wgrad1g_takes(P)) return {W3_STREAM1G, 0, 0, 0, false, false};
   if (wgrad1_streaming(P)) return {W3_STREAM1, 0, 0, 0, false, P.d.dh[0] != 0 || P.d.dw[0] != 0};
   const int v = wgrad_variant(P), maxs = v / 16, nw = v % 16;
   if (wgrad3_pipelined(P, smem)) {
@@ -1044,6 +1032,7 @@
 }
 
 static int wgrad3_dispatch(const WgradParams& P, const W3Plan& pl, const BsedLaunch& L) {
+  if (pl.kind == W3_STREAM1G) return bsed_launch_wgrad1g(P, L);
   if (pl.kind == W3_STREAM1) return pl.shifted ? launch_wgrad1<true>(P, L) : launch_wgrad1<false>(P, L);
   if (pl.kind == W3_PIPE) return launch_wgrad3p(pl, P, L);
   if (pl.nw == 8) {
@@ -1056,6 +1045,11 @@
   if (pl.maxs == 3) return launch_wgrad3_tile<3, 4>(pl, P, L);
   if (pl.maxs == 5) return launch_wgrad3_tile<5, 4>(pl, P, L);
   return launch_wgrad3_tile<9, 4>(pl, P, L);
+}
+
+static bool wgrad1g_recommended(const WgradParams& P) {
+  (void)P;
+  return false;
 }
 
 int bsed_run_wgrad(const BsedWgradDesc* desc, int mode3, void* stream, BsedContractPlan* plan) {
@@ -1065,12 +1059,25 @@
   const int rc = wgrad_prepare(desc, P, smem, gyz, mode3);
   if (rc != BSED_OK) return rc;
   const BsedWgradDesc& d = P.d;
+  const char* who = mode3 ? "bsed_wgrad3" : "bsed_wgrad";
+  if (d.glu) {
+    BSED_CHECK_ARG(mode3, "bsed_wgrad: glu (d_lin formed on load) is built into bsed_wgrad3's streaming kernel only");
+    const int rg = bsed_wgrad1g_check(P, who);
+    if (rg != BSED_OK) return rg;
+  }
   const W3Plan pl = mode3 ? wgrad3_plan(P, smem) : W3Plan{};
   BsedLaunch L;
-  if (plan) L = bsed_plan_begin(plan, mode3 ? wgrad3_auto_g(P, pl, smem, gyz) : wgrad_auto_g(P, smem, gyz), P.ntiles, 0);
-  else {
-    const char* who = mode3 ? "bsed_wgrad3" : "bsed_wgrad";
-    BSED_CHECK_ARG(d.in && d.dy && d.part, "%s: null tensor", who);
+  if (plan) {
+    int G = mode3 ? wgrad3_auto_g(P, pl, smem, gyz) : wgrad_auto_g(P, smem, gyz);
+    if (d.glu && !(pl.kind == W3_STREAM1G && wgrad1g_recommended(P))) G = 0;
+    L = bsed_plan_begin(plan, G, P.ntiles, 0);
+    if (d.glu) return bsed_launch_wgrad1g(P, L);
+  } else {
+    BSED_CHECK_ARG(d.in && d.part && (d.dy || d.glu), d.in && d.part ? "%s: null tensor dy (or glu: the inputs dy is formed from)"
+                                                                     : "%s: null tensor", who);
+    BSED_CHECK_ARG(!d.glu || d.glu->dpool, "%s: null tensor glu->dpool", who);
+    BSED_CHECK_ARG(!d.glu || pl.kind == W3_STREAM1G, "%s: glu: the streaming kernel does not take this shape (NB*H*W*128 must "
+                   "stay below 2^32): keep d_lin", who);
     BSED_CHECK_ARG(d.G > 0 && d.G <= P.ntiles, "%s: G (%d) must be in 1..%d tiles", who, d.G, P.ntiles);
     L = BsedLaunch{dim3((unsigned)d.G, gyz.y, gyz.z), smem, (hipStream_t)stream, nullptr};
   }
diff --git a/bird-sound-event-detecion_amd/csrc/wgrad_glu.hip b/bird-sound-event-detecion_amd/csrc/wgrad_glu.hip
--- /dev/null
+++ b/bird-sound-event-detecion_amd/csrc/wgrad_glu.hip
@@ -0,0 +1,204 @@
+#include "wgrad_tiles.h"
+
+struct W1Div { uint32_t mul; int sh; };
+static W1Div w1_div(uint32_t d) {
+  if (d == 1) return W1Div{0u, 0};
+  int s = 1;
+  while ((1u << s) < d) ++s;
+  return W1Div{(uint32_t)(((1ull << (31 + s)) + d - 1) / d), s - 1};
+}
+__device__ __forceinline__ int w1_quot(int n, const W1Div& dv) {
+  return dv.mul ? (int)(__umulhi((uint32_t)n, dv.mul) >> dv.sh) : n;
+}
+
+struct W1Glu {
+  const float* dpool;
+  int ph, pw, Hp, Wp;
+  float drop_p; uint32_t rng_stream; uint64_t seed;
+  const uint64_t* seed_add;
+  W1Div by_hw, by_w;
+};
+
+template <bool FLAT, int ABF>
+__global__ __launch_bounds__(W1_THREADS) __attribute__((amdgpu_waves_per_eu(2, 2))) void wgrad1g_kernel(const WgradParams P,
+                                                                                                       const W1Glu Gl) {
+  const BsedWgradDesc& p = P.d;
+  extern __shared__ __align__(16) uint32_t smw[];
+  const int tid = threadIdx.x, wave = tid >> 6, lane = tid & 63, li = lane & 31, lh = lane >> 5;
+  const int HW = p.H * p.W, M = p.NB * HW;
+  const int ntile = (M + W1_TP - 1) / W1_TP;
+  const int cit = wave & 3, nt0 = wave >> 2;
+  const int gq = (lane >> 2) & 3, gc = 4 * (lane & 3), gh = (lane >> 4) & 1;
+  const uint32_t base = (uint32_t)(uintptr_t)smw;
+  uint32_t xa[2], xb[2][2];
+#pragma unroll
+  for (int rd = 0; rd < 2; ++rd) {
+    const int mk = 8 * lh + 4 * rd + gq;
+    xa[rd] = base + 2 * (mk * 128 + (w3_chunk(cit, mk, 4) << 5) + 16 * gh + gc);
+#pragma unroll
+    for (int s = 0; s < 2; ++s)
+      xb[s][rd] = base + 2 * W1_PLANE + 2 * (mk * 128 + (w3_chunk(nt0 + 2 * s, mk, 4) << 5) + 16 * gh + gc);
+  }
+  f32x16 acc[2];
+#pragma unroll
+  for (int s = 0; s < 2; ++s)
+#pragma unroll
+    for (int r = 0; r < 16; ++r) acc[s][r] = 0.f;
+
+  const int c4 = tid & 31, p0 = tid >> 5;
+  const float* xsrc = p.in + 4 * c4;
+  const float* dsrc = Gl.dpool + 4 * c4;
+  const float4 sc = *reinterpret_cast<const float4*>(p.a_scale + 4 * c4);
+  const float4 sh = *reinterpret_cast<const float4*>(p.a_shift + 4 * c4);
+  const int so = p0 * 128 + (w3_chunk(c4 >> 3, p0, 4) << 5) + 4 * (c4 & 7);
+  w3_lds_u16* lds = (w3_lds_u16*)smw;
+
+  const int sph = Gl.ph >> 1, spw = Gl.pw >> 1;
+  const float inv_pool = 1.0f / (float)(Gl.ph * Gl.pw);
+  const uint32_t dkey = drop_key(Gl.rng_stream, Gl.seed + (Gl.seed_add ? *Gl.seed_add : 0)), dthr = drop_threshold(Gl.drop_p);
+  const float dscale = Gl.drop_p > 0.f ? 1.0f / (1.0f - Gl.drop_p) : 1.0f;
+
+  auto issue = [&](int tile, W1Set& S, uint32_t& pooled) {
+    pooled = 0;
+#pragma unroll
+    for (int u = 0; u < 4; ++u) {
+      const int m = tile * W1_TP + p0 + 16 * u;
+      const int mc = m < M ? m : M - 1;
+      uint32_t dpo;
+      if constexpr (FLAT) {
+        pooled |= 1u << u;
+        dpo = (uint32_t)(mc >> spw) * 128u;
+      } else {
+        const int nb = w1_quot(mc, Gl.by_hw), rem = mc - nb * HW;
+        const int gh_ = w1_quot(rem, Gl.by_w), gw = rem - gh_ * p.W;
+        const int gph = gh_ >> sph, gpw = gw >> spw;
+        pooled |= (gph < Gl.Hp && gpw < Gl.Wp ? 1u : 0u) << u;
+        dpo = ((uint32_t)(nb * Gl.Hp + min(gph, Gl.Hp - 1)) * (uint32_t)Gl.Wp + min(gpw, Gl.Wp - 1)) * 128u;
+      }
+      S.x[u] = w3_ld4<ABF>(p.in, xsrc + (size_t)mc * 128);
+      S.d[u] = w3_ld4<ABF>(Gl.dpool, dsrc + (size_t)dpo);
+    }
+  };
+  auto dlin_of = [&](float xn, float dp, float mk, uint32_t e) {
+    const float sg = sigmoid_fast(xn);
+    const float dres = dp * mk * drop_mul32(e, dkey, dthr, dscale);
+    return dres * sg;
+  };
+  auto convert = [&](int tile, const W1Set& S, uint32_t pooled, int stage) {
+    w3_lds_u16* xh = lds + stage * (W1_STAGE / 2);
+    w3_lds_u16* xl = xh + W1_PLANE / 2;
+    w3_lds_u16* dh_ = xh + W1_PLANE;
+    w3_lds_u16* dl = dh_ + W1_PLANE / 2;
+#pragma unroll
+    for (int u = 0; u < 4; ++u) {
+      const int m = tile * W1_TP + p0 + 16 * u;
+      const bool ok = m < M;
+      const float4 y = S.x[u], dp = S.d[u];
+      const float4 xn = make_float4(fmaf(y.x, sc.x, sh.x), fmaf(y.y, sc.y, sh.y), fmaf(y.z, sc.z, sh.z), fmaf(y.w, sc.w, sh.w));
+      const float4 v = make_float4(ok ? xn.x : 0.f, ok ? xn.y : 0.f, ok ? xn.z : 0.f, ok ? xn.w : 0.f);
+      w3_store4<ABF>(xh, xl, so + 16 * u * 128, v);
+      const float mk = (pooled >> u) & 1u ? inv_pool : 0.f;
+      const uint32_t e = (uint32_t)m * 128u + 4u * c4;
+      float4 g;
+      g.x = dlin_of(xn.x, dp.x, mk, e); g.y = dlin_of(xn.y, dp.y, mk, e + 1);
+      g.z = dlin_of(xn.z, dp.z, mk, e + 2); g.w = dlin_of(xn.w, dp.w, mk, e + 3);
+      g.x = ok ? g.x : 0.f; g.y = ok ? g.y : 0.f; g.z = ok ? g.z : 0.f; g.w = ok ? g.w : 0.f;
+      w3_store4<ABF>(dh_, dl, so + 16 * u * 128, g);
+    }
+  };
+  auto mma = [&](int stage) {
+    const uint32_t so_ = stage * W1_STAGE;
+#pragma unroll
+    for (int k = 0; k < W1_TP / 16; ++k) {
+      const uint32_t ko = so_ + k * 16 * 128 * 2;
+      const w3_bf16x8 ah = w3_frag(xa[0] + ko, xa[1] + ko);
+      const w3_bf16x8 al = w3_frag(xa[0] + ko + W1_PLANE, xa[1] + ko + W1_PLANE);
+      w3_bf16x8 bh[2], bl[2];
+#pragma unroll
+      for (int s = 0; s < 2; ++s) {
+        bh[s] = w3_frag(xb[s][0] + ko, xb[s][1] + ko);
+        bl[s] = w3_frag(xb[s][0] + ko + W1_PLANE, xb[s][1] + ko + W1_PLANE);
+      }
+#pragma unroll
+      for (int s = 0; s < 2; ++s) {
+        acc[s] = w3_mfma<ABF>(ah, al, bh[s], bl[s], acc[s]);
+      }
+    }
+  };
+
+  const int t0 = blockIdx.x, G = gridDim.x;
+  const int n = t0 < ntile ? (ntile - t0 + G - 1) / G : 0;
+  W1Set A, B;
+  uint32_t pa, pb;
+  if (n > 0) {
+    issue(t0, A, pa);
+    issue(t0 + G, B, pb);
+    convert(t0, A, pa, 0);
+    __syncthreads();
+    for (int i = 0; i < n; i += 2) {
+      issue(t0 + (i + 2) * G, A, pa);
+      mma(0);
+      convert(t0 + (i + 1) * G, B, pb, 1);
+      __syncthreads();
+      if (i + 1 >= n) break;
+      issue(t0 + (i + 3) * G, B, pb);
+      mma(1);
+      convert(t0 + (i + 2) * G, A, pa, 0);
+      __syncthreads();
+    }
+  }
+#pragma unroll
+  for (int s = 0; s < 2; ++s)
+#pragma unroll
+    for (int r = 0; r < 16; ++r) {
+      const int ci = cit * 32 + crow(r, lh);
+      p.part[((size_t)blockIdx.x * 128 + ci) * 128 + (nt0 + 2 * s) * 32 + li] = acc[s][r];
+    }
+}
+
+int bsed_wgrad1g_check(const WgradParams& P, const char* who) {
+  const BsedWgradDesc& d = P.d;
+  const BsedGluDesc& g = *d.glu;
+  BSED_CHECK_ARG(!d.dy, "%s: dy and glu are both set: glu asks for d_lin formed on load INSTEAD of dy", who);
+  BSED_CHECK_ARG((g.ph == 1 || g.ph == 2) && (g.pw == 1 || g.pw == 2), "%s: glu: pooling windows ph, pw must be 1 or 2 "
+                 "(got %d, %d)", who, g.ph, g.pw);
+  BSED_CHECK_ARG(d.CIN == d.N && d.N == 128 && d.CINP == 128 && d.NP == 128, "%s: glu: built for CIN = N = 128 (got CIN = "
+                 "%d, N = %d): a thread forms the dy quad of the `in` quad it loads", who, d.CIN, d.N);
+  BSED_CHECK_ARG(d.ntaps == 1 && d.dh[0] == 0 && d.dw[0] == 0, "%s: glu: ntaps must be 1, the tap (0, 0)", who);
+  BSED_CHECK_ARG(d.in_pitch == 128, "%s: glu: in_pitch must be 128 (in = y with dense rows; got %d)", who, d.in_pitch);
+  BSED_CHECK_ARG(d.a_scale && d.a_shift, "%s: glu: a_scale and a_shift (BatchNorm's scale and shift) are required", who);
+  BSED_CHECK_ARG(!d.bn_y, "%s: glu: no bn_y (BatchNorm backward on load is another form of dy)", who);
+  BSED_CHECK_ARG(g.NB == d.NB && g.H == d.H && g.W == d.W && g.C == d.N && g.act_bf16 == d.act_bf16,
+                 "%s: glu: NB, H, W, C and act_bf16 of *glu must repeat the descriptor's", who);
+  BSED_CHECK_ARG(d.H >= g.ph && d.W >= g.pw, "%s: glu: H >= ph and W >= pw (an empty pooled map)", who);
+  return BSED_OK;
+}
+
+bool bsed_wgrad1g_takes(const WgradParams& P) {
+  return (long)P.d.NB * P.d.H * P.d.W * 128 < (1L << 32);
+}
+
+template <bool FLAT>
+static int launch_wgrad1g(const WgradParams& P, const W1Glu& Gl, const BsedLaunch& L) {
+  BSED_LABEL_ONLY(L, "wgrad1g_kernel<%s, %d>", FLAT ? "true" : "false", P.d.act_bf16 ? 1 : 0);
+  static BsedLdsOnce once, onceb;
+  if (P.d.act_bf16) {
+    BSED_HIP(bsed_max_lds(onceb, (const void*)wgrad1g_kernel<FLAT, 1>));
+    hipLaunchKernelGGL((wgrad1g_kernel<FLAT, 1>), L.grid, dim3(W1_THREADS), 2 * W1_STAGE, L.s, P, Gl);
+  } else {
+    BSED_HIP(bsed_max_lds(once, (const void*)wgrad1g_kernel<FLAT, 0>));
+    hipLaunchKernelGGL((wgrad1g_kernel<FLAT, 0>), L.grid, dim3(W1_THREADS), 2 * W1_STAGE, L.s, P, Gl);
+  }
+  BSED_LAUNCH_CHECK();
+  return BSED_OK;
+}
+int bsed_launch_wgrad1g(const WgradParams& P, const BsedLaunch& L) {
+  const BsedGluDesc& g = *P.d.glu;
+  W1Glu Gl;
+  Gl.dpool = g.dpool;
+  Gl.ph = g.ph; Gl.pw = g.pw; Gl.Hp = P.d.H / g.ph; Gl.Wp = P.d.W / g.pw;
+  Gl.drop_p = g.drop_p; Gl.rng_stream = g.rng_stream; Gl.seed = g.seed;
+  Gl.seed_add = bsed_seed_add_ptr();
+  Gl.by_hw = w1_div((uint32_t)(P.d.H * P.d.W)); Gl.by_w = w1_div((uint32_t)P.d.W);
+  return g.ph == 1 && P.d.W % g.pw == 0 ? launch_wgrad1g<true>(P, Gl, L) : launch_wgrad1g<false>(P, Gl, L);
+}
diff --git a/bird-sound-event-detecion_amd/csrc/wgrad_tiles.h b/bird-sound-event-detecion_amd/csrc/wgrad_tiles.h
--- a/bird-sound-event-detecion_amd/csrc/wgrad_tiles.h
+++ b/bird-sound-event-detecion_amd/csrc/wgrad_tiles.h
@@ -1,6 +1,13 @@
 #pragma once
 #include "bsed_common.h"
 #include "../../include/bsed.h"
+
+struct WgradParams {
+  BsedWgradDesc d;
+  int PW, PH, PP, lgTW, dy_off, ntiles, nct, ntw;
+  int CC, lgc4, pw_magic;
+  int pack2;
+};
 
 struct W3Tile { int nb, th0, tw0; size_t in_img, dy_img; };
 __device__ __forceinline__ W3Tile w3_tile(const BsedWgradDesc& p, int tile) {
@@ -66,3 +73,14 @@
     }
   }
 }
+
+#define W1_TP 64
+#define W1_THREADS 512
+#define W1_PLANE (W1_TP * 128 * 2)
+#define W1_STAGE (4 * W1_PLANE)
+
+struct W1Set { float4 x[4], d[4]; };
+
+int bsed_wgrad1g_check(const WgradParams& P, const char* who);
+bool bsed_wgrad1g_takes(const WgradParams& P);
+int bsed_launch_wgrad1g(const WgradParams& P, const BsedLaunch& L);
diff --git a/bird-sound-event-detecion_amd/ops.py b/bird-sound-event-detecion_amd/ops.py
--- a/bird-sound-event-detecion_amd/ops.py
+++ b/bird-sound-event-detecion_amd/ops.py
@@ -750,10 +750,10 @@
 _frag_tables = {}
 
 
-def glu_bwd3n(y, scale, shift, w, bias, dpool, B, H, W, C, pool, drop_p, rng_stream, seed):
+def glu_bwd3n(y, scale, shift, w, bias, dpool, B, H, W, C, pool, drop_p, rng_stream, seed, store_dlin=True):
     dev = y.device
     g = torch.empty_like(y)
-    dlin = torch.empty_like(y)
+    dlin = torch.empty_like(y) if store_dlin else None
     d, plan = _glu_desc("bsed_glu_bwd3n", B, H, W, C, pool, drop_p, rng_stream, seed, y=y, scale=scale,
                         shift=shift, w=w, bias=bias, dpool=dpool, g=g, dlin=dlin)
     tb = _frag_tables.get(str(dev))
@@ -762,9 +762,48 @@
     part_db = torch.empty((plan.G, 2, C), device=dev, dtype=torch.float32)
     part_st = torch.empty((plan.G, 2, C), device=dev, dtype=torch.float32)
     d.part_db, d.part_st, d.frag_table = L.ptr(part_db), L.ptr(part_st), tb.data_ptr()
-    _glu_launch("bsed_glu_bwd3n", d, plan, 2 * 2.0 * B * H * W * C * C,
-                _esz(y) * B * H * W * C * (3.0 + 1.0 / (pool[0] * pool[1])))
+    nbytes = _esz(y) * B * H * W * C * ((3.0 if store_dlin else 2.0) + 1.0 / (pool[0] * pool[1]))
+    if store_dlin or L.timer is None:
+        _glu_launch("bsed_glu_bwd3n", d, plan, 2 * 2.0 * B * H * W * C * C, nbytes)
+    else:
+        _launch((f"glu_bwd3k_kernel<{d.act_bf16}>", 1, C, C, H, W), 2 * 2.0 * B * H * W * C * C,
+                lambda: L.call("bsed_glu_bwd3n", ctypes.byref(d), L.stream()), nbytes)
     return g, dlin, part_db, part_st, plan.G
+
+
+def glu_wgrad_plan(B, H, W, C, pool, act_bf16=0):
+    gd = GluDesc(NB=B, H=H, W=W, C=C, ph=pool[0], pw=pool[1], act_bf16=act_bf16)
+    d = WgradDesc()
+    _tile_taps(d, H, W, TAP1)
+    d.NB, d.H, d.W, d.CIN, d.CINP, d.N, d.NP = B, H, W, C, round_up(C, 32), C, round_up(C, 32)
+    d.in_pitch, d.dy_pitch, d.act_bf16 = C, C, act_bf16
+    d.a_scale = d.a_shift = 0x1000
+    d.glu = ctypes.addressof(gd)
+    plan = ContractPlan()
+    if L.lib().bsed_wgrad_plan(ctypes.byref(d), L.CONSTANTS["BSED_CONTRACT_WGRAD3"], ctypes.byref(plan)) != 0:
+        return None
+    return d, gd, plan
+
+
+@functools.lru_cache(maxsize=None)
+def _glu_dlin_on_load(B, H, W, C, pool, act_bf16):
+    planned = glu_wgrad_plan(B, H, W, C, pool, act_bf16)
+    return planned is not None and planned[2].G > 0
+
+
+def wgrad_glu(y, dpool, scale, shift, B, H, W, C, pool, drop_p, rng_stream, seed, G=None):
+    planned = glu_wgrad_plan(B, H, W, C, pool, _abf(y, dpool))
+    if planned is None:
+        raise L.BsedError("wgrad_glu: " + L.lib().bsed_last_error().decode())
+    d, gd, plan = planned
+    G = G or plan.G or min(256, plan.max_G)
+    gd.dpool, gd.drop_p, gd.rng_stream, gd.seed = _pa(dpool), drop_p, rng_stream, seed
+    part = torch.empty((G, 1, d.CINP, d.NP), device=y.device, dtype=torch.float32)
+    d.in_, d.part, d.a_scale, d.a_shift, d.G = _dp(y), _p(part), _p(scale), _p(shift), G
+    _launch((plan.label.decode(), 1, C, C, H, W), 2.0 * B * H * W * C * C,
+            lambda: L.call("bsed_wgrad3", ctypes.byref(d), L.stream()),
+            _esz(y) * B * H * W * C * (1.0 + 1.0 / (pool[0] * pool[1])))
+    return part, G, d.CINP, d.NP
 
 
 def glu_route(direction, C, W, pool, mode, fused=True):
@@ -803,14 +842,21 @@
     dpool = dpool.contiguous()
     tail = (pool, drop_p, rng_stream, seed)
     if route in ("glu3n", "unfused"):
+        on_load = False
         if route == "glu3n":
-            g, dlin, pdb, st2, _ = glu_bwd3n(y, scale, shift, w, bias, dpool, B, H, W, C, *tail)
+            on_load = _glu_dlin_on_load(B, H, W, C, tuple(pool), _abf(y, dpool))
+            g, dlin, pdb, st2, _ = glu_bwd3n(y, scale, shift, w, bias, dpool, B, H, W, C, *tail, store_dlin=not on_load)
         else:
             tt = torch.empty_like(y)
             dlin, pdb = igemm(y, pack_weight(w, 1, C, C, 0, 1, C), C, B, H, W, C, bias=bias, epilogue=EPI_GLU_BWD,
                               a_scale=scale, a_shift=shift, e_src=y, e_scale=scale, e_shift=shift, e_dpool=dpool,
                               out2=tt, pool=pool, drop_p=drop_p, rng_stream=rng_stream, seed=seed)
         stats_to_grad(pdb, C, 0, db)
+        if on_load:
+            gv = linear_weight(dw)
+            part, G, KP, NP = wgrad_glu(y, dpool, scale, shift, B, H, W, C, *tail)
+            reduce_partials(part, G, 1, KP, NP, gv.K, gv.N, gv.tensor, gv.s_tap, gv.s_k, gv.s_n, dst_offset=gv.offset)
+            return g, st2
         weight_grad(y, dlin, linear_weight(dw), B, H, W, a_scale=scale, a_shift=shift, mode=mode)
         if route == "unfused":
             g, st2 = igemm(dlin, pack_weight(w, 1, C, C, 0, C, 1), C, B, H, W, C, epilogue=EPI_ADD_STATS2, out=tt,
diff --git a/include/bsed.h b/include/bsed.h
--- a/include/bsed.h
+++ b/include/bsed.h
@@ -133,6 +133,7 @@
   const float* bn_mean;
   float* dy_out;
   int act_bf16;
+  const struct BsedGluDesc* glu;
   const void* w3s;
   float* d_in;
   int din_pitch;
```

Result: no change. 21840 clips/s, median of 2 (+0.1%).
